# Parskatt/RoMa

Hardware: AMD Instinct MI355X
Metric: image-pairs/sec, roma_outdoor 560->864, batch=8 per GPU (higher is better)
Workload: dtype bf16; 1 GPU; roma_outdoor match() 560->864, symmetric, upsample_preds, 8 pairs/GPU/step, seeded synthetic weights + N(0,1) images; precision policy of the reference's bf16 timing script: bfloat16 DINOv2 + float16 autocast for VGG / decoder / refiners (ROMA_MIXED), f32 accumulate; precision_policy=mixed, global_batch=8, streams_per_gpu=2, parallelism=single GPU, outputs_finite=True

## Files before the change

include/roma_hip.h:

```cpp
#ifndef ROMA_HIP_H
#define ROMA_HIP_H
#include <stdint.h>
#ifdef __cplusplus
extern "C" {
#endif

typedef struct roma_model* roma_handle_t;

enum { ROMA_F32 = 0, ROMA_BF16 = 1, ROMA_F16 = 2,
       ROMA_MIXED = 3 };
int roma_h16_format(void);
enum { ROMA_ERR_ARG = -1, ROMA_ERR_HIP = -2, ROMA_ERR_STATE = -3 };

typedef struct {
  int coarse_h, coarse_w;
  int upsample_h, upsample_w;
  int symmetric;
  int upsample_preds;
  int attenuate_cert;
  int precision;
  int max_batch;
  int device;
} roma_config_t;

const char* roma_last_error(void);
const char* roma_version(void);
#define ROMA_ABI_VERSION 5
int roma_abi_stamp(void);
int roma_self_check(void);

typedef struct {
  const float *ln1_w, *ln1_b, *ln2_w, *ln2_b;
  const float *ls1, *ls2;
  const void *qkv_w, *proj_w, *fc1_w, *fc2_w;
  const float *qkv_b, *proj_b, *fc1_b, *fc2_b;
  int qkv_ldw, proj_ldw, fc1_ldw, fc2_ldw;
} roma_vit_block_t;

typedef struct {
  int B, H, W;
  int act;
  int bf16_residual;
  const float *im_a, *im_b;
  const void* patch_w;
  const float* patch_b;
  int patch_ldw;
  const float *cls_tok, *pos_emb;
  const roma_vit_block_t* blocks;
  int nblocks;
  const float *norm_w, *norm_b;
  void *col, *pt, *x, *xs, *ln, *ao, *hid, *q, *k, *vt;
  void* feat_out;
} roma_vit_args_t;
int roma_vit_forward(const roma_vit_args_t* a, void* stream);
int roma_op_convert_from_bf16(const void* in_bf16, void* out_h16, long n, void* stream);

int roma_create(const roma_config_t* cfg, roma_handle_t* out);
int roma_set_tensor(roma_handle_t h, const char* name, int ndim, const int64_t* shape, const void* data, int is_int64);
int roma_finalize(roma_handle_t h);
int roma_set_option(roma_handle_t h, const char* key, int value);
int roma_set_option_f(roma_handle_t h, const char* key, double value);
int roma_match(roma_handle_t h, int B, const float* im_a, const float* im_b, const float* im_a_hr,
               const float* im_b_hr, float* warp_out, float* cert_out, void* stream);
typedef struct {
  int upsample;
  int symmetric;
  double scale_factor;
  const float* seed_flow;
  const float* seed_cert;
  int seed_h, seed_w;
  float* flow[5];
  float* cert[5];
  void* feat[5];
} roma_forward_args_t;
int roma_forward(roma_handle_t h, int B, const float* im_a, const float* im_b, const roma_forward_args_t* a, void* stream);
long roma_debug_fetch(roma_handle_t h, const char* name, void* dst_host, long nbytes);
int roma_debug_inject(roma_handle_t h, const char* name, const void* src_host, long nbytes);
long roma_debug_trace(roma_handle_t h, int slot, unsigned long long* sums_host, long max_entries, char* names_host,
                      long names_bytes);
int roma_destroy(roma_handle_t h);
int roma_tuning(const char* key, int value);
long roma_tuning_describe(char* buf, long nbytes);
long roma_debug_gemm_trace(unsigned int* dst_host, long nbytes);
int roma_profile_enable(int on);
long roma_profile_report(char* buf, long nbytes);


int roma_op_local_corr(const void* feature0, const void* feature1, const float* warp, void* out, int B, int H, int W,
                       int C, int K, int nearest, int dt_in, int dt_out, void* stream);
int roma_op_local_corr_window(const void* feature0, const void* feature1, const float* warp, void* out, int B, int H,
                              int W, int C, int radius, float scale, long ldo, int dt_in, int dt_out, void* stream);

int roma_op_gemm(const void* A, long lda, const void* W, long ldw, void* C, long ldc, int M, int N, int K, int batch,
                 long sA, long sW, long sC, const float* bias, const float* scale, const float* res, long ldr,
                 int act, float alpha, int dt_in, int dt_out, void* stream);
int roma_op_conv3x3(const void* in, const void* w, const float* bias, void* out, int B, int H, int W, int Cin, int Cout,
                    int relu, int dt, void* stream);
int roma_op_conv3x3_slab(const void* in, const void* w, const float* bias, void* out, int B, int H, int W, int Cin, int Cout,
                         int relu, int dt, void* stream);
int roma_op_attention(const void* q, const void* k, const void* vt, void* out, int B, int heads, int N, int npad, int hd,
                      int dt_in, int dt_out, void* stream);
int roma_op_qkv_scatter_gemm(const void* A, const void* W, const float* bias, void* q, void* k, void* vt, int B, int N,
                             int npad, int heads, int hd, int K, int dt_in, int dt_out, void* stream);
int roma_op_layernorm(const float* x, const float* w, const float* b, void* out, long M, int D, float eps, int dt_out,
                      void* stream);
int roma_op_layernorm_dt(const void* x, int dt_in, const float* w, const float* b, void* out, long M, int D, float eps,
                         int dt_out, void* stream);
int roma_op_gemm_res_bf16(const void* A, long lda, const void* W, long ldw, void* C, long ldc, int M, int N, int K,
                          const float* bias, const float* scale, const void* res, long ldr, void* stream);
int roma_op_cholesky_solve_t(float* A, float* Ft, float* LT, float* Linv, float* LinvT, int n, int d, int batch,
                             void* stream);
int roma_op_gp(const void* x, const void* y, const float* pos_w, const float* pos_b, float* mu, int b, int h, int w, int dt,
               void* stream);
int roma_op_cls_to_flow(const float* logits, long ld, float* flow, float* cert, long M, void* stream);
int roma_op_resize_bilinear(const float* in, float* out, int B, int Hin, int Win, int Hout, int Wout, int nc,
                            void* stream);
int roma_op_refiner_input(const void* feat, long ldf, const float* flow, void* d, long ldd, const float* emb_w,
                          const float* emb_b, int B, int H, int W, int C, int E, int Kcorr, int nimg, int shift,
                          float disp_scale, int dt, void* stream);
int roma_op_dwconv5x5(const void* in, void* out, const float* w, const float* bias, int B, int H, int W, int Cp, int dt,
                      void* stream);
int roma_op_refiner_block(const void* in, void* out, const float* dw_w, const float* dw_b, const void* pw,
                          const float* pw_b, int B, int H, int W, int Cp, int dt, void* stream);
int roma_op_refiner_block_final(const void* in, float* delta, const float* dw_w, const float* dw_b, const void* pw_final,
                                const float* bias_final, int B, int H, int W, int Cp, int dt, void* stream);
int roma_op_refiner_apply_delta(const float* delta, float* flow, float* cert, long M, float sx, float sy, void* stream);
int roma_op_kde(const float* x, long n, int down, float std, int half_inputs, float* density, void* stream);
int roma_op_sample_warp_at(const float* warp, const float* cert, int H, int W, const float* xa, long n, float* xa_to_b,
                           float* cert_a, void* stream);
int roma_op_mutual_nn(const float* a, long na, const float* b, long nb, const float* cert_a, float cert_th, float max_dist,
                      int* match_b, void* ws_a, void* ws_b, void* stream);
int roma_op_mutual_nn_count(const float* a, long na, const float* b, long nb, const float* cert_a, float cert_th, float max_dist,
                            void* ws_a, void* ws_b, long long* offsets, void* stream);
int roma_op_mutual_nn_fill(const float* a, long na, const float* b, long nb, const float* cert_a, float cert_th, float max_dist,
                           const void* ws_a, const void* ws_b, long long* offsets, long long* pairs, void* stream);
long roma_op_multinomial_workspace(long n, long k);
int roma_op_multinomial(const float* weights, long n, long k, unsigned long long seed, long long* out_indices, void* workspace,
                        long workspace_bytes, void* stream);
long roma_op_ransac_workspace(int B, int N);
int roma_op_ransac(int model, const float* kpts_a, const float* kpts_b, const int* counts, const unsigned long long* seeds, int B,
                   int N, float threshold, double confidence, int max_iters, int refine, double* out_model, unsigned char* out_mask,
                   unsigned char* out_ok, int* out_info, void* workspace, long workspace_bytes, void* stream);
long roma_op_magsac_workspace(int B, int N);
int roma_op_magsac(int model, const float* kpts_a, const float* kpts_b, const int* counts, const unsigned long long* seeds, int B,
                   int N, float threshold, double confidence, int max_iters, int lo_iters, double* out_model, unsigned char* out_mask,
                   unsigned char* out_ok, int* out_info, double* out_score, void* workspace, long workspace_bytes, void* stream);
long roma_op_essential_workspace(int B, int N);
int roma_op_essential(const float* kpts_a, const float* kpts_b, const int* counts, const unsigned long long* seeds,
                      const double* camera_matrix, int B, int N, float threshold, double prob, int max_iters, double* out_e,
                      unsigned char* out_mask, unsigned char* out_ok, int* out_info, void* workspace, long workspace_bytes,
                      void* stream);
long roma_op_essential_magsac_workspace(int B, int N);
int roma_op_essential_magsac(const float* kpts_a, const float* kpts_b, const int* counts, const unsigned long long* seeds,
                             const double* camera_matrix, int B, int N, float threshold, double prob, int max_iters, int lo_iters,
                             double* out_e, unsigned char* out_mask, unsigned char* out_ok, int* out_info, double* out_score,
                             void* workspace, long workspace_bytes, void* stream);
int roma_op_essential_minimal(const double* x0, const double* x1, int S, double* out_e, int* out_n, void* stream);
long roma_op_recover_pose_workspace(int B, int N);
int roma_op_recover_pose(const double* E, const float* kpts_a, const float* kpts_b, const unsigned char* mask, const int* counts,
                         const double* camera_matrix, int B, int N, double distance_thresh, int* out_n_good, double* out_r,
                         double* out_t, unsigned char* out_mask, void* workspace, long workspace_bytes, void* stream);
long roma_op_refine_pose_workspace(int B, int N);
int roma_op_refine_pose(const double* R, const double* t, const float* kpts_a, const float* kpts_b, const int* counts,
                        const unsigned char* valid, int B, int N, double thr, int max_steps, double* out_r, double* out_t,
                        unsigned char* out_mask, int* out_info, void* workspace, long workspace_bytes, void* stream);
long roma_op_refine_model_workspace(int B, int N);
int roma_op_refine_model(int model, const double* M, const float* kpts_a, const float* kpts_b, const int* counts,
                         const unsigned char* valid, int B, int N, double thr, int max_steps, double* out_m, unsigned char* out_mask,
                         int* out_info, double* out_cost, void* workspace, long workspace_bytes, void* stream);
int roma_op_nchw_to_nhwc(const float* in, float* out, int B, int C, int H, int W, void* stream);
int roma_op_tiny_pos_embed(const float* corr_volume, float* out, int B, int H1, int W1, int H0, int W0, int exact_softmax,
                           void* stream);
int roma_op_gray_instnorm(const float* in, float* out, int B, int H, int W, int C, float eps, void* stream);
int roma_op_conv2d_nhwc(const float* in, const float* w, const float* bias, const float* res, float* out, int B, int H, int W,
                        int Cin, int Cout, int K, int stride, int pad, int relu, void* stream);
int roma_op_avgpool_nhwc(const float* in, float* out, int B, int H, int W, int C, int k, void* stream);
int roma_op_add3(const float* a, const float* b, const float* c, float* out, long n, void* stream);
int roma_op_tiny_matcher_input(const float* f0, const float* f1, const float* warp, int warp_channels, float* d, int B, int H,
                               int W, int H1, int W1, int C, int Cp, void* stream);
int roma_op_tiny_update(const float* base, int base_channels, const float* delta, long ldd, float sx, float sy, float* out,
                        long npix, void* stream);
int roma_op_tiny_final(const float* matches, float* warp, float* certainty, int B, int H, int W, void* stream);
int roma_op_visualize_warp(const float* warp, const float* certainty, const float* im_a, const float* im_b, int H, int W,
                           int symmetric, int im_h, int im_w, float* out, void* stream);
int roma_op_fb_consistency(const float* flow_fwd, const float* flow_bwd, int B, int H, int W, float th_n, float* out,
                           void* stream);
int roma_op_maxpool2x2(const void* in, void* out, int B, int H, int W, int C, int dt, void* stream);
int roma_op_pool_proj(const void* in, void* pooled, void* pf, const void* pw, long ldw, const float* pb, int N, int ldf, int B, int H,
                      int W, int C, int dt, void* stream);
int roma_op_refiner_out(const void* d, long ldd, int dt, const float* w, const float* b, float* flow, float* cert, long M,
                        int Cp, float sx, float sy, void* stream);
int roma_op_conv3x3_c3(const float* img, const float* w, const float* bias, void* out, int B, int H, int W, int dt_out,
                       void* stream);
int roma_op_conv3x3_c3_bf16(const float* img, const void* w, const float* bias, void* out, int B, int H, int W, void* stream);

#ifdef __cplusplus
}
#endif
#endif
```

roma_amd/_lib.py:

```python
from __future__ import annotations

import ctypes as C
import os

_HERE = os.path.dirname(os.path.abspath(__file__))
_HERE = os.environ.get("ROMA_LIB_DIR", _HERE)
LIB_PATH = os.path.join(_HERE, "libroma_hip.so")
LIB_PATHS = {"bf16": LIB_PATH, "f16": os.path.join(_HERE, "libroma_hip_f16.so")}

ROMA_F32, ROMA_BF16, ROMA_F16, ROMA_MIXED = 0, 1, 2, 3
H16_CODE = {"bf16": ROMA_BF16, "f16": ROMA_F16}


class RomaConfig(C.Structure):
    _fields_ = [("coarse_h", C.c_int), ("coarse_w", C.c_int), ("upsample_h", C.c_int), ("upsample_w", C.c_int),
                ("symmetric", C.c_int), ("upsample_preds", C.c_int), ("attenuate_cert", C.c_int),
                ("precision", C.c_int), ("max_batch", C.c_int), ("device", C.c_int)]


class RomaForwardArgs(C.Structure):
    _fields_ = [("upsample", C.c_int), ("symmetric", C.c_int), ("scale_factor", C.c_double),
                ("seed_flow", C.c_void_p), ("seed_cert", C.c_void_p), ("seed_h", C.c_int), ("seed_w", C.c_int),
                ("flow", C.c_void_p * 5), ("cert", C.c_void_p * 5), ("feat", C.c_void_p * 5)]


_vp, _i, _l, _f = C.c_void_p, C.c_int, C.c_long, C.c_float

SIGNATURES = {
    "roma_last_error": (C.c_char_p, []),
    "roma_version": (C.c_char_p, []),
    "roma_h16_format": (_i, []),
    "roma_abi_stamp": (_i, []),
    "roma_self_check": (_i, []),
    "roma_create": (_i, [C.POINTER(RomaConfig), C.POINTER(_vp)]),
    "roma_set_tensor": (_i, [_vp, C.c_char_p, _i, C.POINTER(C.c_int64), _vp, _i]),
    "roma_finalize": (_i, [_vp]),
    "roma_set_option": (_i, [_vp, C.c_char_p, _i]),
    "roma_set_option_f": (_i, [_vp, C.c_char_p, C.c_double]),
    "roma_match": (_i, [_vp, _i, _vp, _vp, _vp, _vp, _vp, _vp, _vp]),
    "roma_forward": (_i, [_vp, _i, _vp, _vp, C.POINTER(RomaForwardArgs), _vp]),
    "roma_debug_fetch": (_l, [_vp, C.c_char_p, _vp, _l]),
    "roma_debug_trace": (_l, [_vp, _i, _vp, _l, C.c_char_p, _l]),
    "roma_debug_inject": (_i, [_vp, C.c_char_p, _vp, _l]),
    "roma_destroy": (_i, [_vp]),
    "roma_tuning": (_i, [C.c_char_p, _i]),
    "roma_tuning_describe": (_l, [C.c_char_p, _l]),
    "roma_debug_gemm_trace": (_l, [_vp, _l]),
    "roma_vit_forward": (_i, [_vp, _vp]),
    "roma_op_convert_from_bf16": (_i, [_vp, _vp, _l, _vp]),
    "roma_profile_enable": (_i, [_i]),
    "roma_profile_report": (_l, [C.c_char_p, _l]),
    "roma_op_local_corr": (_i, [_vp, _vp, _vp, _vp, _i, _i, _i, _i, _i, _i, _i, _i, _vp]),
    "roma_op_local_corr_window": (_i, [_vp, _vp, _vp, _vp, _i, _i, _i, _i, _i, _f, _l, _i, _i, _vp]),
    "roma_op_gemm": (_i, [_vp, _l, _vp, _l, _vp, _l, _i, _i, _i, _i, _l, _l, _l, _vp, _vp, _vp, _l, _i, _f, _i, _i, _vp]),
    "roma_op_conv3x3": (_i, [_vp, _vp, _vp, _vp, _i, _i, _i, _i, _i, _i, _i, _vp]),
    "roma_op_conv3x3_slab": (_i, [_vp, _vp, _vp, _vp, _i, _i, _i, _i, _i, _i, _i, _vp]),
    "roma_op_attention": (_i, [_vp, _vp, _vp, _vp, _i, _i, _i, _i, _i, _i, _i, _vp]),
    "roma_op_qkv_scatter_gemm": (_i, [_vp, _vp, _vp, _vp, _vp, _vp, _i, _i, _i, _i, _i, _i, _i, _i, _vp]),
    "roma_op_layernorm": (_i, [_vp, _vp, _vp, _vp, _l, _i, _f, _i, _vp]),
    "roma_op_layernorm_dt": (_i, [_vp, _i, _vp, _vp, _vp, _l, _i, _f, _i, _vp]),
    "roma_op_gemm_res_bf16": (_i, [_vp, _l, _vp, _l, _vp, _l, _i, _i, _i, _vp, _vp, _vp, _l, _vp]),
    "roma_op_cholesky_solve_t": (_i, [_vp, _vp, _vp, _vp, _vp, _i, _i, _i, _vp]),
    "roma_op_gp": (_i, [_vp, _vp, _vp, _vp, _vp, _i, _i, _i, _i, _vp]),
    "roma_op_cls_to_flow": (_i, [_vp, _l, _vp, _vp, _l, _vp]),
    "roma_op_resize_bilinear": (_i, [_vp, _vp, _i, _i, _i, _i, _i, _i, _vp]),
    "roma_op_refiner_input": (_i, [_vp, _l, _vp, _vp, _l, _vp, _vp, _i, _i, _i, _i, _i, _i, _i, _i, _f, _i, _vp]),
    "roma_op_dwconv5x5": (_i, [_vp, _vp, _vp, _vp, _i, _i, _i, _i, _i, _vp]),
    "roma_op_refiner_block": (_i, [_vp, _vp, _vp, _vp, _vp, _vp, _i, _i, _i, _i, _i, _vp]),
    "roma_op_refiner_block_final": (_i, [_vp, _vp, _vp, _vp, _vp, _vp, _i, _i, _i, _i, _i, _vp]),
    "roma_op_refiner_apply_delta": (_i, [_vp, _vp, _vp, _l, _f, _f, _vp]),
    "roma_op_kde": (_i, [_vp, _l, _i, _f, _i, _vp, _vp]),
    "roma_op_sample_warp_at": (_i, [_vp, _vp, _i, _i, _vp, _l, _vp, _vp, _vp]),
    "roma_op_mutual_nn": (_i, [_vp, _l, _vp, _l, _vp, _f, _f, _vp, _vp, _vp, _vp]),
    "roma_op_mutual_nn_count": (_i, [_vp, _l, _vp, _l, _vp, _f, _f, _vp, _vp, _vp, _vp]),
    "roma_op_mutual_nn_fill": (_i, [_vp, _l, _vp, _l, _vp, _f, _f, _vp, _vp, _vp, _vp, _vp]),
    "roma_op_fb_consistency": (_i, [_vp, _vp, _i, _i, _i, _f, _vp, _vp]),
    "roma_op_visualize_warp": (_i, [_vp, _vp, _vp, _vp, _i, _i, _i, _i, _i, _vp, _vp]),
    "roma_op_multinomial_workspace": (_l, [_l, _l]),
    "roma_op_multinomial": (_i, [_vp, _l, _l, C.c_ulonglong, _vp, _vp, _l, _vp]),
    "roma_op_ransac_workspace": (_l, [_i, _i]),
    "roma_op_ransac": (_i, [_i, _vp, _vp, _vp, _vp, _i, _i, _f, C.c_double, _i, _i, _vp, _vp, _vp, _vp, _vp, _l, _vp]),
    "roma_op_magsac_workspace": (_l, [_i, _i]),
    "roma_op_magsac": (_i, [_i, _vp, _vp, _vp, _vp, _i, _i, _f, C.c_double, _i, _i, _vp, _vp, _vp, _vp, _vp, _vp, _l, _vp]),
    "roma_op_essential_workspace": (_l, [_i, _i]),
    "roma_op_essential": (_i, [_vp, _vp, _vp, _vp, _vp, _i, _i, _f, C.c_double, _i, _vp, _vp, _vp, _vp, _vp, _l, _vp]),
    "roma_op_essential_magsac_workspace": (_l, [_i, _i]),
    "roma_op_essential_magsac": (_i, [_vp, _vp, _vp, _vp, _vp, _i, _i, _f, C.c_double, _i, _i, _vp, _vp, _vp, _vp, _vp, _vp, _l, _vp]),
    "roma_op_essential_minimal": (_i, [_vp, _vp, _i, _vp, _vp, _vp]),
    "roma_op_recover_pose_workspace": (_l, [_i, _i]),
    "roma_op_recover_pose": (_i, [_vp, _vp, _vp, _vp, _vp, _vp, _i, _i, C.c_double, _vp, _vp, _vp, _vp, _vp, _l, _vp]),
    "roma_op_refine_pose_workspace": (_l, [_i, _i]),
    "roma_op_refine_pose": (_i, [_vp, _vp, _vp, _vp, _vp, _vp, _i, _i, C.c_double, _i, _vp, _vp, _vp, _vp, _vp, _l, _vp]),
    "roma_op_refine_model_workspace": (_l, [_i, _i]),
    "roma_op_refine_model": (_i, [_i, _vp, _vp, _vp, _vp, _vp, _i, _i, C.c_double, _i, _vp, _vp, _vp, _vp, _vp, _l, _vp]),
    "roma_op_nchw_to_nhwc": (_i, [_vp, _vp, _i, _i, _i, _i, _vp]),
    "roma_op_tiny_pos_embed": (_i, [_vp, _vp, _i, _i, _i, _i, _i, _i, _vp]),
    "roma_op_gray_instnorm": (_i, [_vp, _vp, _i, _i, _i, _i, _f, _vp]),
    "roma_op_conv2d_nhwc": (_i, [_vp, _vp, _vp, _vp, _vp, _i, _i, _i, _i, _i, _i, _i, _i, _i, _vp]),
    "roma_op_avgpool_nhwc": (_i, [_vp, _vp, _i, _i, _i, _i, _i, _vp]),
    "roma_op_add3": (_i, [_vp, _vp, _vp, _vp, _l, _vp]),
    "roma_op_tiny_matcher_input": (_i, [_vp, _vp, _vp, _i, _vp, _i, _i, _i, _i, _i, _i, _i, _vp]),
    "roma_op_tiny_update": (_i, [_vp, _i, _vp, _l, _f, _f, _vp, _l, _vp]),
    "roma_op_tiny_final": (_i, [_vp, _vp, _vp, _i, _i, _i, _vp]),
    "roma_op_maxpool2x2": (_i, [_vp, _vp, _i, _i, _i, _i, _i, _vp]),
    "roma_op_pool_proj": (_i, [_vp, _vp, _vp, _vp, _l, _vp, _i, _i, _i, _i, _i, _i, _i, _vp]),
    "roma_op_conv3x3_c3": (_i, [_vp, _vp, _vp, _vp, _i, _i, _i, _i, _vp]),
    "roma_op_conv3x3_c3_bf16": (_i, [_vp, _vp, _vp, _vp, _i, _i, _i, _vp]),
    "roma_op_refiner_out": (_i, [_vp, _l, _i, _vp, _vp, _vp, _vp, _l, _i, _f, _f, _vp]),
}

_libs = {}


class RomaHipError(RuntimeError):
    pass


def load(fmt: str = "bf16"):
    if fmt in _libs:
        return _libs[fmt]
    path = LIB_PATHS[fmt]
    if not os.path.exists(path):
        raise ImportError(f"{path} not found - build it with `python -c 'import __graft_entry__ as g; g.build()'` "
                          "(roma_amd has no CPU fallback)")
    lib = C.CDLL(path)
    for name, (res, args) in SIGNATURES.items():
        fn = getattr(lib, name)
        fn.restype = res
        fn.argtypes = args
    if lib.roma_h16_format() != H16_CODE[fmt]:
        raise ImportError(f"{path} does not store {fmt} (roma_h16_format() = {lib.roma_h16_format()})")
    lib.h16 = fmt
    _libs[fmt] = lib
    return lib


def fmt_of(dtype) -> str:
    return "f16" if str(dtype) == "torch.float16" else "bf16"


def last_error(lib=None) -> str:
    return (lib or load()).roma_last_error().decode("utf-8", "replace")


def check(rc: int, exc=RomaHipError, lib=None):
    if rc != 0:
        raise exc(last_error(lib))
    return rc
```

roma_amd/csrc/api.hip:

```cpp
#include <algorithm>
#include <mutex>
#include <map>
#include <vector>
#include <dlfcn.h>
#include <string.h>

#include "../../include/roma_hip.h"
#include "attention.h"
#include "conv64.h"
#include "conv_patch.h"
#include "elementwise.h"
#include "gemm.h"
#include "local_corr.h"
#include "pool_proj.h"
#include "model.h"
#include "refiner_block.h"
#include "kde.h"
#include "keypoints.h"
#include "tiny.h"
#include "tuning.h"
#include "vit.h"
#include "sampling.h"
#include "essential.h"
#include "model_refine.h"
// ... 262 lines not shown
    first = false;
  }
  if (auto f = peer_sym<long (*)(char*, long)>("roma_profile_report")) {
    const long n = f(nullptr, 0);
    if (n > 3) {
      std::string peer((size_t)n, '\0');
      if (f(&peer[0], n) > 0) {
        peer.resize(strlen(peer.c_str()));
        if (peer.size() > 2) js += (first ? "" : ", ") + peer.substr(1, peer.size() - 2);
      }
    }
  }
  js += "}";
  if (!buf) return (long)js.size() + 1;
  if (nbytes < (long)js.size() + 1) return ROMA_ERR_ARG;
  memcpy(buf, js.c_str(), js.size() + 1);
  return (long)js.size() + 1;
}

int roma_op_local_corr(const void* feature0, const void* feature1, const float* warp, void* out, int B, int H, int W,
                       int C, int K, int nearest, int dt_in, int dt_out, void* stream) {
  LocalCorrArgs a;
  a.nearest = nearest ? 1 : 0;
  a.f0 = feature0; a.f1 = feature1; a.warp = warp; a.out = out; a.B = B; a.H = H; a.W = W; a.C = C; a.K = K;
  a.ld0 = C; a.ld1 = C; a.ldo = K; a.nimg = B; a.f1_shift = 0; a.scale = 1.f; a.in_dt = DT(dt_in); a.out_dt = DT(dt_out);
  return local_corr_general_launch(a, S(stream));
}

int roma_op_local_corr_window(const void* feature0, const void* feature1, const float* warp, void* out, int B, int H,
                              int W, int C, int radius, float scale, long ldo, int dt_in, int dt_out, void* stream) {
  LocalCorrArgs a;
  a.f0 = feature0; a.f1 = feature1; a.warp = warp; a.out = out; a.B = B; a.H = H; a.W = W; a.C = C; a.radius = radius;
  a.ld0 = C; a.ld1 = C; a.ldo = ldo; a.nimg = B; a.f1_shift = 0; a.scale = scale; a.in_dt = DT(dt_in); a.out_dt = DT(dt_out);
  ROMA_REQUIRE(ldo >= (2 * radius + 1) * (2 * radius + 1), "local_corr_window: ldo < K");
  return local_corr_window_launch(a, S(stream));
}

int roma_op_gemm(const void* A, long lda, const void* W, long ldw, void* C, long ldc, int M, int N, int K, int batch,
                 long sA, long sW, long sC, const float* bias, const float* scale, const float* res, long ldr, int act,
                 float alpha, int dt_in, int dt_out, void* stream) {
  GemmArgs g;
  g.A = A; g.lda = lda; g.W = W; g.ldw = ldw; g.C = C; g.ldc = ldc; g.M = M; g.N = N; g.K = K; g.batch = batch;
  g.sA = sA; g.sW = sW; g.sC = sC; g.bias = bias; g.scale = scale; g.res = res; g.ldr = ldr; g.sR = sC; g.act = act;
  g.alpha = alpha; g.in_dt = DT(dt_in); g.out_dt = DT(dt_out);
  return gemm_launch(g, S(stream));
}

int roma_op_conv3x3(const void* in, const void* w, const float* bias, void* out, int B, int H, int W, int Cin, int Cout,
                    int relu, int dt, void* stream) {
  GemmArgs g;
  g.A = in; g.W = w; g.ldw = 9 * Cin; g.C = out; g.ldc = Cout; g.M = B * H * W; g.N = Cout; g.K = 9 * Cin;
  g.in_dt = DT(dt); g.out_dt = DT(dt); g.bias = bias; g.act = relu ? ACT_RELU : ACT_NONE;
  g.conv_h = H; g.conv_w = W; g.conv_c = Cin;
  return gemm_launch(g, S(stream));
}

int roma_op_conv3x3_slab(const void* in, const void* w, const float* bias, void* out, int B, int H, int W, int Cin, int Cout,
                         int relu, int dt, void* stream) {
  GemmArgs g;
  g.A = in; g.W = w; g.ldw = 9 * Cin; g.C = out; g.ldc = Cout; g.M = B * H * W; g.N = Cout; g.K = 9 * Cin;
  g.in_dt = DT(dt); g.out_dt = DT(dt); g.bias = bias; g.act = relu ? ACT_RELU : ACT_NONE;
  g.conv_h = H; g.conv_w = W; g.conv_c = Cin; g.conv_korder = 1;
  return gemm_launch(g, S(stream));
}

int roma_op_attention(const void* q, const void* k, const void* vt, void* out, int B, int heads, int N, int npad, int hd,
                      int dt_in, int dt_out, void* stream) {
  AttnArgs a;
  a.q = q; a.k = k; a.vt = vt; a.out = out; a.B = B; a.heads = heads; a.N = N; a.npad = npad; a.hd = hd;
  a.ldo = (long)heads * hd; a.in_dt = DT(dt_in); a.out_dt = DT(dt_out);
  return attention_launch(a, S(stream));
}

int roma_op_qkv_scatter_gemm(const void* A, const void* W, const float* bias, void* q, void* k, void* vt, int B, int N,
                             int npad, int heads, int hd, int K, int dt_in, int dt_out, void* stream) {
  GemmArgs g;
  g.A = A; g.lda = K; g.W = W; g.ldw = K; g.M = B * N; g.N = 3 * heads * hd; g.K = K; g.in_dt = DT(dt_in);
  g.out_dt = DT(dt_out); g.bias = bias; g.mode = EPI_QKV; g.q = q; g.k = k; g.vt = vt; g.heads = heads; g.hd = hd;
  g.ntok = N; g.npad = npad; g.qscale = 1.0f / sqrtf((float)hd);
  return gemm_launch(g, S(stream));
}

int roma_op_layernorm(const float* x, const float* w, const float* b, void* out, long M, int D, float eps, int dt_out,
                      void* stream) {
  return layernorm_launch(x, w, b, out, M, D, eps, DT(dt_out), S(stream));
}

int roma_op_layernorm_dt(const void* x, int dt_in, const float* w, const float* b, void* out, long M, int D, float eps,
                         int dt_out, void* stream) {
  return layernorm_launch_dt(x, DT(dt_in), w, b, out, M, D, eps, DT(dt_out), S(stream));
}

int roma_op_gemm_res_bf16(const void* A, long lda, const void* W, long ldw, void* C, long ldc, int M, int N, int K,
                          const float* bias, const float* scale, const void* res, long ldr, void* stream) {
  GemmArgs g;
  g.A = A; g.lda = lda; g.W = W; g.ldw = ldw; g.C = C; g.ldc = ldc; g.M = M; g.N = N; g.K = K;
  g.bias = bias; g.scale = scale; g.res_bf16 = res; g.ldr = ldr; g.in_dt = DT_BF16; g.out_dt = DT_BF16;
  return gemm_launch(g, S(stream));
}

int roma_op_cholesky_solve_t(float* A, float* Ft, float* LT, float* Linv, float* LinvT, int n, int d, int batch,
                             void* stream) {
  if (batch > 1 && Ft == A + (long)n * n)
    return cholesky_solve_t(A, Ft, LT, Linv, LinvT, n, d, batch, S(stream), (long)(n + d) * n, (long)(n + d) * n);
  return cholesky_solve_t(A, Ft, LT, Linv, LinvT, n, d, batch, S(stream));
}

int roma_op_gp(const void* x, const void* y, const float* pos_w, const float* pos_b, float* mu, int b, int h, int w, int dt,
               void* stream) {
  ROMA_REQUIRE(x && y && pos_w && pos_b && mu && b > 0 && h > 0 && w > 0, "roma_op_gp: bad arguments");
  hipStream_t st = S(stream);
  const int n = h * w;
  const size_t esz = DT(dt) == DT_F32 ? 4 : 2;
  Arena plan;
  plan.alloc((size_t)2 * b * n * 512 * esz);
  if (int rc = gp_posterior(nullptr, 512, DT(dt), b, false, h, w, pos_w, pos_b, mu, 512, plan, st, true)) return rc;
  Arena ar;
  ar.cap = plan.peak + 4096;
  ar.dry = false;
  ROMA_CHECK_HIP(hipMallocAsync(reinterpret_cast<void**>(&ar.base), ar.cap, st));
  char* pf = static_cast<char*>(ar.alloc((size_t)2 * b * n * 512 * esz));
  int rc = 0;
  if (hipMemcpyAsync(pf, x, (size_t)b * n * 512 * esz, hipMemcpyDeviceToDevice, st) != hipSuccess ||
      hipMemcpyAsync(pf + (size_t)b * n * 512 * esz, y, (size_t)b * n * 512 * esz, hipMemcpyDeviceToDevice, st) != hipSuccess) {
    set_error("roma_op_gp: device copy failed");
    rc = ROMA_ERR_HIP;
  }
  if (!rc) rc = gp_posterior(pf, 512, DT(dt), b, false, h, w, pos_w, pos_b, mu, 512, ar, st, false);
  (void)hipFreeAsync(ar.base, st);
  return rc;
}

int roma_op_cls_to_flow(const float* logits, long ld, float* flow, float* cert, long M, void* stream) {
  return cls_to_flow_launch(logits, ld, flow, cert, M, S(stream));
}

int roma_op_resize_bilinear(const float* in, float* out, int B, int Hin, int Win, int Hout, int Wout, int nc,
                            void* stream) {
  return resize_bilinear_launch(in, out, B, Hin, Win, Hout, Wout, nc, S(stream));
}

int roma_op_refiner_input(const void* feat, long ldf, const float* flow, void* d, long ldd, const float* emb_w,
                          const float* emb_b, int B, int H, int W, int C, int E, int Kcorr, int nimg, int shift,
                          float disp_scale, int dt, void* stream) {
  RefinerInputArgs a;
  a.feat = feat; a.ldf = ldf; a.flow = flow; a.d = d; a.ldd = ldd; a.emb_w = emb_w; a.emb_b = emb_b;
  a.B = B; a.H = H; a.W = W; a.C = C; a.E = E; a.Kcorr = Kcorr; a.nimg = nimg; a.shift = shift;
  a.disp_scale = disp_scale; a.dt = DT(dt);
  ROMA_REQUIRE(feat && flow && d && B > 0 && H > 0 && W > 0 && C > 0 && nimg > 0, "roma_op_refiner_input: bad arguments");
  ROMA_REQUIRE(ldd >= 2 * C + E + Kcorr && ldf >= C, "roma_op_refiner_input: row strides too small");
  return refiner_input_launch(a, S(stream));
}

int roma_op_dwconv5x5(const void* in, void* out, const float* w, const float* bias, int B, int H, int W, int Cp, int dt,
                      void* stream) {
  return dwconv5x5_launch(in, out, w, bias, B, H, W, Cp, DT(dt), S(stream));
}

int roma_op_refiner_block(const void* in, void* out, const float* dw_w, const float* dw_b, const void* pw,
                          const float* pw_b, int B, int H, int W, int Cp, int dt, void* stream) {
  if (refiner_block_wide_supported(Cp, DT(dt))) {
    const int rc = refiner_block_wide_try_launch(in, out, dw_w, dw_b, pw, Cp, pw_b, B, H, W, Cp, DT(dt), S(stream), true);
    if (rc <= 0) return rc;
    set_error("roma_op_refiner_block: the C = 576 kernel declined these tensors (16-byte aligned bf16 in / out / weights are required)");
    return ROMA_ERR_ARG;
  }
  return refiner_block_launch(in, out, dw_w, dw_b, pw, Cp, pw_b, B, H, W, Cp, DT(dt), S(stream));
}

int roma_op_refiner_block_final(const void* in, float* delta, const float* dw_w, const float* dw_b, const void* pw_final,
                                const float* bias_final, int B, int H, int W, int Cp, int dt, void* stream) {
  ROMA_REQUIRE(in && delta && dw_w && dw_b && pw_final && bias_final, "roma_op_refiner_block_final: null pointer");
  return refiner_block_final_launch(in, delta, dw_w, dw_b, pw_final, Cp, bias_final, B, H, W, Cp, DT(dt), S(stream));
}

int roma_op_refiner_apply_delta(const float* delta, float* flow, float* cert, long M, float sx, float sy, void* stream) {
  ROMA_REQUIRE(delta && flow && cert && M >= 0, "roma_op_refiner_apply_delta: null pointer");
  return refiner_apply_delta_launch(delta, flow, cert, M, sx, sy, S(stream));
}

int roma_op_kde(const float* x, long n, int down, float std, int half_inputs, float* density, void* stream) {
  return kde_launch(x, n, down, std, half_inputs, density, S(stream));
}

int roma_op_sample_warp_at(const float* warp, const float* cert, int H, int W, const float* xa, long n, float* xa_to_b,
                           float* cert_a, void* stream) {
  return sample_warp_at_launch(warp, cert, H, W, xa, n, xa_to_b, cert_a, S(stream));
}

int roma_op_mutual_nn(const float* a, long na, const float* b, long nb, const float* cert_a, float cert_th, float max_dist,
                      int* match_b, void* ws_a, void* ws_b, void* stream) {
  return mutual_nn_launch(a, na, b, nb, cert_a, cert_th, max_dist, match_b, static_cast<unsigned long long*>(ws_a),
                          static_cast<unsigned long long*>(ws_b), S(stream));
}

int roma_op_mutual_nn_count(const float* a, long na, const float* b, long nb, const float* cert_a, float cert_th, float max_dist,
                            void* ws_a, void* ws_b, long long* offsets, void* stream) {
  return mutual_nn_count_launch(a, na, b, nb, cert_a, cert_th, max_dist, static_cast<unsigned long long*>(ws_a),
                                static_cast<unsigned long long*>(ws_b), offsets, S(stream));
}
int roma_op_mutual_nn_fill(const float* a, long na, const float* b, long nb, const float* cert_a, float cert_th, float max_dist,
                           const void* ws_a, const void* ws_b, long long* offsets, long long* pairs, void* stream) {
  return mutual_nn_fill_launch(a, na, b, nb, cert_a, cert_th, max_dist, static_cast<const unsigned long long*>(ws_a),
                               static_cast<const unsigned long long*>(ws_b), offsets, pairs, S(stream));
}

long roma_op_multinomial_workspace(long n, long k) { return (long)multinomial_workspace_bytes(n, k); }
int roma_op_multinomial(const float* weights, long n, long k, unsigned long long seed, long long* out_indices, void* workspace,
                        long workspace_bytes, void* stream) {
  return multinomial_launch(weights, n, k, seed, out_indices, workspace, (size_t)workspace_bytes, S(stream));
}
long roma_op_ransac_workspace(int B, int N) { return (long)ransac_workspace_bytes(B, N); }
int roma_op_ransac(int model, const float* kpts_a, const float* kpts_b, const int* counts, const unsigned long long* seeds, int B,
                   int N, float threshold, double confidence, int max_iters, int refine, double* out_model, unsigned char* out_mask,
                   unsigned char* out_ok, int* out_info, void* workspace, long workspace_bytes, void* stream) {
  return ransac_launch(model, kpts_a, kpts_b, counts, seeds, B, N, threshold, confidence, max_iters, refine, out_model, out_mask,
                       out_ok, out_info, workspace, (size_t)(workspace_bytes > 0 ? workspace_bytes : 0), S(stream));
}
long roma_op_magsac_workspace(int B, int N) { return (long)magsac_workspace_bytes(B, N); }
int roma_op_magsac(int model, const float* kpts_a, const float* kpts_b, const int* counts, const unsigned long long* seeds, int B,
                   int N, float threshold, double confidence, int max_iters, int lo_iters, double* out_model, unsigned char* out_mask,
                   unsigned char* out_ok, int* out_info, double* out_score, void* workspace, long workspace_bytes, void* stream) {
  return magsac_launch(model, kpts_a, kpts_b, counts, seeds, B, N, threshold, confidence, max_iters, lo_iters, out_model, out_mask,
                       out_ok, out_info, out_score, workspace, (size_t)(workspace_bytes > 0 ? workspace_bytes : 0), S(stream));
}
long roma_op_essential_workspace(int B, int N) { return (long)essential_workspace_bytes(B, N); }
int roma_op_essential(const float* kpts_a, const float* kpts_b, const int* counts, const unsigned long long* seeds,
                      const double* camera_matrix, int B, int N, float threshold, double prob, int max_iters, double* out_e,
                      unsigned char* out_mask, unsigned char* out_ok, int* out_info, void* workspace, long workspace_bytes,
                      void* stream) {
  return essential_launch(kpts_a, kpts_b, counts, seeds, camera_matrix, B, N, threshold, prob, max_iters, out_e, out_mask, out_ok,
                          out_info, workspace, (size_t)(workspace_bytes > 0 ? workspace_bytes : 0), S(stream));
}
long roma_op_essential_magsac_workspace(int B, int N) { return (long)essential_magsac_workspace_bytes(B, N); }
int roma_op_essential_magsac(const float* kpts_a, const float* kpts_b, const int* counts, const unsigned long long* seeds,
                             const double* camera_matrix, int B, int N, float threshold, double prob, int max_iters, int lo_iters,
                             double* out_e, unsigned char* out_mask, unsigned char* out_ok, int* out_info, double* out_score,
                             void* workspace, long workspace_bytes, void* stream) {
  return essential_magsac_launch(kpts_a, kpts_b, counts, seeds, camera_matrix, B, N, threshold, prob, max_iters, lo_iters, out_e,
                                 out_mask, out_ok, out_info, out_score, workspace,
                                 (size_t)(workspace_bytes > 0 ? workspace_bytes : 0), S(stream));
}
int roma_op_essential_minimal(const double* x0, const double* x1, int S_, double* out_e, int* out_n, void* stream) {
  return essential_minimal_launch(x0, x1, S_, out_e, out_n, S(stream));
}
long roma_op_recover_pose_workspace(int B, int N) { return (long)recover_pose_workspace_bytes(B, N); }
int roma_op_recover_pose(const double* E, const float* kpts_a, const float* kpts_b, const unsigned char* mask, const int* counts,
                         const double* camera_matrix, int B, int N, double distance_thresh, int* out_n_good, double* out_r,
                         double* out_t, unsigned char* out_mask, void* workspace, long workspace_bytes, void* stream) {
  return recover_pose_launch(E, kpts_a, kpts_b, mask, counts, camera_matrix, B, N, distance_thresh, out_n_good, out_r, out_t,
                             out_mask, workspace, (size_t)(workspace_bytes > 0 ? workspace_bytes : 0), S(stream));
}
long roma_op_refine_pose_workspace(int B, int N) { return (long)refine_pose_workspace_bytes(B, N); }
int roma_op_refine_pose(const double* R, const double* t, const float* kpts_a, const float* kpts_b, const int* counts,
                        const unsigned char* valid, int B, int N, double thr, int max_steps, double* out_r, double* out_t,
                        unsigned char* out_mask, int* out_info, void* workspace, long workspace_bytes, void* stream) {
  return refine_pose_launch(R, t, kpts_a, kpts_b, counts, valid, B, N, thr, max_steps, out_r, out_t, out_mask, out_info, workspace,
                            (size_t)(workspace_bytes > 0 ? workspace_bytes : 0), S(stream));
}
long roma_op_refine_model_workspace(int B, int N) { return (long)refine_model_workspace_bytes(B, N); }
int roma_op_refine_model(int model, const double* M, const float* kpts_a, const float* kpts_b, const int* counts,
                         const unsigned char* valid, int B, int N, double thr, int max_steps, double* out_m, unsigned char* out_mask,
                         int* out_info, double* out_cost, void* workspace, long workspace_bytes, void* stream) {
  return refine_model_launch(model, M, kpts_a, kpts_b, counts, valid, B, N, thr, max_steps, out_m, out_mask, out_info, out_cost,
                             workspace, (size_t)(workspace_bytes > 0 ? workspace_bytes : 0), S(stream));
}
int roma_op_nchw_to_nhwc(const float* in, float* out, int B, int C, int H, int W, void* stream) {
  return nchw_to_nhwc_launch(in, out, B, C, H, W, S(stream));
}
int roma_op_tiny_pos_embed(const float* corr_volume, float* out, int B, int H1, int W1, int H0, int W0, int exact_softmax,
                           void* stream) {
  return tiny_pos_embed_launch(corr_volume, out, B, H1, W1, H0, W0, exact_softmax, S(stream));
}
int roma_op_gray_instnorm(const float* in, float* out, int B, int H, int W, int C, float eps, void* stream) {
  return gray_instnorm_launch(in, out, B, H, W, C, eps, S(stream));
}
int roma_op_conv2d_nhwc(const float* in, const float* w, const float* bias, const float* res, float* out, int B, int H, int W,
                        int Cin, int Cout, int K, int stride, int pad, int relu, void* stream) {
  return conv2d_nhwc_launch(in, w, bias, res, out, B, H, W, Cin, Cout, K, stride, pad, relu, S(stream));
}
int roma_op_avgpool_nhwc(const float* in, float* out, int B, int H, int W, int C, int k, void* stream) {
  return avgpool_nhwc_launch(in, out, B, H, W, C, k, S(stream));
}
int roma_op_add3(const float* a, const float* b, const float* c, float* out, long n, void* stream) {
  return add3_launch(a, b, c, out, n, S(stream));
}
int roma_op_tiny_matcher_input(const float* f0, const float* f1, const float* warp, int warp_channels, float* d, int B, int H,
                               int W, int H1, int W1, int C, int Cp, void* stream) {
  return tiny_matcher_input_launch(f0, f1, warp, warp_channels, d, B, H, W, H1, W1, C, Cp, S(stream));
}
int roma_op_tiny_update(const float* base, int base_channels, const float* delta, long ldd, float sx, float sy, float* out,
                        long npix, void* stream) {
  return tiny_update_launch(base, base_channels, delta, ldd, sx, sy, out, npix, S(stream));
}
int roma_op_tiny_final(const float* matches, float* warp, float* certainty, int B, int H, int W, void* stream) {
  return tiny_final_launch(matches, warp, certainty, B, H, W, S(stream));
}
int roma_op_visualize_warp(const float* warp, const float* certainty, const float* im_a, const float* im_b, int H, int W,
                           int symmetric, int im_h, int im_w, float* out, void* stream) {
  return visualize_warp_launch(warp, certainty, im_a, im_b, H, W, symmetric, im_h, im_w, out, S(stream));
}
int roma_op_fb_consistency(const float* flow_fwd, const float* flow_bwd, int B, int H, int W, float th_n, float* out,
                           void* stream) {
  return fb_consistency_launch(flow_fwd, flow_bwd, B, H, W, th_n, out, S(stream));
}

int roma_op_maxpool2x2(const void* in, void* out, int B, int H, int W, int C, int dt, void* stream) {
  return maxpool2x2_launch(in, out, B, H, W, C, DT(dt), S(stream));
}
// ... 23 lines not shown
```

roma_amd/csrc/dwconv_ring.hip:

```cpp
#include <stdlib.h>

#include <algorithm>

#include "elementwise.h"
#include "tuning.h"
#include "gemm.h"

namespace roma {

typedef __attribute__((ext_vector_type(2))) float f32x2;
#define ROMA_LDS __attribute__((address_space(3)))
typedef ROMA_LDS unsigned char lds_u8;

__device__ __attribute__((aligned(256))) unsigned int g_dwr_zero_page[64];

constexpr int DWR_ROWB = 3072;
constexpr int DWR_PXW = 16;
constexpr int DWR_NR = 6;
constexpr int DWR_RING = 4 * DWR_NR * DWR_ROWB;
static_assert(3 * (DWR_NR - 1) + 4 * (DWR_NR - 1) <= 63, "vmcnt is a 6-bit counter");
static_assert(2 * DWR_RING <= 160 * 1024, "two workgroups per CU");

#define ROMA_DWR_WAIT_VM(N) asm volatile("s_waitcnt vmcnt(%0)" ::"n"(N) : "memory")

__device__ __forceinline__ void dwr_glds16(const char* src, lds_u8* lds_wave_base) {
  __builtin_amdgcn_global_load_lds((const __attribute__((address_space(1))) void*)src, (ROMA_LDS void*)lds_wave_base, 16, 0, 0);
}

__device__ __forceinline__ void dwr_read(unsigned long long (&cr)[8], unsigned rd) {
  asm volatile(
      "ds_read_b64 %0, %8\n\tds_read_b64 %1, %8 offset:128\n\tds_read_b64 %2, %8 offset:256\n\t"
      "ds_read_b64 %3, %8 offset:384\n\tds_read_b64 %4, %8 offset:640\n\tds_read_b64 %5, %8 offset:768\n\t"
      "ds_read_b64 %6, %8 offset:896\n\tds_read_b64 %7, %8 offset:1024"
      : "=&v"(cr[0]), "=&v"(cr[1]), "=&v"(cr[2]), "=&v"(cr[3]), "=&v"(cr[4]), "=&v"(cr[5]), "=&v"(cr[6]), "=&v"(cr[7])
      : "v"(rd)
      : "memory");
}
__device__ __forceinline__ void dwr_wait(unsigned long long (&cr)[8]) {
  asm volatile("s_waitcnt lgkmcnt(0)"
               : "+v"(cr[0]), "+v"(cr[1]), "+v"(cr[2]), "+v"(cr[3]), "+v"(cr[4]), "+v"(cr[5]), "+v"(cr[6]), "+v"(cr[7])::"memory");
}

__device__ __forceinline__ void dwr_row(f32x2 (&acc)[5][4][2], const f32x4 (&wreg)[25], f32x2 bias0, f32x2 bias1,
                                        unsigned long long (&cr)[8], unsigned rd_next, bool store, bf16_t* orow, long Cp, int npx) {
  f32x2 v[8][2];
#define ROMA_DWR_CVT(J)                                                  \
  {                                                                      \
    const uint32_t lo_ = (uint32_t)cr[J], hi_ = (uint32_t)(cr[J] >> 32); \
    v[J][0] = f32x2{h16_lo(lo_), h16_hi(lo_)};                           \
    v[J][1] = f32x2{h16_lo(hi_), h16_hi(hi_)};                           \
  }
  ROMA_DWR_CVT(0) ROMA_DWR_CVT(1) ROMA_DWR_CVT(2) ROMA_DWR_CVT(3) ROMA_DWR_CVT(4) ROMA_DWR_CVT(5) ROMA_DWR_CVT(6) ROMA_DWR_CVT(7)
#undef ROMA_DWR_CVT
#pragma unroll
  for (int j = 0; j < 8; ++j) asm volatile("" : "+v"(v[j][0]), "+v"(v[j][1]));
  dwr_read(cr, rd_next);
#pragma unroll
  for (int kx = 0; kx < 5; ++kx) {
    __builtin_amdgcn_sched_barrier(0);
#pragma unroll
    for (int k = 0; k < 5; ++k) {
      const f32x4 wx = wreg[(4 - k) * 5 + kx];
      const f32x2 w0 = f32x2{wx[0], wx[1]}, w1 = f32x2{wx[2], wx[3]};
#pragma unroll
      for (int px = 0; px < 4; ++px) {
        acc[k][px][0] = v[px + kx][0] * w0 + (k == 4 && kx == 0 ? bias0 : acc[k][px][0]);
        acc[k][px][1] = v[px + kx][1] * w1 + (k == 4 && kx == 0 ? bias1 : acc[k][px][1]);
      }
    }
    __builtin_amdgcn_sched_barrier(0);
  }
  if (store) {
#pragma unroll
    for (int px = 0; px < 4; ++px) {
      if (px < npx) {
        uint2 u;
        u.x = pack_relu_h16x2(acc[0][px][0][0], acc[0][px][0][1]);
        u.y = pack_relu_h16x2(acc[0][px][1][0], acc[0][px][1][1]);
        *reinterpret_cast<uint2*>(orow + (long)px * Cp) = u;
      }
    }
  }
#pragma unroll
  for (int k = 0; k < 4; ++k)
#pragma unroll
    for (int px = 0; px < 4; ++px) {
      acc[k][px][0] = acc[k + 1][px][0];
      acc[k][px][1] = acc[k + 1][px][1];
    }
  dwr_wait(cr);
}

__global__ __launch_bounds__(256, 2) void dwconv5x5_ring_kernel(const bf16_t* __restrict__ in, bf16_t* __restrict__ out,
                                                                const float* __restrict__ w, const float* __restrict__ bias,
                                                                int B, int H, int W, int Cp, int SY, int nchunk, int nxg,
                                                                long ntasks) {
  constexpr int NR = DWR_NR;
  __shared__ __attribute__((aligned(1024))) unsigned char ring[DWR_RING];
  const long nwg = (ntasks + 3) / 4, wg_per_xcd = (nwg + 7) / 8;
  const long lw = (long)(blockIdx.x % 8) * wg_per_xcd + blockIdx.x / 8;
  const int lane = threadIdx.x & 63;
  const int wv = __builtin_amdgcn_readfirstlane((int)(threadIdx.x >> 6));
  const long task = lw * 4 + wv;
  if (lw >= nwg || task >= ntasks) return;
  const int xg = (int)(task % nxg);
  long r = task / nxg;
  const int chunk = (int)(r % nchunk);
  r /= nchunk;
  const int yt = (H + SY - 1) / SY;
  const int ys = (int)(r % yt) * SY;
  const int b = (int)(r / yt);
  const int sy = min(SY, H - ys);
  const int T = sy + 4;

  const int cg = lane & 15, xq = lane >> 4;
  const int c = chunk * 64 + cg * 4;

  f32x4 wreg[25];
#pragma unroll
  for (int t = 0; t < 25; ++t) wreg[t] = *reinterpret_cast<const f32x4*>(w + (long)t * Cp + c);
  const f32x4 bx = *reinterpret_cast<const f32x4*>(bias + c);
#pragma unroll
  for (int t = 0; t < 25; ++t) asm volatile("" : "+v"(wreg[t]));
  const f32x2 bias0 = f32x2{bx[0], bx[1]}, bias1 = f32x2{bx[2], bx[3]};
  asm volatile("s_waitcnt vmcnt(0)" ::: "memory");

  const int xb = xg * DWR_PXW + xq * 4;
  const int x0 = xg * DWR_PXW - 2;
  const int npx = min(4, W - xb);

  const char* zsrc = reinterpret_cast<const char*>(g_dwr_zero_page);
  const char* inb = reinterpret_cast<const char*>(in + ((long)b * H * W) * Cp) + (long)chunk * 128;
  const long pitch = (long)W * Cp * 2;
  const __amdgpu_buffer_rsrc_t rs_in = __builtin_amdgcn_make_buffer_rsrc(const_cast<char*>(inb), 0, (int)((long)H * pitch - (long)chunk * 128), 0x00020000);
  unsigned voff[3];
#pragma unroll
  for (int i = 0; i < 3; ++i) {
    const int p = 64 * i + lane, s = p >> 3, part = p & 7;
    const int x = x0 + s - s / 5;
    const bool ok = (s % 5 != 4) && x >= 0 && x < W;
    voff[i] = ok ? (unsigned)(x * Cp * 2 + part * 16) : 0x80000000u;
  }
  unsigned vout = 0x80000000u;
  asm volatile("" : "+v"(vout));
  lds_u8* const myring = (lds_u8*)ring + wv * (NR * DWR_ROWB);
#define ROMA_DWR_BL16(VOFF, SOFF, DST) \
  __builtin_amdgcn_raw_ptr_buffer_load_lds(rs_in, (ROMA_LDS void*)(DST), 16, (int)(VOFF), (int)(SOFF), 0, 0)
#define ROMA_DWR_ISSUE(RROW, SLOT)                                                         \
  {                                                                                        \
    const int yy_ = ys - 2 + (RROW);                                                       \
    if ((RROW) < T && yy_ >= 0 && yy_ < H) {                             \
      const int so_ = yy_ * (int)pitch;                                                    \
      _Pragma("unroll") for (int i = 0; i < 3; ++i) ROMA_DWR_BL16(voff[i], so_, myring + (SLOT) * DWR_ROWB + i * 1024); \
    } else {                                                                               \
      _Pragma("unroll") for (int i = 0; i < 3; ++i) ROMA_DWR_BL16(vout, 0, myring + (SLOT) * DWR_ROWB + i * 1024); \
    }                                                                                      \
  }

  f32x2 acc[5][4][2];
#pragma unroll
  for (int s5 = 0; s5 < 5; ++s5)
#pragma unroll
    for (int px = 0; px < 4; ++px) {
      acc[s5][px][0] = bias0;
      acc[s5][px][1] = bias1;
    }
  const unsigned ring_lds = (unsigned)(size_t)myring;
  const unsigned rd0 = ring_lds + (unsigned)(xq * 5 * 128 + cg * 8);
  bf16_t* const obase = out + ((long)b * H * W) * Cp + c;

#pragma unroll
  for (int rr = 0; rr < NR - 1; ++rr) ROMA_DWR_ISSUE(rr, rr);
  unsigned long long cr[8];
  ROMA_DWR_WAIT_VM(3 * (NR - 2));
  dwr_read(cr, rd0);
  dwr_wait(cr);

  int slot1 = 1;
  int fill = NR - 1;
  bf16_t* orow = obase + ((long)ys * W + xb) * Cp;
  const long orow_step = (long)W * Cp;
#pragma nounroll
  for (int t = 0; t < T; ++t) {
    ROMA_DWR_ISSUE(t + NR - 1, fill);
    ROMA_DWR_WAIT_VM(3 * (NR - 2));
    const bool st = t >= 4;
    dwr_row(acc, wreg, bias0, bias1, cr, rd0 + (unsigned)slot1 * DWR_ROWB, st && npx > 0, orow, (long)Cp, npx);
    if (st) orow += orow_step;
    fill = fill + 1 == NR ? 0 : fill + 1;
    slot1 = slot1 + 1 == NR ? 0 : slot1 + 1;
  }
#undef ROMA_DWR_ISSUE
  ROMA_DWR_WAIT_VM(0);
}

int dwconv5x5_ring_try_launch(const void* in, void* out, const float* w, const float* bias, int B, int H, int W, int Cp, int dt,
                              hipStream_t s) {
  const int dw_ring = tuning(SW_DW_RING);
  if (!dw_ring) return 1;
  if (dt != DT_BF16 || Cp % 64 != 0 || Cp < 256 || H < 1 || W < 1) return 1;
  if ((long)H * W * Cp * 2 >= (1l << 31)) return 1;
  if ((reinterpret_cast<uintptr_t>(in) & 15) != 0 || (reinterpret_cast<uintptr_t>(out) & 7) != 0) return 1;
  if ((reinterpret_cast<uintptr_t>(w) & 15) != 0 || (reinterpret_cast<uintptr_t>(bias) & 15) != 0) return 1;
  const int nchunk = Cp / 64;
  const int nxg = (W + DWR_PXW - 1) / DWR_PXW;
  int SY = H;
  {
    long best = -1;
    const long per_strip = (long)B * nxg * nchunk;
    const int max_sy = std::max(6, (int)tuning(SW_DWR_MAXSY));
    for (int ns = (H + max_sy - 1) / max_sy; ns <= std::max(1, H / 6); ++ns) {
      const int sy = (H + ns - 1) / ns;
      const long nt = per_strip * ((H + sy - 1) / sy);
      const long cost = ((nt + 2047) / 2048) * (sy + 7);
      if (best < 0 || cost < best) {
        best = cost;
        SY = sy;
      }
    }
  }
  const long ntasks = (long)B * ((H + SY - 1) / SY) * nxg * nchunk;
  ROMA_REQUIRE(ntasks < (1l << 31), "dwconv5x5: grid too large");
  const long min_elems = tuning(SW_DW_RING_MINELEMS);
  if (dw_ring != 2 && (long)B * H * W * Cp < min_elems) return 1;
  ProfScope ps("dwconv5x5_kernel<" ROMA_H16_NAME ">", 2.0 * (double)B * H * W * Cp * 2.0, "byte", s);
  const long nwg = (ntasks + 3) / 4;
  hipLaunchKernelGGL(dwconv5x5_ring_kernel, dim3((unsigned)(((nwg + 7) / 8) * 8)), dim3(256), 0, s, (const bf16_t*)in,
                     (bf16_t*)out, w, bias, B, H, W, Cp, SY, nchunk, nxg, ntasks);
  ROMA_LAUNCH_CHECK();
  return 0;
}

}
```

roma_amd/csrc/elementwise.h:

```cpp
#pragma once
#include "common.h"

namespace roma {

int layernorm_launch(const float* x, const float* w, const float* b, void* out, long M, int D, float eps,
                     int dt_out, hipStream_t s);
int layernorm_launch_dt(const void* x, int dt_in, const float* w, const float* b, void* out, long M, int D, float eps,
                        int dt_out, hipStream_t s);

int conv3x3_c3_launch(const float* img, const float* w, const float* bias, void* out, int B, int H, int W,
                      int dt_out, hipStream_t s);

int im2col3x3_c3_launch(const float* img, void* out, int B, int H, int W, int dt_out, hipStream_t s);

int maxpool2x2_launch(const void* in, void* out, int B, int H, int W, int C, int dt, hipStream_t s);

int im2col_patch14_launch(const float* img, void* out, int B, int H, int W, int Kpad, int dt_out, hipStream_t s);

int assemble_tokens_launch(const float* patch, const float* cls, const float* pos, float* tokens, int B, int T,
                           int D, hipStream_t s);

int copy2d_launch(const void* in, long ldi, int dt_in, void* out, long ldo, int dt_out, long rows, int cols,
                  hipStream_t s);

int convert_from_bf16_launch(const void* in, void* out, long n, hipStream_t s);

int rownorm_launch(const void* in, long ld, int dt, float* norms, long M, int C, hipStream_t s);

int gp_basis_launch(const float* w, const float* b, float* Ft, int Dg, int h, int wdt, int npad, hipStream_t s, int copies = 1,
                    long stride = 0);

int transpose_launch(const float* in, float* out, int n, long ld, int batch, hipStream_t s, long stride_in = 0, long stride_out = 0);

int chol_diag_launch(float* A, long ld, long strideA, float* Linv, float* LinvT, int k, int nblk, int batch,
                     hipStream_t s);

int chol_col_launch(float* A, long ld, long strideA, float* LT, long strideLT, int n, int d, float* Linv, float* LinvT, int k,
                    int nblk, int batch, unsigned epoch, hipStream_t s);
int chol_col_restore_launch(float* A, long ld, long strideA, const float* LT, long strideLT, int n, int batch, hipStream_t s);

int pad_identity_launch(float* A, long ld, long strideA, int n, int npad, int batch, hipStream_t s);

int cls_to_flow_launch(const float* logits, long ld, float* flow, float* cert, long M, hipStream_t s);

struct RefinerInputArgs {
  const void* feat = nullptr;
  long ldf = 0;
  const float* flow = nullptr;
  void* d = nullptr;
  long ldd = 0;
  const float* emb_w = nullptr;
  const float* emb_b = nullptr;
  int B = 0, H = 0, W = 0, C = 0, E = 0, Kcorr = 0, nimg = 0, shift = 0;
  float disp_scale = 1.f;
  int dt = 0;
};
int refiner_input_launch(const RefinerInputArgs& a, hipStream_t s);

int dwconv5x5_launch(const void* in, void* out, const float* w, const float* bias, int B, int H, int W, int Cp,
                     int dt, hipStream_t s);
int dwconv5x5_ring_try_launch(const void* in, void* out, const float* w, const float* bias, int B, int H, int W, int Cp, int dt,
                              hipStream_t s);

int refiner_out_launch(const void* d, long ldd, int dt, const float* w , const float* b ,
                       float* flow, float* cert, long M, int Cp, float sx, float sy, hipStream_t s);
int refiner_apply_delta_launch(const float* delta, float* flow, float* cert, long M, float sx, float sy, hipStream_t s);

int resize_bilinear_launch(const float* in, float* out, int B, int Hin, int Win, int Hout, int Wout, int nc,
                           hipStream_t s);

struct FinalArgs {
  const float* flow = nullptr;
  const float* cert = nullptr;
  const float* cert16 = nullptr;
  float* warp = nullptr;
  float* certainty = nullptr;
  int B = 0, H = 0, W = 0, h16 = 0, w16 = 0, symmetric = 1;
};
int final_epilogue_launch(const FinalArgs& a, hipStream_t s);

int checksum_cols_launch(const void* p, long rows, int ld, int c0, int c1, unsigned long long* out, hipStream_t s);
int checksum_launch(const void* p, size_t bytes, unsigned long long* out, hipStream_t s);

}
```

roma_amd/csrc/elementwise.hip:

```cpp
#include <algorithm>
#include "elementwise.h"
#include "tuning.h"
#include "chol_diag.h"
#include <stdio.h>

#include <stdlib.h>
#include "gemm.h"

namespace roma {

#define ROMA_DT_SWITCH(dt, T, ...)            \
  if ((dt) == DT_F32) { using T = float; __VA_ARGS__; } else { using T = bf16_t; __VA_ARGS__; }

__device__ inline float wave_sum(float v) {
#pragma unroll
  for (int off = 32; off >= 1; off >>= 1) v += __shfl_xor(v, off);
  return v;
}

__device__ inline float pix_coord(int i, int n) {
  const float start = (float)(-1.0 + 1.0 / n), end = (float)(1.0 - 1.0 / n);
  if (n == 1) return start;
  const float step = (end - start) / (float)(n - 1);
  return (i < n / 2) ? start + step * (float)i : end - step * (float)(n - 1 - i);
// ... 357 lines not shown
  for (int j = ty; j < 32; j += 8)
    if (y0 + j < n && x0 + tx < n) tile[j][tx] = ib[(long)(y0 + j) * ld + x0 + tx];
  __syncthreads();
  for (int j = ty; j < 32; j += 8)
    if (x0 + j < n && y0 + tx < n) ob[(long)(x0 + j) * ld + y0 + tx] = tile[tx][j];
}

int transpose_launch(const float* in, float* out, int n, long ld, int batch, hipStream_t s, long stride_in, long stride_out) {
  dim3 grid((unsigned)((n + 31) / 32), (unsigned)((n + 31) / 32), (unsigned)batch);
  hipLaunchKernelGGL(transpose_kernel, grid, dim3(256), 0, s, in, out, n, ld, stride_in > 0 ? stride_in : (long)n * ld,
                     stride_out > 0 ? stride_out : (long)n * ld);
  ROMA_LAUNCH_CHECK();
  return 0;
}

__global__ __launch_bounds__(256) void chol_diag_kernel(float* A, long ld, long strideA, float* Linv, float* LinvT,
                                                        int k, int nblk) {
  constexpr int S = CHOL_S;
  __shared__ __attribute__((aligned(16))) float L[64 * S];
  __shared__ __attribute__((aligned(16))) float LT[64 * S];
  __shared__ __attribute__((aligned(16))) float XT[64 * S];
  __shared__ int progress;
  float* Ab = A + (long)blockIdx.x * strideA + ((long)k * 64) * ld + (long)k * 64;
  const int tid = threadIdx.x;
  const int wave = __builtin_amdgcn_readfirstlane(tid >> 6);
  const int i = tid & 63;
  for (int idx = tid; idx < 64 * 16; idx += 256) {
    const int row = idx >> 4, c4 = idx & 15;
    *reinterpret_cast<f32x4*>(&L[row * S + c4 * 4]) = *reinterpret_cast<const f32x4*>(Ab + (long)row * ld + c4 * 4);
  }
  if (tid == 0) progress = -1;
  __syncthreads();
  if (wave == 0) chol_diag_factor_wave(L, LT, &progress, i);
  else if (wave == 1) chol_diag_inverse_wave(L, XT, &progress, i);
  __syncthreads();
  chol_diag_writeback(L, XT, Ab, ld, Linv + ((long)blockIdx.x * nblk + k) * 4096, LinvT + ((long)blockIdx.x * nblk + k) * 4096,
                      tid, 256);
}

int chol_diag_launch(float* A, long ld, long strideA, float* Linv, float* LinvT, int k, int nblk, int batch,
                     hipStream_t s) {
  hipLaunchKernelGGL(chol_diag_kernel, dim3((unsigned)batch), dim3(256), 0, s, A, ld, strideA, Linv, LinvT, k, nblk);
  ROMA_LAUNCH_CHECK();
  return 0;
}

__global__ __launch_bounds__(256) void pad_identity_kernel(float* A, long ld, long strideA, int n, int npad) {
  float* Ab = A + (long)blockIdx.y * strideA;
  const long total = (long)npad * npad;
  for (long idx = (long)blockIdx.x * 256 + threadIdx.x; idx < total; idx += (long)gridDim.x * 256) {
    const int i = (int)(idx / npad), j = (int)(idx % npad);
    if (i >= n || j >= n) Ab[(long)i * ld + j] = (i == j) ? 1.f : 0.f;
  }
}

int pad_identity_launch(float* A, long ld, long strideA, int n, int npad, int batch, hipStream_t s) {
  if (npad == n) return 0;
  const long total = (long)npad * npad;
  dim3 grid((unsigned)std::min<long>((total + 255) / 256, 4096), (unsigned)batch);
  hipLaunchKernelGGL(pad_identity_kernel, grid, dim3(256), 0, s, A, ld, strideA, n, npad);
  ROMA_LAUNCH_CHECK();
  return 0;
}

__global__ __launch_bounds__(256) void cls_to_flow_kernel(const float* logits, long ld, float* flow, float* cert, long M) {
  const int lane = threadIdx.x & 63;
  const long row = (long)blockIdx.x * 4 + (threadIdx.x >> 6);
  if (row >= M) return;
  const float* lr = logits + row * ld;
  float mx = -INFINITY;
  int arg = 0;
  f32x4 v[16];
#pragma unroll
  for (int i = 0; i < 16; ++i) {
    v[i] = *reinterpret_cast<const f32x4*>(lr + (i * 64 + lane) * 4);
#pragma unroll
    for (int j = 0; j < 4; ++j)
      if (v[i][j] > mx) {
        mx = v[i][j];
        arg = (i * 64 + lane) * 4 + j;
      }
  }
#pragma unroll
  for (int off = 32; off >= 1; off >>= 1) {
    const float om = __shfl_xor(mx, off);
    const int oa = __shfl_xor(arg, off);
    if (om > mx || (om == mx && oa < arg)) {
      mx = om;
      arg = oa;
    }
  }
  float se = 0.f;
#pragma unroll
  for (int i = 0; i < 16; ++i)
#pragma unroll
    for (int j = 0; j < 4; ++j) se += expf(v[i][j] - mx);
  se = wave_sum(se);
  if (lane == 0) {
    const int idx5[5] = {arg - 1, arg, arg + 1, arg - 64, arg + 64};
    float fx = 0.f, fy = 0.f, tot = 0.f;
#pragma unroll
    for (int t = 0; t < 5; ++t) {
      const int c = min(max(idx5[t], 0), 4095);
      const float p = expf(lr[c] - mx) / se;
      fx += p * pix_coord(c & 63, 64);
      fy += p * pix_coord(c >> 6, 64);
      tot += p;
    }
    flow[row * 2 + 0] = fx / tot;
    flow[row * 2 + 1] = fy / tot;
    cert[row] = lr[4096];
  }
}

int cls_to_flow_launch(const float* logits, long ld, float* flow, float* cert, long M, hipStream_t s) {
  ROMA_REQUIRE(ld % 4 == 0 && ld >= 4097, "cls_to_flow: bad leading dimension");
  dim3 grid((unsigned)((M + 3) / 4));
  hipLaunchKernelGGL(cls_to_flow_kernel, grid, dim3(256), 0, s, logits, ld, flow, cert, M);
  ROMA_LAUNCH_CHECK();
  return 0;
}

template <typename T>
__global__ __launch_bounds__(256) void refiner_input_kernel(const RefinerInputArgs a) {
  const int lane = threadIdx.x & 63;
  const long HW = (long)a.H * a.W;
  const long pix = (long)blockIdx.x * 4 + (threadIdx.x >> 6);
  if (pix >= (long)a.B * HW) return;
  const int b = (int)(pix / HW);
  const long p = pix - (long)b * HW;
  const int y = (int)(p / a.W), x = (int)(p - (long)y * a.W);
  const T* feat = reinterpret_cast<const T*>(a.feat);
  const T* fq = feat + ((long)b * HW + p) * a.ldf;
  const int simg = (b + a.shift) % a.nimg;
  const T* fs = feat + (long)simg * HW * a.ldf;
  T* d = reinterpret_cast<T*>(a.d) + pix * a.ldd;
  const float wx = a.flow[pix * 2 + 0], wy = a.flow[pix * 2 + 1];
  float ix = ((wx + 1.f) * a.W - 1.f) * 0.5f, iy = ((wy + 1.f) * a.H - 1.f) * 0.5f;
  ix = fminf(fmaxf(ix, -1.0e6f), 1.0e6f);
  iy = fminf(fmaxf(iy, -1.0e6f), 1.0e6f);
  const float fx0 = floorf(ix), fy0 = floorf(iy);
  const int x0 = (int)fx0, y0 = (int)fy0;
  const float tx = ix - fx0, ty = iy - fy0;
  const float wgt[4] = {(1.f - tx) * (1.f - ty), tx * (1.f - ty), (1.f - tx) * ty, tx * ty};
  bool ok[4];
  long off[4];
#pragma unroll
  for (int t = 0; t < 4; ++t) {
    const int yy = y0 + (t >> 1), xx = x0 + (t & 1);
    ok[t] = yy >= 0 && yy < a.H && xx >= 0 && xx < a.W;
    off[t] = ((long)yy * a.W + xx) * a.ldf;
  }
  for (int c = lane * 4; c < a.C; c += 256) {
    ElemIO<T>::st4(d + c, ElemIO<T>::ld4(fq + c));
    f32x4 acc = {0.f, 0.f, 0.f, 0.f};
#pragma unroll
    for (int t = 0; t < 4; ++t)
      if (ok[t]) {
        const f32x4 v = ElemIO<T>::ld4(fs + off[t] + c);
        acc += wgt[t] * v;
      }
    ElemIO<T>::st4(d + a.C + c, acc);
  }
  const float dx = a.disp_scale * (wx - pix_coord(x, a.W)), dy = a.disp_scale * (wy - pix_coord(y, a.H));
  for (int e = lane; e < a.E; e += 64) {
    const float v = a.emb_w[e * 2 + 0] * dx + a.emb_w[e * 2 + 1] * dy + a.emb_b[e];
    ElemIO<T>::st(d + 2 * a.C + e, v);
  }
  for (long c = 2 * a.C + a.E + a.Kcorr + lane; c < a.ldd; c += 64) ElemIO<T>::st(d + c, 0.f);
}

template <typename T>
__global__ __launch_bounds__(256) void refiner_input_small_kernel(const RefinerInputArgs a) {
  const long HW = (long)a.H * a.W;
  const int slots = (int)a.ldd;
  const long total = (long)a.B * HW * slots;
  const T* feat = reinterpret_cast<const T*>(a.feat);
  for (long idx = (long)blockIdx.x * 256 + threadIdx.x; idx < total; idx += (long)gridDim.x * 256) {
    const int c = (int)(idx % slots);
    const long pix = idx / slots;
    const int b = (int)(pix / HW);
    const long p = pix - (long)b * HW;
    T* d = reinterpret_cast<T*>(a.d) + pix * a.ldd;
    if (c < a.C) {
      ElemIO<T>::st(d + c, ElemIO<T>::ld(feat + ((long)b * HW + p) * a.ldf + c));
    } else if (c < 2 * a.C) {
      const int cc = c - a.C;
      const int simg = (b + a.shift) % a.nimg;
      const T* fs = feat + (long)simg * HW * a.ldf;
      const float wx = a.flow[pix * 2 + 0], wy = a.flow[pix * 2 + 1];
      float ix = ((wx + 1.f) * a.W - 1.f) * 0.5f, iy = ((wy + 1.f) * a.H - 1.f) * 0.5f;
      ix = fminf(fmaxf(ix, -1.0e6f), 1.0e6f);
      iy = fminf(fmaxf(iy, -1.0e6f), 1.0e6f);
      const float fx0 = floorf(ix), fy0 = floorf(iy);
      const int x0 = (int)fx0, y0 = (int)fy0;
      const float tx = ix - fx0, ty = iy - fy0;
      const float wgt[4] = {(1.f - tx) * (1.f - ty), tx * (1.f - ty), (1.f - tx) * ty, tx * ty};
      float acc = 0.f;
#pragma unroll
      for (int t = 0; t < 4; ++t) {
        const int yy = y0 + (t >> 1), xx = x0 + (t & 1);
        if (yy >= 0 && yy < a.H && xx >= 0 && xx < a.W)
          acc += wgt[t] * ElemIO<T>::ld(fs + ((long)yy * a.W + xx) * a.ldf + cc);
      }
      ElemIO<T>::st(d + c, acc);
    } else if (c < 2 * a.C + a.E) {
      const int e = c - 2 * a.C;
      const int y = (int)(p / a.W), x = (int)(p - (long)y * a.W);
      const float dx = a.disp_scale * (a.flow[pix * 2 + 0] - pix_coord(x, a.W));
      const float dy = a.disp_scale * (a.flow[pix * 2 + 1] - pix_coord(y, a.H));
      ElemIO<T>::st(d + c, a.emb_w[e * 2 + 0] * dx + a.emb_w[e * 2 + 1] * dy + a.emb_b[e]);
    } else if (c >= 2 * a.C + a.E + a.Kcorr) {
      ElemIO<T>::st(d + c, 0.f);
    }
  }
}

template <typename T> struct VecIO;
template <> struct VecIO<float> {
  static constexpr int CV = 4;
  typedef f32x4 Raw;
  __device__ static inline Raw ldraw(const float* p) { return *reinterpret_cast<const f32x4*>(p); }
  __device__ static inline void cvt(const Raw& x, float* v) { v[0] = x[0]; v[1] = x[1]; v[2] = x[2]; v[3] = x[3]; }
  __device__ static inline void ld(const float* p, float* v) {
    const f32x4 x = *reinterpret_cast<const f32x4*>(p);
    v[0] = x[0]; v[1] = x[1]; v[2] = x[2]; v[3] = x[3];
  }
  __device__ static inline void st(float* p, const float* v) { *reinterpret_cast<f32x4*>(p) = f32x4{v[0], v[1], v[2], v[3]}; }
};
template <> struct VecIO<bf16_t> {
  static constexpr int CV = 8;
  typedef uint4 Raw;
  __device__ static inline Raw ldraw(const bf16_t* p) { return *reinterpret_cast<const uint4*>(p); }
  __device__ static inline void cvt(const Raw& u, float* v) {
    v[0] = h16_lo(u.x); v[1] = h16_hi(u.x);
    v[2] = h16_lo(u.y); v[3] = h16_hi(u.y);
    v[4] = h16_lo(u.z); v[5] = h16_hi(u.z);
    v[6] = h16_lo(u.w); v[7] = h16_hi(u.w);
  }
  __device__ static inline void ld(const bf16_t* p, float* v) {
    const uint4 u = *reinterpret_cast<const uint4*>(p);
    v[0] = h16_lo(u.x); v[1] = h16_hi(u.x);
    v[2] = h16_lo(u.y); v[3] = h16_hi(u.y);
    v[4] = h16_lo(u.z); v[5] = h16_hi(u.z);
    v[6] = h16_lo(u.w); v[7] = h16_hi(u.w);
  }
  __device__ static inline void st(bf16_t* p, const float* v) {
    uint4 u;
    u.x = pack_bf16x2(v[0], v[1]);
    u.y = pack_bf16x2(v[2], v[3]);
    u.z = pack_bf16x2(v[4], v[5]);
    u.w = pack_bf16x2(v[6], v[7]);
    *reinterpret_cast<uint4*>(p) = u;
  }
};

template <typename T, int C, int E>
__global__ __launch_bounds__(256) void refiner_input_pix_kernel(const RefinerInputArgs a) {
  constexpr int LDF = 16, LDD = 24;
  const long HW = (long)a.H * a.W;
  const long pix = (long)blockIdx.x * 256 + threadIdx.x;
  if (pix >= (long)a.B * HW) return;
  const int b = (int)(pix / HW);
  const long p = pix - (long)b * HW;
  const int y = (int)(p / a.W), x = (int)(p - (long)y * a.W);
  const T* feat = reinterpret_cast<const T*>(a.feat);
  const T* fq = feat + ((long)b * HW + p) * LDF;
  const int simg = (b + a.shift) % a.nimg;
  const T* fs = feat + (long)simg * HW * LDF;
  if constexpr (sizeof(T) == 2) {
    static_assert(C <= 16 && 2 * C + E <= LDD && LDD == 24 && LDF == 16, "layout");
    float q[16], xh[16];
    VecIO<T>::ld(fq, q);
    VecIO<T>::ld(fq + 8, q + 8);
#pragma unroll
    for (int j = 0; j < 16; ++j) xh[j] = 0.f;
    const float wx = a.flow[pix * 2 + 0], wy = a.flow[pix * 2 + 1];
    float ix = ((wx + 1.f) * a.W - 1.f) * 0.5f, iy = ((wy + 1.f) * a.H - 1.f) * 0.5f;
    ix = fminf(fmaxf(ix, -1.0e6f), 1.0e6f);
    iy = fminf(fmaxf(iy, -1.0e6f), 1.0e6f);
    const float fx0 = floorf(ix), fy0 = floorf(iy);
    const int x0 = (int)fx0, y0 = (int)fy0;
    const float tx = ix - fx0, ty = iy - fy0;
    const float wgt[4] = {(1.f - tx) * (1.f - ty), tx * (1.f - ty), (1.f - tx) * ty, tx * ty};
#pragma unroll
    for (int t = 0; t < 4; ++t) {
      const int yy = y0 + (t >> 1), xx = x0 + (t & 1);
      if (yy >= 0 && yy < a.H && xx >= 0 && xx < a.W) {
        const T* r = fs + ((long)yy * a.W + xx) * LDF;
        float v[16];
        VecIO<T>::ld(r, v);
        VecIO<T>::ld(r + 8, v + 8);
#pragma unroll
        for (int j = 0; j < C; ++j) xh[j] += wgt[t] * v[j];
      }
    }
    const float dx = a.disp_scale * (wx - pix_coord(x, a.W)), dy = a.disp_scale * (wy - pix_coord(y, a.H));
    float o[LDD];
#pragma unroll
    for (int c = 0; c < C; ++c) {
      o[c] = q[c];
      o[C + c] = xh[c];
    }
#pragma unroll
    for (int e = 0; e < E; ++e) o[2 * C + e] = a.emb_w[e * 2 + 0] * dx + a.emb_w[e * 2 + 1] * dy + a.emb_b[e];
#pragma unroll
    for (int c = 2 * C + E; c < LDD; ++c) o[c] = 0.f;
    T* d = reinterpret_cast<T*>(a.d) + pix * LDD;
#pragma unroll
    for (int c8 = 0; c8 < LDD / 8; ++c8) VecIO<T>::st(d + c8 * 8, o + c8 * 8);
    return;
  }
  float q[12], xh[12];
#pragma unroll
  for (int c4 = 0; c4 < 3; ++c4) {
    const f32x4 v = ElemIO<T>::ld4(fq + c4 * 4);
#pragma unroll
    for (int j = 0; j < 4; ++j) {
      q[c4 * 4 + j] = v[j];
      xh[c4 * 4 + j] = 0.f;
    }
  }
  const float wx = a.flow[pix * 2 + 0], wy = a.flow[pix * 2 + 1];
  float ix = ((wx + 1.f) * a.W - 1.f) * 0.5f, iy = ((wy + 1.f) * a.H - 1.f) * 0.5f;
  ix = fminf(fmaxf(ix, -1.0e6f), 1.0e6f);
  iy = fminf(fmaxf(iy, -1.0e6f), 1.0e6f);
  const float fx0 = floorf(ix), fy0 = floorf(iy);
  const int x0 = (int)fx0, y0 = (int)fy0;
  const float tx = ix - fx0, ty = iy - fy0;
  const float wgt[4] = {(1.f - tx) * (1.f - ty), tx * (1.f - ty), (1.f - tx) * ty, tx * ty};
#pragma unroll
  for (int t = 0; t < 4; ++t) {
    const int yy = y0 + (t >> 1), xx = x0 + (t & 1);
    if (yy >= 0 && yy < a.H && xx >= 0 && xx < a.W) {
      const T* r = fs + ((long)yy * a.W + xx) * LDF;
#pragma unroll
      for (int c4 = 0; c4 < 3; ++c4) {
        const f32x4 v = ElemIO<T>::ld4(r + c4 * 4);
#pragma unroll
        for (int j = 0; j < 4; ++j) xh[c4 * 4 + j] += wgt[t] * v[j];
      }
    }
  }
  const float dx = a.disp_scale * (wx - pix_coord(x, a.W)), dy = a.disp_scale * (wy - pix_coord(y, a.H));
  float o[LDD];
#pragma unroll
  for (int c = 0; c < C; ++c) {
    o[c] = q[c];
    o[C + c] = xh[c];
  }
#pragma unroll
  for (int e = 0; e < E; ++e) o[2 * C + e] = a.emb_w[e * 2 + 0] * dx + a.emb_w[e * 2 + 1] * dy + a.emb_b[e];
#pragma unroll
  for (int c = 2 * C + E; c < LDD; ++c) o[c] = 0.f;
  T* d = reinterpret_cast<T*>(a.d) + pix * LDD;
#pragma unroll
  for (int c4 = 0; c4 < LDD / 4; ++c4) ElemIO<T>::st4(d + c4 * 4, f32x4{o[c4 * 4], o[c4 * 4 + 1], o[c4 * 4 + 2], o[c4 * 4 + 3]});
}

template <typename T>
__global__ __launch_bounds__(256) void refiner_input_vec_kernel(const RefinerInputArgs a, int lpp) {
  constexpr int CV = VecIO<T>::CV;
  const int lane = threadIdx.x & 63;
  const int sub = lane & (lpp - 1), pw = lane / lpp, ppw = 64 / lpp;
  const long HW = (long)a.H * a.W;
  const long pix = ((long)blockIdx.x * 4 + (threadIdx.x >> 6)) * ppw + pw;
  if (pix >= (long)a.B * HW) return;
  const int b = (int)(pix / HW);
  const long p = pix - (long)b * HW;
  const int y = (int)(p / a.W), x = (int)(p - (long)y * a.W);
  const T* feat = reinterpret_cast<const T*>(a.feat);
  const T* fq = feat + ((long)b * HW + p) * a.ldf;
  const int simg = (b + a.shift) % a.nimg;
  const T* fs = feat + (long)simg * HW * a.ldf;
  T* d = reinterpret_cast<T*>(a.d) + pix * a.ldd;
  const float wx = a.flow[pix * 2 + 0], wy = a.flow[pix * 2 + 1];
  float ix = ((wx + 1.f) * a.W - 1.f) * 0.5f, iy = ((wy + 1.f) * a.H - 1.f) * 0.5f;
  ix = fminf(fmaxf(ix, -1.0e6f), 1.0e6f);
  iy = fminf(fmaxf(iy, -1.0e6f), 1.0e6f);
  const float fx0 = floorf(ix), fy0 = floorf(iy);
  const int x0 = (int)fx0, y0 = (int)fy0;
  const float tx = ix - fx0, ty = iy - fy0;
  const float wgt[4] = {(1.f - tx) * (1.f - ty), tx * (1.f - ty), (1.f - tx) * ty, tx * ty};
  bool ok[4];
  long off[4];
#pragma unroll
  for (int t = 0; t < 4; ++t) {
    const int yy = y0 + (t >> 1), xx = x0 + (t & 1);
    ok[t] = yy >= 0 && yy < a.H && xx >= 0 && xx < a.W;
    off[t] = ((long)min(max(yy, 0), a.H - 1) * a.W + min(max(xx, 0), a.W - 1)) * a.ldf;
  }
  for (int c = sub * CV; c < a.C; c += lpp * CV) {
    *reinterpret_cast<uint4*>(d + c) = *reinterpret_cast<const uint4*>(fq + c);
    float r[CV];
#pragma unroll
    for (int j = 0; j < CV; ++j) r[j] = 0.f;
#pragma unroll
    for (int t = 0; t < 4; ++t) {
      float tv[CV];
      VecIO<T>::ld(fs + off[t] + c, tv);
#pragma unroll
      for (int j = 0; j < CV; ++j) r[j] = ok[t] ? r[j] + wgt[t] * tv[j] : r[j];
    }
    VecIO<T>::st(d + a.C + c, r);
  }
  const float dx = a.disp_scale * (wx - pix_coord(x, a.W)), dy = a.disp_scale * (wy - pix_coord(y, a.H));
  for (int e = sub; e < a.E; e += lpp) {
    const float v = a.emb_w[e * 2 + 0] * dx + a.emb_w[e * 2 + 1] * dy + a.emb_b[e];
    ElemIO<T>::st(d + 2 * a.C + e, v);
  }
  for (long c = 2 * a.C + a.E + a.Kcorr + sub; c < a.ldd; c += lpp) ElemIO<T>::st(d + c, 0.f);
}

int refiner_input_launch(const RefinerInputArgs& a, hipStream_t s) {
  const long npix = (long)a.B * a.H * a.W;
  const double es = a.dt == DT_F32 ? 4.0 : 2.0;
  char pname[64];
  snprintf(pname, sizeof pname, "refiner_input_warp<C=%d,%s>", a.C, a.dt == DT_F32 ? "f32" : ROMA_H16_NAME);
  ProfScope ps(pname, (double)npix * (2.0 * a.C * es + 8.0 + (double)(a.ldd - a.Kcorr) * es), "byte", s);
  if (a.C == 9 && a.E == 6 && a.Kcorr == 0 && a.ldf == 16 && a.ldd == 24) {
    dim3 grid((unsigned)((npix + 255) / 256));
    ROMA_DT_SWITCH(a.dt, T, hipLaunchKernelGGL((refiner_input_pix_kernel<T, 9, 6>), grid, dim3(256), 0, s, a));
    ROMA_LAUNCH_CHECK();
    return 0;
  }
  if (a.C % 4 != 0 || a.C < 32) {
    const long total = npix * a.ldd;
    dim3 grid((unsigned)std::min<long>((total + 255) / 256, 1 << 20));
    ROMA_DT_SWITCH(a.dt, T, hipLaunchKernelGGL(refiner_input_small_kernel<T>, grid, dim3(256), 0, s, a));
    ROMA_LAUNCH_CHECK();
    return 0;
  }
  ROMA_REQUIRE(a.ldf % 4 == 0 && a.ldd % 4 == 0, "refiner_input: strides must be multiples of 4");
  {
    const int cv = a.dt == DT_F32 ? 4 : 8;
    const bool aligned = ((reinterpret_cast<uintptr_t>(a.feat) | reinterpret_cast<uintptr_t>(a.d)) & 15) == 0;
    const bool vec_off = tuning(SW_RI_VEC) == 0;
    if (!vec_off && aligned && a.C % cv == 0 && a.ldf % cv == 0 && a.ldd % cv == 0) {
      int lpp = 1;
      while (lpp < 64 && lpp * cv < a.C) lpp *= 2;
      const long per_wg = 4 * (64 / lpp);
      dim3 vgrid((unsigned)((npix + per_wg - 1) / per_wg));
      ROMA_DT_SWITCH(a.dt, T, hipLaunchKernelGGL(refiner_input_vec_kernel<T>, vgrid, dim3(256), 0, s, a, lpp));
      ROMA_LAUNCH_CHECK();
      return 0;
    }
  }
  dim3 grid((unsigned)((npix + 3) / 4));
  ROMA_DT_SWITCH(a.dt, T, hipLaunchKernelGGL(refiner_input_kernel<T>, grid, dim3(256), 0, s, a));
  ROMA_LAUNCH_CHECK();
  return 0;
}

typedef __attribute__((ext_vector_type(2))) float f32x2;

template <typename T> struct RawVec;
template <> struct RawVec<float> {
  typedef f32x4 raw;
  __device__ static inline raw ld(const float* p) { return *reinterpret_cast<const f32x4*>(p); }
  __device__ static inline raw zero() { return f32x4{0.f, 0.f, 0.f, 0.f}; }
  __device__ static inline raw mask(raw r, uint32_t m) {
    return f32x4{__uint_as_float(__float_as_uint(r[0]) & m), __uint_as_float(__float_as_uint(r[1]) & m),
                 __uint_as_float(__float_as_uint(r[2]) & m), __uint_as_float(__float_as_uint(r[3]) & m)};
  }
  __device__ static inline void cvt(raw r, f32x2& a, f32x2& b) { a = f32x2{r[0], r[1]}; b = f32x2{r[2], r[3]}; }
  __device__ static inline void st(float* p, f32x2 a, f32x2 b) { *reinterpret_cast<f32x4*>(p) = f32x4{a[0], a[1], b[0], b[1]}; }
};
template <> struct RawVec<bf16_t> {
  typedef uint2 raw;
  __device__ static inline raw ld(const bf16_t* p) { return *reinterpret_cast<const uint2*>(p); }
  __device__ static inline raw zero() { return make_uint2(0, 0); }
  __device__ static inline raw mask(raw r, uint32_t m) { return make_uint2(r.x & m, r.y & m); }
  __device__ static inline void cvt(raw r, f32x2& a, f32x2& b) {
    a = f32x2{h16_lo(r.x), h16_hi(r.x)};
    b = f32x2{h16_lo(r.y), h16_hi(r.y)};
  }
  __device__ static inline void st(bf16_t* p, f32x2 a, f32x2 b) {
    uint2 u;
    u.x = pack_bf16x2(a[0], a[1]);
    u.y = pack_bf16x2(b[0], b[1]);
    *reinterpret_cast<uint2*>(p) = u;
  }
};

template <typename T>
__global__ __launch_bounds__(256, 2) void dwconv5x5_kernel(const T* in, T* out, const float* w, const float* bias, int B,
                                                           int H, int W, int Cp, int SY, int GC, int nchunk, int nxg,
                                                           int nblocks) {
  typedef typename RawVec<T>::raw raw_t;
  extern __shared__ __attribute__((aligned(16))) float wsm[];
  const int per_xcd = (nblocks + 7) / 8;
  const long lb = (long)(blockIdx.x % 8) * per_xcd + blockIdx.x / 8;
  if (lb >= nblocks) return;
  const int chunk = (int)(lb % nchunk);
  long r = lb / nchunk;
  const int xg = (int)(r % nxg);
  r /= nxg;
  const int yt = (H + SY - 1) / SY;
  const int ys = (int)(r % yt) * SY;
  const int b = (int)(r / yt);
  const int XQ = 256 / GC;
  const int cg = threadIdx.x % GC, xq = threadIdx.x / GC;
  const int c0 = chunk * GC * 4;
  constexpr int cw = 256;
  {
    const int q4 = GC;
    const int nvec = 26 * q4;
    f32x4 tmp[7];
#pragma unroll
    for (int it = 0; it < 7; ++it) {
      const int i = threadIdx.x + 256 * it;
      f32x4 v = {0.f, 0.f, 0.f, 0.f};
      if (i < nvec) {
        const int t = i / q4, cq = i - t * q4;
        const int ch = c0 + cq * 4;
        if (ch < Cp) v = *reinterpret_cast<const f32x4*>(t < 25 ? w + (long)t * Cp + ch : bias + ch);
      }
      tmp[it] = v;
    }
#pragma unroll
    for (int it = 0; it < 7; ++it) {
      const int i = threadIdx.x + 256 * it;
      if (i < nvec) {
        const int t = i / q4, cq = i - t * q4;
        *reinterpret_cast<f32x4*>(&wsm[t * cw + cq * 4]) = tmp[it];
      }
    }
  }
  __syncthreads();
  const int c = c0 + cg * 4;
  const int xb = (xg * XQ + xq) * 4;
  if (xq >= XQ || c >= Cp || xb >= W) return;
  const int sy = min(SY, H - ys);

  const f32x4 bx = *reinterpret_cast<const f32x4*>(&wsm[25 * cw + cg * 4]);
  const f32x2 bias0 = f32x2{bx[0], bx[1]}, bias1 = f32x2{bx[2], bx[3]};
  f32x2 acc[5][4][2];
#pragma unroll
  for (int s5 = 0; s5 < 5; ++s5)
#pragma unroll
    for (int px = 0; px < 4; ++px) {
      acc[s5][px][0] = bias0;
      acc[s5][px][1] = bias1;
    }
  bool colok[8];
#pragma unroll
  for (int j = 0; j < 8; ++j) colok[j] = (xb - 2 + j >= 0) && (xb - 2 + j < W);
  long colofs[8];
#pragma unroll
  for (int j = 0; j < 8; ++j) colofs[j] = (long)min(max(xb - 2 + j, 0), W - 1) * Cp;
  const T* base = in + ((long)b * H * W) * Cp + c;
  T* obase = out + ((long)b * H * W) * Cp + c;

#define ROMA_DW_LOAD_ROW(TT, DST)                                                                         \
  {                                                                                                       \
    const int yy_ = ys - 2 + (TT);                                                                        \
    const bool rok_ = yy_ >= 0 && yy_ < H;                                                                \
    const T* rowp_ = base + (long)min(max(yy_, 0), H - 1) * W * Cp;                                       \
    _Pragma("unroll") for (int j = 0; j < 8; ++j) {                                                       \
      DST[j] = RawVec<T>::mask(RawVec<T>::ld(rowp_ + colofs[j]), (rok_ && colok[j]) ? 0xffffffffu : 0u);  \
    }                                                                                                     \
  }

  raw_t cur[8], nxt[8];
  ROMA_DW_LOAD_ROW(0, cur);
#pragma nounroll
  for (int t = 0; t < sy + 4; ++t) {
    ROMA_DW_LOAD_ROW(t + 1, nxt);
    f32x2 v[8][2];
#pragma unroll
    for (int j = 0; j < 8; ++j) RawVec<T>::cvt(cur[j], v[j][0], v[j][1]);
#pragma unroll
// ... 74 lines not shown
  const int lane = threadIdx.x & 63;
  const int sub = lane % G, rw = lane / G;
  constexpr int RPW = 64 / G;
  const long row = ((long)blockIdx.x * 4 + (threadIdx.x >> 6)) * RPW + rw;
  float a0 = 0.f, a1 = 0.f, a2 = 0.f;
  if (row < M) {
    for (int c = sub * 4; c < Cp; c += G * 4) {
      const f32x4 v = ElemIO<T>::ld4(d + row * ldd + c);
      const f32x4 w0 = *reinterpret_cast<const f32x4*>(w + c);
      const f32x4 w1 = *reinterpret_cast<const f32x4*>(w + Cp + c);
      const f32x4 w2 = *reinterpret_cast<const f32x4*>(w + 2 * Cp + c);
#pragma unroll
      for (int j = 0; j < 4; ++j) {
        a0 = fmaf(v[j], w0[j], a0);
        a1 = fmaf(v[j], w1[j], a1);
        a2 = fmaf(v[j], w2[j], a2);
      }
    }
  }
#pragma unroll
  for (int off = G / 2; off >= 1; off >>= 1) {
    a0 += __shfl_xor(a0, off);
    a1 += __shfl_xor(a1, off);
    a2 += __shfl_xor(a2, off);
  }
  if (row < M && sub == 0) {
    flow[row * 2 + 0] += sx * (a0 + bb[0]);
    flow[row * 2 + 1] += sy * (a1 + bb[1]);
    cert[row] += a2 + bb[2];
  }
}

template <typename T, int NK>
__global__ __launch_bounds__(256) void refiner_out_vec_kernel(const T* d, long ldd, const float* w, const float* bb,
                                                              float* flow, float* cert, long M, int Cp, float sx, float sy,
                                                              int lpr, int rows_it) {
  constexpr int CV = VecIO<T>::CV;
  const int lane = threadIdx.x & 63;
  const int sub = lane & (lpr - 1), rw = lane / lpr, rpw = 64 / lpr;
  float wr[NK][3][CV];
#pragma unroll
  for (int k = 0; k < NK; ++k) {
    const int c = (sub + k * lpr) * CV;
    const bool okc = c < Cp;
#pragma unroll
    for (int o = 0; o < 3; ++o)
#pragma unroll
      for (int j4 = 0; j4 < CV; j4 += 4) {
        const f32x4 t = *reinterpret_cast<const f32x4*>(w + (long)o * Cp + (okc ? c : 0) + j4);
#pragma unroll
        for (int u = 0; u < 4; ++u) wr[k][o][j4 + u] = okc ? t[u] : 0.f;
      }
  }
  const float b0 = bb[0], b1 = bb[1], b2 = bb[2];
  const long row0 = ((long)blockIdx.x * 4 + (threadIdx.x >> 6)) * rpw * rows_it + rw;
  typedef typename VecIO<T>::Raw Raw;
  struct Group {
    Raw v[NK];
    float f0, f1, c0;
  };
  auto fetch = [&](Group& g, long row) __attribute__((always_inline)) {
    const long rowc = row < M ? row : M - 1;
    g.f0 = flow[rowc * 2 + 0];
    g.f1 = flow[rowc * 2 + 1];
    g.c0 = cert[rowc];
#pragma unroll
    for (int k = 0; k < NK; ++k) {
      const int c = (sub + k * lpr) * CV;
      g.v[k] = VecIO<T>::ldraw(d + rowc * ldd + (c < Cp ? c : 0));
    }
  };
  auto finish = [&](const Group& g, long row) __attribute__((always_inline)) {
    float a0 = 0.f, a1 = 0.f, a2 = 0.f;
#pragma unroll
    for (int k = 0; k < NK; ++k) {
      float v[CV];
      VecIO<T>::cvt(g.v[k], v);
      const bool ok = (sub + k * lpr) * CV < Cp;
#pragma unroll
      for (int j = 0; j < CV; ++j) {
        const float x = ok ? v[j] : 0.f;
        a0 = fmaf(x, wr[k][0][j], a0);
        a1 = fmaf(x, wr[k][1][j], a1);
        a2 = fmaf(x, wr[k][2][j], a2);
      }
    }
    for (int off = lpr >> 1; off >= 1; off >>= 1) {
      a0 += __shfl_xor(a0, off);
      a1 += __shfl_xor(a1, off);
      a2 += __shfl_xor(a2, off);
    }
    if (row < M && sub == 0) {
      flow[row * 2 + 0] = g.f0 + sx * (a0 + b0);
      flow[row * 2 + 1] = g.f1 + sy * (a1 + b1);
      cert[row] = g.c0 + (a2 + b2);
    }
  };
  Group ga, gb;
  fetch(ga, row0);
  for (int it = 0; it < rows_it; it += 2) {
    const long row = row0 + (long)it * rpw;
    fetch(gb, row + rpw);
    finish(ga, row);
    if (it + 2 < rows_it) fetch(ga, row + 2 * rpw);
    finish(gb, row + rpw);
  }
}

template <int NCH, int ROWS>
__global__ __launch_bounds__(256) void refiner_out_row_kernel(const bf16_t* d, long ldd, const float* w, const float* bb,
                                                              float* flow, float* cert, long M, int Cp, float sx, float sy) {
  float wr[3][NCH * 8];
#pragma unroll
  for (int o = 0; o < 3; ++o)
#pragma unroll
    for (int j = 0; j < NCH * 8; ++j) wr[o][j] = j < Cp ? w[(long)o * Cp + j] : 0.f;
  const float b0 = bb[0], b1 = bb[1], b2 = bb[2];
  const long row0 = (long)blockIdx.x * 256 * ROWS + threadIdx.x;
#pragma unroll 2
  for (int it = 0; it < ROWS; ++it) {
    const long row = row0 + (long)it * 256;
    if (row >= M) break;
    const f32x2 f = *reinterpret_cast<const f32x2*>(flow + row * 2);
    const float c0 = cert[row];
    float v[NCH][8];
#pragma unroll
    for (int k = 0; k < NCH; ++k) VecIO<bf16_t>::ld(d + row * ldd + k * 8, v[k]);
    float a0 = 0.f, a1 = 0.f, a2 = 0.f;
#pragma unroll
    for (int k = 0; k < NCH; ++k)
#pragma unroll
      for (int j = 0; j < 8; ++j) {
        a0 = fmaf(v[k][j], wr[0][k * 8 + j], a0);
        a1 = fmaf(v[k][j], wr[1][k * 8 + j], a1);
        a2 = fmaf(v[k][j], wr[2][k * 8 + j], a2);
      }
    *reinterpret_cast<f32x2*>(flow + row * 2) = f32x2{f[0] + sx * (a0 + b0), f[1] + sy * (a1 + b1)};
    cert[row] = c0 + (a2 + b2);
  }
}

__global__ __launch_bounds__(256) void refiner_apply_delta_kernel(const f32x4* __restrict__ delta, float* __restrict__ flow,
                                                                  float* __restrict__ cert, long M, float sx, float sy) {
  for (long i = (long)blockIdx.x * 256 + threadIdx.x; i < M; i += (long)gridDim.x * 256) {
    const f32x4 d = delta[i];
    f32x2 f = *reinterpret_cast<const f32x2*>(flow + 2 * i);
    f[0] += sx * d[0];
    f[1] += sy * d[1];
    *reinterpret_cast<f32x2*>(flow + 2 * i) = f;
    cert[i] += d[2];
  }
}

int refiner_apply_delta_launch(const float* delta, float* flow, float* cert, long M, float sx, float sy, hipStream_t s) {
  ROMA_REQUIRE((reinterpret_cast<uintptr_t>(delta) & 15) == 0 && (reinterpret_cast<uintptr_t>(flow) & 7) == 0, "refiner_apply_delta: alignment");
  const long nb = std::min<long>((M + 255) / 256, 256 * 32);
  hipLaunchKernelGGL(refiner_apply_delta_kernel, dim3((unsigned)nb), dim3(256), 0, s, (const f32x4*)delta, flow, cert, M, sx, sy);
  ROMA_LAUNCH_CHECK();
  return 0;
}

int refiner_out_launch(const void* d, long ldd, int dt, const float* w, const float* b, float* flow, float* cert,
                       long M, int Cp, float sx, float sy, hipStream_t s) {
  ROMA_REQUIRE(Cp % 4 == 0 && ldd % 4 == 0, "refiner_out: channel padding must be a multiple of 4");
  const int row_env = tuning(SW_OUT_ROW);
  if (row_env && dt == DT_BF16 && Cp == 24 && ldd % 8 == 0 && (reinterpret_cast<uintptr_t>(d) & 15) == 0 &&
      (reinterpret_cast<uintptr_t>(flow) & 7) == 0) {
    constexpr int ROWS = 8;
    dim3 grid((unsigned)((M + 256l * ROWS - 1) / (256l * ROWS)));
    hipLaunchKernelGGL((refiner_out_row_kernel<3, ROWS>), grid, dim3(256), 0, s, (const bf16_t*)d, ldd, w, b, flow, cert, M, Cp, sx, sy);
    ROMA_LAUNCH_CHECK();
    return 0;
  }
  {
    const int cv = dt == DT_F32 ? 4 : 8;
    const int chunks = Cp / cv;
    if (Cp % cv == 0 && ldd % cv == 0 && (reinterpret_cast<uintptr_t>(d) & 15) == 0 && (reinterpret_cast<uintptr_t>(w) & 15) == 0 && chunks >= 1) {
      int lpr = 1;
      while (lpr < 64 && lpr * 2 <= chunks) lpr *= 2;
      const int lpr_env = tuning(SW_OUT_LPR);
      if (dt == DT_BF16 && lpr_env) {
        int best_l = lpr;
        double best_e = (double)chunks / ((double)lpr * ((chunks + lpr - 1) / lpr));
        for (int l = lpr / 2; l >= 2; l /= 2) {
          const int n = (chunks + l - 1) / l;
          if (n > 5) break;
          const double e = (double)chunks / ((double)l * n);
          if (e > best_e + 1e-9) {
            best_e = e;
            best_l = l;
          }
        }
        lpr = best_l;
      }
      const int nk = (chunks + lpr - 1) / lpr;
      if (nk <= 6) {
        const int rows_it_env = tuning(SW_OUT_ROWS_IT);
        const int rows_it = rows_it_env >= 2 ? rows_it_env & ~1 : 8;
        const long rows_per_block = 4l * (64 / lpr) * rows_it;
        dim3 grid((unsigned)((M + rows_per_block - 1) / rows_per_block));
#define ROMA_ROV(NKV)                                                                                          \
  ROMA_DT_SWITCH(dt, T, hipLaunchKernelGGL((refiner_out_vec_kernel<T, NKV>), grid, dim3(256), 0, s, (const T*)d, ldd, w, b, \
                                           flow, cert, M, Cp, sx, sy, lpr, rows_it))
        if (nk <= 1) { ROMA_ROV(1); }
        else if (nk == 2) { ROMA_ROV(2); }
        else if (nk == 3) { ROMA_ROV(3); }
        else if (nk == 5) { ROMA_ROV(5); }
        else { ROMA_ROV(6); }
#undef ROMA_ROV
        ROMA_LAUNCH_CHECK();
        return 0;
      }
    }
  }
  const int chunks = Cp / 4;
#define ROMA_RO(G)                                                                                          \
  {                                                                                                         \
    const long rows_per_block = 4 * (64 / G);                                                               \
    dim3 grid((unsigned)((M + rows_per_block - 1) / rows_per_block));                                       \
    ROMA_DT_SWITCH(dt, T, hipLaunchKernelGGL((refiner_out_kernel<T, G>), grid, dim3(256), 0, s, (const T*)d, ldd, w, b, \
                                             flow, cert, M, Cp, sx, sy));                                   \
  }
  if (chunks <= 8) ROMA_RO(8)
  else if (chunks <= 16) ROMA_RO(16)
  else if (chunks <= 32) ROMA_RO(32)
  else ROMA_RO(64)
#undef ROMA_RO
  ROMA_LAUNCH_CHECK();
  return 0;
}

__device__ inline void bilinear_src(int dst, float scale, int in_size, int& i0, int& i1, float& l1) {
  float src = scale * ((float)dst + 0.5f) - 0.5f;
  if (src < 0.f) src = 0.f;
  i0 = (int)src;
  if (i0 > in_size - 1) i0 = in_size - 1;
  i1 = i0 + ((i0 < in_size - 1) ? 1 : 0);
  l1 = src - (float)i0;
}

__global__ __launch_bounds__(256) void resize_bilinear_kernel(const float* in, float* out, int B, int Hin, int Win, int Hout,
                                                              int Wout, int nc) {
  const float sh = (float)Hin / (float)Hout, sw = (float)Win / (float)Wout;
  const long total = (long)B * Hout * Wout;
  for (long idx = (long)blockIdx.x * 256 + threadIdx.x; idx < total; idx += (long)gridDim.x * 256) {
    const int x = (int)(idx % Wout);
    long r = idx / Wout;
    const int y = (int)(r % Hout);
    const int b = (int)(r / Hout);
    int y0, y1, x0, x1;
    float ly, lx;
    bilinear_src(y, sh, Hin, y0, y1, ly);
    bilinear_src(x, sw, Win, x0, x1, lx);
    const float* ib = in + (long)b * Hin * Win * nc;
    for (int c = 0; c < nc; ++c) {
      const float v00 = ib[((long)y0 * Win + x0) * nc + c], v01 = ib[((long)y0 * Win + x1) * nc + c];
      const float v10 = ib[((long)y1 * Win + x0) * nc + c], v11 = ib[((long)y1 * Win + x1) * nc + c];
      out[idx * nc + c] = (1.f - ly) * ((1.f - lx) * v00 + lx * v01) + ly * ((1.f - lx) * v10 + lx * v11);
    }
  }
}

int resize_bilinear_launch(const float* in, float* out, int B, int Hin, int Win, int Hout, int Wout, int nc,
                           hipStream_t s) {
  const long total = (long)B * Hout * Wout;
  dim3 grid((unsigned)std::min<long>((total + 255) / 256, 65536));
  hipLaunchKernelGGL(resize_bilinear_kernel, grid, dim3(256), 0, s, in, out, B, Hin, Win, Hout, Wout, nc);
  ROMA_LAUNCH_CHECK();
  return 0;
}

__global__ __launch_bounds__(256) void final_epilogue_kernel(const FinalArgs a) {
  const int Wout = a.symmetric ? 2 * a.W : a.W;
  const long total = (long)a.B * a.H * Wout;
  const float sh = a.cert16 ? (float)a.h16 / (float)a.H : 0.f, sw = a.cert16 ? (float)a.w16 / (float)a.W : 0.f;
  for (long idx = (long)blockIdx.x * 256 + threadIdx.x; idx < total; idx += (long)gridDim.x * 256) {
    const int xo = (int)(idx % Wout);
    long r = idx / Wout;
    const int y = (int)(r % a.H);
    const int bo = (int)(r / a.H);
    const int half = xo / a.W, x = xo - half * a.W;
    const int dp = bo + half * a.B;
    const long src = ((long)dp * a.H + y) * a.W + x;
    float fx = a.flow[src * 2 + 0], fy = a.flow[src * 2 + 1];
    float c = a.cert[src];
    if (a.cert16) {
      int y0, y1, x0, x1;
      float ly, lx;
      bilinear_src(y, sh, a.h16, y0, y1, ly);
      bilinear_src(x, sw, a.w16, x0, x1, lx);
      const float* cb = a.cert16 + (long)dp * a.h16 * a.w16;
      const float low = (1.f - ly) * ((1.f - lx) * cb[y0 * a.w16 + x0] + lx * cb[y0 * a.w16 + x1]) +
                        ly * ((1.f - lx) * cb[y1 * a.w16 + x0] + lx * cb[y1 * a.w16 + x1]);
      c -= (low < 0.f) ? 0.5f * low : 0.f;
    }
    c = 1.f / (1.f + expf(-c));
    if (fabsf(fx) > 1.f || fabsf(fy) > 1.f) c = 0.f;
    fx = fminf(fmaxf(fx, -1.f), 1.f);
    fy = fminf(fmaxf(fy, -1.f), 1.f);
    const float gx = pix_coord(x, a.W), gy = pix_coord(y, a.H);
    f32x4 o;
    if (half == 0) o = f32x4{gx, gy, fx, fy};
    else o = f32x4{fx, fy, gx, gy};
    *reinterpret_cast<f32x4*>(a.warp + idx * 4) = o;
    a.certainty[idx] = c;
  }
// ... 68 lines not shown
```

roma_amd/csrc/model.hip:

```cpp
#include "model.h"

#include <dlfcn.h>
#include <math.h>
#include <stdlib.h>
#include <string.h>

#include <algorithm>
#include <atomic>
#include <set>

#include "attention.h"
#include "conv64.h"
#include "pool_proj.h"
#include "elementwise.h"
#include "gemm.h"
#include "local_corr.h"
#include "refiner_block.h"
#include "vit.h"

namespace roma {

std::mutex g_peer_mutex;
extern void* g_peer_lib;
extern int g_mixed_handles;
// ... 929 lines not shown
      if (int rc = CK((up ? "p2_feat" : "p1_feat") + std::to_string(1 << l), feat[l], (size_t)nimg * fh[l] * fw_[l] * fc[l] * esz)) return rc;
    if (fw && !dry)
      for (int l = 0; l < 4; ++l)
        if (fw->feat[4 - l])
          ROMA_CHECK_HIP(hipMemcpyAsync(fw->feat[4 - l], feat[l], (size_t)nimg * fh[l] * fw_[l] * fc[l] * esz, hipMemcpyDeviceToDevice, st));
    if (debug && !dry && !up) {
      for (int l = 0; l < 4; ++l) {
        const std::string nm = "feat" + std::to_string(1 << l);
        if (int rc = dbg_save(nm.c_str(), feat[l], (size_t)nimg * fh[l] * fw_[l] * fc[l] * esz, st)) return rc;
      }
    }
    const long rows_d = (long)nimg * Nd, rows_t = (long)ndp * T;
    void *ln = nullptr, *ao = nullptr, *hid = nullptr;
    if (!up) {
      feat[4] = AL((size_t)nimg * T * 1024, esz);
      const long rmax = std::max(rows_d, rows_t);
      ln = AL((size_t)rmax * 1024, esz);
      ao = AL((size_t)rmax * 1024, esz);
      hid = AL((size_t)rmax * 4096, esz);
      const size_t dmark = arena.mark();
      void* col = AL((size_t)nimg * T * patch.ldw, esz);
      float* pt = (float*)AL((size_t)nimg * T * 1024, 4);
      float* x = (float*)AL((size_t)rows_d * 1024, 4);
      const bool res_f32_env = tuning(SW_VIT_RES_F32) != 0;
      void* xs = nullptr;
      if (act_dt == DT_BF16) xs = AL((size_t)rows_d * 1024, 2);
      void* feat_vit = feat[4];
      if (mixed) feat_vit = AL((size_t)nimg * T * 1024, 2);
      if (!dry) {
        roma_vit_block_t blk[24];
        for (int i = 0; i < 24; ++i) blk[i] = dino[i].pub();
        roma_vit_args_t va{};
        va.B = B; va.H = H; va.W = W;
        va.act = act_dt == DT_F32 ? ROMA_F32 : (mixed ? ROMA_BF16 : roma_h16_format());
        va.bf16_residual = act_dt == DT_BF16 && vit_bf16_residual && !res_f32_env;
        va.im_a = imA; va.im_b = imB;
        va.patch_w = patch.w; va.patch_b = patch.b; va.patch_ldw = patch.ldw;
        va.cls_tok = cls_tok; va.pos_emb = pos_emb;
        va.blocks = blk; va.nblocks = 24;
        va.norm_w = dino_nw; va.norm_b = dino_nb;
        va.col = col; va.pt = pt; va.x = x; va.xs = xs; va.ln = ln; va.ao = ao; va.hid = hid;
        va.q = qbuf; va.k = kbuf; va.vt = vtbuf;
        va.feat_out = feat_vit;
        if (mixed) {
          if (int rc = peer_vit_forward(&va, st)) {
            set_error("ROMA_MIXED: roma_vit_forward of the bfloat16 library failed");
            return rc;
          }
          RUN(convert_from_bf16_launch(feat_vit, feat[4], (long)nimg * T * 1024, st));
        } else {
          RUN(vit_forward(va, st));
        }
      }
      arena.release(dmark);
      if (int rc = CK("feat16", feat[4], (size_t)nimg * T * 1024 * esz)) return rc;
      if (debug && !dry)
        if (int rc = dbg_save("feat16", feat[4], (size_t)nimg * T * 1024 * esz, st)) return rc;
      if (fw && !dry && fw->feat[0])
        ROMA_CHECK_HIP(hipMemcpyAsync(fw->feat[0], feat[4], (size_t)nimg * T * 1024 * esz, hipMemcpyDeviceToDevice, st));
    }

    float *flow = pp_flow[pass][0], *cert = pp_cert[pass][0], *flow_alt = pp_flow[pass][1], *cert_alt = pp_cert[pass][1];
    int ch = 0, cw = 0;
    if (up) {
      ch = H / 8; cw = W / 8;
      if (fw) {
        RUN(resize_bilinear_launch(fw->seed_flow, flow, ndp, fw->seed_h, fw->seed_w, ch, cw, 2, st));
        RUN(resize_bilinear_launch(fw->seed_cert, cert, ndp, fw->seed_h, fw->seed_w, ch, cw, 1, st));
      } else {
        RUN(resize_bilinear_launch(flow_p1, flow, ndp, cfg.coarse_h, cfg.coarse_w, ch, cw, 2, st));
        RUN(resize_bilinear_launch(cert_p1, cert, ndp, cfg.coarse_h, cfg.coarse_w, ch, cw, 1, st));
      }
    }
    double scale_factor = sqrt((double)H * (double)W / (560.0 * 560.0));
    if (!up && coarse_scale_factor > 0.0) scale_factor = coarse_scale_factor;
    if (fw && fw->scale_factor > 0.0) scale_factor = fw->scale_factor;
    for (int si = up ? 1 : 0; si < 5; ++si) {
      const int ins = SCALE_INT[si];
      const int hs = ins == 16 ? th : H / ins, ws = ins == 16 ? tw : W / ins;
      const long hw = (long)hs * ws;
      const RefinerW& r = ref[si];
      const size_t smark = arena.mark();
      const int ldf = (int)round_up(r.Cf, 8);
      const int lvl = ins == 16 ? 4 : (ins == 8 ? 3 : (ins == 4 ? 2 : (ins == 2 ? 1 : 0)));
      const bool pf_ready = lvl < 2 && pp_on[lvl];
      void* pf = pf_ready ? pf_pre[lvl] : AL((size_t)nimg * hw * ldf, esz);
      if (!pf_ready) {
        GemmArgs g;
        g.A = feat[lvl]; g.lda = PROJ_CIN[si]; g.W = proj[si].w; g.ldw = proj[si].ldw; g.C = pf; g.ldc = ldf;
        g.M = (int)(nimg * hw); g.N = r.Cf; g.K = PROJ_CIN[si]; g.in_dt = act_dt; g.out_dt = act_dt; g.bias = proj[si].b;
        RUN(gemm_launch(g, st));
      }
      const std::string tp = std::string(up ? "p2_s" : "p1_s") + SCALES[si];
      if (int rc = CK(tp + "_proj", pf, (size_t)nimg * hw * ldf * esz)) return rc;
      if (ins == 16) {
        if (debug && !dry)
          if (int rc = dbg_save("proj16", pf, (size_t)nimg * hw * ldf * esz, st)) return rc;
        const size_t gmark = arena.mark();
        float* tokens = (float*)AL((size_t)rows_t * 1024, 4);
        const size_t gmark2 = arena.mark();
        if (int rc = gp_posterior(pf, ldf, act_dt, B, sym, th, tw, gp_w, gp_b, tokens, 1024, arena, st, dry)) return rc;
        arena.release(gmark2);
        RUN(copy2d_launch(pf, ldf, act_dt, tokens + 512, 1024, DT_F32, rows_t, 512, st));
        if (debug && !dry)
          if (int rc = dbg_save("tokens16", tokens, (size_t)rows_t * 1024 * 4, st)) return rc;
        for (int i = 0; i < 5; ++i)
          if (int rc = vit_block(tdec[i], tokens, DT_F32, rows_t, ndp, T, Npt, 8, 128, 1e-5f, ln, ao, hid)) return rc;
        const int ldl = 4104;
        float* logits = (float*)AL((size_t)rows_t * ldl, 4);
        const void* zin = tokens;
        if (act_dt != DT_F32) {
          RUN(copy2d_launch(tokens, 1024, DT_F32, ln, 1024, act_dt, rows_t, 1024, st));
          zin = ln;
        }
        {
          GemmArgs g;
          g.A = zin; g.lda = 1024; g.W = to_out.w; g.ldw = to_out.ldw; g.C = logits; g.ldc = ldl;
          g.M = (int)rows_t; g.N = to_out.N; g.K = 1024; g.in_dt = act_dt; g.out_dt = DT_F32; g.bias = to_out.b;
          RUN(gemm_launch(g, st));
        }
        if (debug && !dry)
          if (int rc = dbg_save("logits16", logits, (size_t)rows_t * ldl * 4, st)) return rc;
        if (int rc = CK(tp + "_tokens_gp", tokens, (size_t)rows_t * 1024 * 4)) return rc;
        if (int rc = CK(tp + "_logits", logits, (size_t)rows_t * ldl * 4)) return rc;
        RUN(cls_to_flow_launch(logits, ldl, flow, cert, rows_t, st));
        if (int rc = CK(tp + "_gm_flow", flow, (size_t)rows_t * 2 * 4)) return rc;
        ch = th; cw = tw;
        if (debug && !dry) {
          if (int rc = dbg_save("gm_flow16_own", flow, (size_t)rows_t * 2 * 4, st)) return rc;
          auto inj = [&](const char* nm, float* dst, size_t bytes) -> int {
            auto it = inject.find(nm);
            if (it == inject.end()) return 0;
            ROMA_REQUIRE(it->second.second == bytes, "roma_debug_inject: injected stage has the wrong size for this batch");
            ROMA_CHECK_HIP(hipMemcpyAsync(dst, it->second.first, bytes, hipMemcpyDeviceToDevice, st));
            return 0;
          };
          if (int rc = inj("gm_flow16", flow, (size_t)rows_t * 2 * 4)) return rc;
          if (int rc = inj("gm_cert16", cert, (size_t)rows_t * 4)) return rc;
        }
        if (debug && !dry) {
          if (int rc = dbg_save("gm_flow16", flow, (size_t)rows_t * 2 * 4, st)) return rc;
          if (int rc = dbg_save("gm_cert16", cert, (size_t)rows_t * 4, st)) return rc;
        }
        arena.release(gmark);
      }
      {
        const long M = (long)ndp * hw;
        void* d0 = AL((size_t)M * r.Cp, esz);
        void* d1 = AL((size_t)M * r.Cp, esz);
        RefinerInputArgs ia;
        ia.feat = pf; ia.ldf = ldf; ia.flow = flow; ia.d = d0; ia.ldd = r.Cp; ia.emb_w = r.emb_w; ia.emb_b = r.emb_b;
        ia.B = ndp; ia.H = hs; ia.W = ws; ia.C = r.Cf; ia.E = r.E; ia.Kcorr = r.K; ia.nimg = nimg; ia.shift = shift;
        ia.disp_scale = (float)(40.0 / 32.0 * scale_factor); ia.dt = act_dt;
        if (tracing)
          if (int rc = CK(tp + "_flow_before", flow, (size_t)M * 2 * 4)) return rc;
        RUN(refiner_input_launch(ia, st));
        if (r.radius) {
          LocalCorrArgs lc;
          lc.f0 = pf; lc.f1 = pf; lc.warp = flow; lc.out = off(d0, 2 * r.Cf + r.E);
          lc.B = ndp; lc.H = hs; lc.W = ws; lc.C = r.Cf; lc.radius = r.radius; lc.ld0 = ldf; lc.ld1 = ldf; lc.ldo = r.Cp;
          lc.nimg = nimg; lc.f1_shift = shift; lc.scale = 1.0f / sqrtf((float)r.Cf); lc.in_dt = act_dt; lc.out_dt = act_dt;
          const long lc_ints = local_corr_ws_ints(ndp, hs, ws, r.radius);
          lc.ws = (int*)AL((size_t)lc_ints, 4); lc.ws_bytes = lc_ints * 4;
          RUN(local_corr_window_launch(lc, st));
        }
        if (debug && !dry) {
          const std::string nm = std::string("p") + (up ? "2" : "1") + "_din" + SCALES[si];
          if ((size_t)M * r.Cp * esz <= ((size_t)(dbg_dual_slot() >= 0 ? 512 : 64) << 20))
            if (int rc = dbg_save(nm.c_str(), d0, (size_t)M * r.Cp * esz, st)) return rc;
          if (dbg_dual_slot() >= 0 && ins == 1)
            if (int rc = dbg_save((std::string("p") + (up ? "2" : "1") + "_flowin1").c_str(), flow, (size_t)M * 2 * 4, st)) return rc;
        }
        void *dcur = d0, *dalt = d1;
        if (int rc = CK(tp + "_din", d0, (size_t)M * r.Cp * esz)) return rc;
        if (tracing) {
          if (int rc = CK(tp + "_proj_again", pf, (size_t)nimg * hw * ldf * esz)) return rc;
          if (int rc = CK(tp + "_flow_again", flow, (size_t)M * 2 * 4)) return rc;
          if (int rc = CK(tp + "_din_again", d0, (size_t)M * r.Cp * esz)) return rc;
          if (esz == 2 && r.E > 0) {
            auto CKC = [&](const std::string& name, const void* p, long rows, int c0, int c1) -> int {
              if (trace_n[tslot] >= TRACE_MAX) return 0;
              const int k = trace_n[tslot]++;
              if ((int)trace_names[tslot].size() <= k) trace_names[tslot].push_back(name);
              else trace_names[tslot][k] = name;
              return checksum_cols_launch(p, rows, r.Cp, c0, c1, trace_dev[tslot] + k, st);
            };
            if (int rc = CKC(tp + "_din_x", d0, M, 0, r.Cf)) return rc;
            if (int rc = CKC(tp + "_din_xhat", d0, M, r.Cf, 2 * r.Cf)) return rc;
            if (int rc = CKC(tp + "_din_emb", d0, M, 2 * r.Cf, 2 * r.Cf + r.E)) return rc;
            if (int rc = CKC(tp + "_din_rest", d0, M, 2 * r.Cf + r.E, r.Cp)) return rc;
            for (int b = 0; b < ndp; ++b)
              if (int rc = CKC(tp + "_din_pair" + std::to_string(b), off(d0, (long)b * hw * r.Cp), hw, 0, r.Cp)) return rc;
          }
        }
        const bool fused = fuse_refiner_blocks && refiner_block_supported(r.Cp, act_dt);
        bool composed = false, final_done = false;
        if (dry && fused) {
          const size_t mk = arena.mark();
          (void)AL((size_t)M * 4, 4);
          arena.release(mk);
        }
        for (int b = 0; b < 9; ++b) {
          if (b == 8 && compose_out_conv && fused) {
            float* delta = (float*)AL((size_t)M * 4, 4);
            RUN(refiner_block_final_launch(dcur, delta, r.dw_w[b], r.dw_b[b], r.ocf_w, r.Cp, r.ocf_b, ndp, hs, ws, r.Cp, act_dt, st));
            const float sxf = (float)ins / (4.0f * (float)W), syf = (float)ins / (4.0f * (float)H);
            RUN(refiner_apply_delta_launch(delta, flow, cert, M, sxf, syf, st));
            composed = true;
            final_done = true;
            break;
          }
          if (b == 8 && compose_out_conv && !fused) {
            RUN(dwconv5x5_launch(dcur, dalt, r.dw_w[b], r.dw_b[b], ndp, hs, ws, r.Cp, act_dt, st));
            std::swap(dcur, dalt);
            if (int rc = CK(tp + "_dw" + std::to_string(b), dcur, (size_t)M * r.Cp * esz)) return rc;
            composed = true;
            break;
          }
          if (fused) {
            RUN(refiner_block_launch(dcur, dalt, r.dw_w[b], r.dw_b[b], r.pw[b].w, r.pw[b].ldw, r.pw[b].b, ndp, hs, ws,
                                     r.Cp, act_dt, st));
            std::swap(dcur, dalt);
            if (int rc = CK(tp + "_blk" + std::to_string(b), dcur, (size_t)M * r.Cp * esz)) return rc;
            continue;
          }
          if (fuse_refiner_blocks && !dry && refiner_block_wide_supported(r.Cp, act_dt)) {
            const int rcw = refiner_block_wide_try_launch(dcur, dalt, r.dw_w[b], r.dw_b[b], r.pw[b].w, r.pw[b].ldw, r.pw[b].b, ndp,
                                                          hs, ws, r.Cp, act_dt, st);
            if (rcw < 0) return rcw;
            if (rcw == 0) {
              std::swap(dcur, dalt);
              if (int rc = CK(tp + "_blk" + std::to_string(b), dcur, (size_t)M * r.Cp * esz)) return rc;
              continue;
            }
          }
          RUN(dwconv5x5_launch(dcur, dalt, r.dw_w[b], r.dw_b[b], ndp, hs, ws, r.Cp, act_dt, st));
          if (int rc = CK(tp + "_dw" + std::to_string(b), dalt, (size_t)M * r.Cp * esz)) return rc;
          GemmArgs g;
          g.A = dalt; g.lda = r.Cp; g.W = r.pw[b].w; g.ldw = r.pw[b].ldw; g.C = dcur; g.ldc = r.Cp;
          g.M = (int)M; g.N = r.Cp; g.K = r.Cp; g.in_dt = act_dt; g.out_dt = act_dt; g.bias = r.pw[b].b;
          g.n_alg = g.k_alg = r.C;
          RUN(gemm_launch(g, st));
          if (int rc = CK(tp + "_blk" + std::to_string(b), dcur, (size_t)M * r.Cp * esz)) return rc;
        }
        const float sx = (float)ins / (4.0f * (float)W), sy = (float)ins / (4.0f * (float)H);
        if (!final_done)
          RUN(refiner_out_launch(dcur, r.Cp, act_dt, composed ? r.oc_w : r.out_w, composed ? r.oc_b : r.out_b, flow, cert, M, r.Cp,
                                 sx, sy, st));
        if (int rc = CK(tp + "_flow", flow, (size_t)M * 2 * 4)) return rc;
        if (int rc = CK(tp + "_cert", cert, (size_t)M * 4)) return rc;
      }
      if (debug && !dry) {
        const std::string pfx = std::string("p") + (up ? "2" : "1");
        if (int rc = dbg_save((pfx + "_flow" + SCALES[si]).c_str(), flow, (size_t)ndp * hw * 2 * 4, st)) return rc;
        if (int rc = dbg_save((pfx + "_cert" + SCALES[si]).c_str(), cert, (size_t)ndp * hw * 4, st)) return rc;
      }
      if (fw && !dry) {
        if (fw->flow[si]) ROMA_CHECK_HIP(hipMemcpyAsync(fw->flow[si], flow, (size_t)ndp * hw * 2 * 4, hipMemcpyDeviceToDevice, st));
        if (fw->cert[si]) ROMA_CHECK_HIP(hipMemcpyAsync(fw->cert[si], cert, (size_t)ndp * hw * 4, hipMemcpyDeviceToDevice, st));
      }
      if (ins == 16) {
        const long nkeep = (long)ndp * hw;
        if (nkeep % 4 == 0) {
          RUN(copy2d_launch(cert, nkeep, DT_F32, cert16_keep, nkeep, DT_F32, 1, (int)nkeep, st));
        } else if (!dry) {
          ROMA_CHECK_HIP(hipMemcpyAsync(cert16_keep, cert, (size_t)nkeep * 4, hipMemcpyDeviceToDevice, st));
        }
      }
      arena.release(smark);
      if (ins != 1) {
        const int nh = H / (ins / 2), nw = W / (ins / 2);
        RUN(resize_bilinear_launch(flow, flow_alt, ndp, hs, ws, nh, nw, 2, st));
        RUN(resize_bilinear_launch(cert, cert_alt, ndp, hs, ws, nh, nw, 1, st));
        std::swap(flow, flow_alt);
        std::swap(cert, cert_alt);
        if (int rc = CK(tp + "_flow_up", flow, (size_t)ndp * nh * nw * 2 * 4)) return rc;
        ch = nh; cw = nw;
      }
    }
    (void)ch; (void)cw;
    flow_fin = flow; cert_fin = cert;
    if (!up) { flow_p1 = flow; cert_p1 = cert; }
    arena.release(pass_mark);
  }
  if (!dry && (arena.overflow || persist.overflow)) {
    arena.overflow = persist.overflow = false;
    set_error("roma_match / roma_forward: the workspace planned by roma_finalize is too small for this call (an option that "
              "changes the buffer plan was switched after roma_finalize); the results of this call are invalid");
    return -5;
  }
  if (fw) return 0;
  FinalArgs fa;
  fa.flow = flow_fin;
  fa.cert = cert_fin;
  fa.cert16 = cfg.attenuate_cert ? cert16_keep : nullptr;
  fa.warp = warp_out; fa.certainty = cert_out;
  fa.B = B; fa.H = Hfin; fa.W = Wfin; fa.h16 = th; fa.w16 = tw; fa.symmetric = cfg.symmetric;
  RUN(final_epilogue_launch(fa, st));
  if (int rc = CK("final_warp", warp_out, (size_t)B * Hfin * Wfin * (cfg.symmetric ? 2 : 1) * 4 * 4)) return rc;
  if (int rc = CK("final_cert", cert_out, (size_t)B * Hfin * Wfin * (cfg.symmetric ? 2 : 1) * 4)) return rc;
  return 0;
}

}
```

roma_amd/csrc/tuning.hip:

```cpp
#include "tuning.h"

#include <stdlib.h>
#include <string.h>

#include "../../include/roma_hip.h"

namespace roma {
void set_error(const std::string& msg);
namespace {

struct Row {
  Switch id;
  const char* key;
  const char* env;
  long def;
  int floor;
  bool tools_env;
  const char* doc;
};

constexpr Row ROWS[] = {
    {SW_GEMM8P, "gemm8p", "ROMA_GEMM8P", 1, 0, false, "large bf16 GEMMs on the 8-phase 256 x 256 kernel (1) or on the one-barrier-per-slab kernel (0)"},
    {SW_GEMM_DBG, "gemm_dbg", "ROMA_GEMM_DBG", 0, 0, false, "experiment bits of the GEMM kernels (1 skip output stores, 2 skip the K loop, 2048 no streaming stores, ...)"},
    {SW_GEMM8P_WALK, "gemm8p_walk", nullptr, -1, 1, false, "gemm8p: tile rows per group of the persistent walk (1 = row major); unset = 8 from 24 tile columns on, else 1"},
    {SW_GEMM8P_SCHED, "gemm8p_sched", "ROMA_GEMM8P_SCHED", 1, 0, false, "gemm8p K-loop schedule: 1 k-half phases, 0 quadrant phases (tools builds only)"},
    {SW_GEMM8P_MAXWG, "gemm8p_maxwg", nullptr, -1, 8, false, "gemm8p, measurement only: cap the persistent grid at n workgroups (a multiple of 8); unset = one per CU"},
    {SW_WS1X1, "ws1x1", "ROMA_WS1X1", 1, 0, false, "N = K = 576 refiner 1x1 on the weight-stationary kernel (1) or on the 256 x 192 tile kernel (0)"},
    {SW_LC_MODE, "lc_mode", "ROMA_LC_MODE", 0, 0, false, "local correlation: 0 tiled form + gather work list, 1 every tile on the gather list (key only), 2 per-pixel kernel"},
    {SW_LC_BIN, "lc_bin", "ROMA_LC_BIN", 1, 0, false, "local correlation: queries of incoherent tiles sorted by target bin (1) or gathered per query (0)"},
    {SW_CONV64, "conv64", "ROMA_CONV64", 7, 0, false, "weight-stationary VGG front end, bit mask: 1 the Cin = 64 kernels, 2 the Cin = 128 kernel, 4 the fused first layer"},
    {SW_CONV_PATCH, "conv_patch", "ROMA_CONV_PATCH", 1, 0, false, "patch-resident 3x3 kernel for slab-major VGG layers (1) or gemm8p (0); environment 0 also packs tap-major weights"},
    {SW_ATTN_XCD, "attn_xcd", "ROMA_ATTN_XCD", 1, 0, false, "attention work items in per-XCD bands of (batch, head) (1) or in plain order (0)"},
    {SW_ATTN_EXP2, "attn_exp2", nullptr, -1, 0, false, "tools only: force the 2^x softmax of the 16-bit attention kernel on / off; unset = as the caller says"},
    {SW_RB24W, "rb24w", "ROMA_RB24W", 1, 0, false, "C = 24 fused refiner block: wave-private kernel (1) or two-barrier workgroup kernel (0); consulted in tools builds only"},
    {SW_RB144_1B, "rb144_1b", "ROMA_RB144_1B", 1, 0, true, "C = 144 fused refiner block: one barrier per row (1) or two (0, tools builds only)"},
    {SW_RB_WIDE, "rb_wide", "ROMA_RB_WIDE", 0, 0, false, "C = 576 refiner block as one fused kernel (1; key 2 / 3 = with the scalar / packed stencil) or dwconv5x5 + 1x1 GEMM (0)"},
    {SW_DW_RING, "dw_ring", "ROMA_DW_RING", 1, 0, false, "depthwise 5x5: 0 register-prefetch kernel, 1 ring kernel for the large launches, 2 ring kernel for every shape it takes"},
    {SW_GP_COL, "gp_col", "ROMA_GP_COL", 1, 0, false, "GP Cholesky left-looking, one launch per block column (1) or the right-looking launch chain (0)"},
    {SW_POOL_PROJ, "pool_proj", "ROMA_POOL_PROJ", 1, 0, false, "max-pool + proj head of strides 1 / 2 in one pass (1) or as separate kernels (0)"},
    {SW_GP_COL_LEADER, "gp_col_leader", "ROMA_GP_COL_LEADER", 1, 0, false, "block-column Cholesky: one leader workgroup factorises the diagonal block (1) or every workgroup its own copy (0)"},
    {SW_GEMM8P_MINM, nullptr, "ROMA_GEMM8P_MINM", 2048, 0, false, "gemm8p: smallest M it takes for the wide (N >= 2048) dense launches"},
    {SW_GEMM_NT, nullptr, "ROMA_GEMM_NT", 1, 0, false, "non-temporal output stores in the 16-bit GEMM row writer"},
    {SW_GEMM_F32_FILL, nullptr, "ROMA_GEMM_F32_FILL", 1, 0, false, "exact-f32 GEMMs below 192 tiles of 256 x 256 run on 128 x 128 tiles"},
    {SW_GEMM_SMALLM, nullptr, "ROMA_GEMM_SMALLM", 1, 0, false, "GEMMs below 320 tiles of 128 x 128 run on 128 x 64 tiles"},
    {SW_CONV64_SY, nullptr, "ROMA_CONV64_SY", 0, 0, false, "conv64 strip height in rows; 0 = the split of H with the fewest rounds"},
    {SW_CONV_KORDER, nullptr, "ROMA_CONV_KORDER", 1, 0, false, "VGG layers with Cout >= 256 pack slab-major weight rows (read when a handle is created)"},
    {SW_RB_SY, nullptr, "ROMA_RB_SY", 0, 0, false, "fused refiner block strip height in rows; 0 = the split of H with the fewest rounds"},
    {SW_RB_DBG, nullptr, "ROMA_RB_DBG", 0, 0, true, "ablation bits of the two-barrier refiner block kernel"},
    {SW_RB_WIDE_PK, nullptr, "ROMA_RB_WIDE_PK", 1, 0, false, "rb_wide: packed (1) or scalar (0) stencil"},
    {SW_RBW_DBG, nullptr, "ROMA_RBW_DBG", 0, 0, true, "ablation bits of the rb_wide kernel (they produce wrong outputs by design)"},
    {SW_DWR_MAXSY, nullptr, "ROMA_DWR_MAXSY", 1 << 20, 0, false, "depthwise ring kernel: cap of the strip height in rows (at least 6)"},
    {SW_DW_RING_MINELEMS, nullptr, "ROMA_DW_RING_MINELEMS", 64l << 20, 0, false, "dw_ring = 1: smallest launch, in elements, that goes to the ring kernel"},
    {SW_RI_VEC, nullptr, "ROMA_RI_VEC", 1, 0, false, "refiner_input on the 16-byte vector kernel where alignment allows"},
    {SW_OUT_ROW, nullptr, "ROMA_OUT_ROW", 1, 0, false, "refiner_out: row kernel for C = 24 in 16-bit storage"},
    {SW_OUT_LPR, nullptr, "ROMA_OUT_LPR", 1, 0, false, "refiner_out, 16-bit: lanes per row chosen to fill the 16-byte pieces best"},
    {SW_OUT_ROWS_IT, nullptr, "ROMA_OUT_ROWS_IT", 0, 0, false, "refiner_out: row groups per wave (even, >= 2); otherwise 8"},
    {SW_GP_AUG, nullptr, "ROMA_GP_AUG", 1, 0, false, "GP Cholesky: right-hand sides stored behind A ride along the factorisation (0 = separate forward loop)"},
    {SW_GP_BWD2, nullptr, "ROMA_GP_BWD2", 1, 0, false, "GP Cholesky: backward substitution with one launch per step (0 = two)"},
    {SW_COMPOSE_OUT, nullptr, "ROMA_COMPOSE_OUT", 1, 0, false, "initial value of the handle option compose_out_conv (read when a handle is created)"},
    {SW_VIT_RES_F32, nullptr, "ROMA_VIT_RES_F32", 0, 0, false, "force DINOv2's f32 residual stream in the 16-bit modes"},
    {SW_STREAMS, nullptr, "ROMA_STREAMS", 0, 0, false, "number of sub-batch streams of match(); 0 = the handle's option"},
    {SW_STREAMS_SERIAL, nullptr, "ROMA_STREAMS_SERIAL", 0, 0, false, "diagnostic: sub-batch streams run one after the other"},
    {SW_DEBUG_DUAL_SLOT, nullptr, "ROMA_DEBUG_DUAL_SLOT", -1, 0, false, "diagnostic: keep the stream split in debug mode, sub-batch k captures the stages of ROMA_DEBUG_ONLY"},
};
constexpr int NROWS = sizeof(ROWS) / sizeof(ROWS[0]);
constexpr bool rows_in_enum_order() {
  for (int i = 0; i < NROWS; ++i)
    if (ROWS[i].id != i) return false;
  return true;
}
static_assert(NROWS == SW_COUNT && rows_in_enum_order(), "one row per Switch, in enum order");
constexpr bool json_plain(const char* s) {
  for (; s && *s; ++s)
    if (*s == '"' || *s == '\\' || *s < ' ') return false;
  return true;
}
constexpr bool rows_json_plain() {
  for (const Row& r : ROWS)
    if (!json_plain(r.key) || !json_plain(r.env) || !json_plain(r.doc)) return false;
  return true;
}
static_assert(rows_json_plain(), "keys, environment names and docs: plain ASCII without quote, backslash or control character");

#ifdef ROMA_TOOLS_BUILD
constexpr bool TOOLS_BUILD = true;
#else
constexpr bool TOOLS_BUILD = false;
#endif

struct Overrides {
  long v[SW_COUNT];
  constexpr Overrides() : v{} {
    for (long& x : v) x = -1;
  }
};
[[clang::require_constant_initialization]] Overrides g_override;

struct Env {
  long v[SW_COUNT];
  Env() {
    for (int i = 0; i < NROWS; ++i) {
      const char* s = ROWS[i].env && (TOOLS_BUILD || !ROWS[i].tools_env) ? getenv(ROWS[i].env) : nullptr;
      v[i] = s ? atol(s) : ROWS[i].def;
    }
  }
};
const Env& env() {
  static const Env e;
  return e;
}

}

long tuning_env(Switch id) { return env().v[id]; }
long tuning_override(Switch id) { return g_override.v[id] >= ROWS[id].floor ? g_override.v[id] : -1; }
long tuning(Switch id) { return g_override.v[id] >= ROWS[id].floor ? g_override.v[id] : tuning_env(id); }

int tuning_set(const char* key, long value) {
  for (const Row& r : ROWS)
    if (r.key && !strcmp(r.key, key)) {
      g_override.v[r.id] = value >= r.floor ? value : -1;
      return 0;
    }
  set_error(std::string("roma_tuning: unknown key ") + key);
  return ROMA_ERR_ARG;
}

std::string tuning_describe() {
  std::string js = "[";
  for (const Row& r : ROWS) {
    const auto quoted = [](const char* s) { return s ? "\"" + std::string(s) + "\"" : std::string("null"); };
    const long ov = tuning_override(r.id);
    js += std::string(r.id ? ", " : "") + "{\"key\": " + quoted(r.key) + ", \"env\": " + quoted(r.env) +
          ", \"default\": " + std::to_string(r.def) + ", \"override\": " + (ov >= 0 ? std::to_string(ov) : "null") +
          ", \"value\": " + std::to_string(tuning(r.id)) + ", \"tools_only_env\": " + (r.tools_env ? "true" : "false") + ", \"doc\": " + quoted(r.doc) + "}";
  }
  return js + "]";
}

}
```

Measured before the change: 106.5 image-pairs/s.

## Fuse refiner x-copy into block-0 depthwise conv and out-conv into last depthwise

For the wide ConvRefiner path on the ring depthwise kernel, refiner_input no longer copies the feature columns of x into the block input. The block-0 depthwise conv reads them straight from the feature map as a second source. The last block's depthwise conv also applies the 1x1 output conv in-kernel and writes per-channel-chunk partial sums. A small kernel then reduces those partials into flow and certainty. This removes one large activation copy and the full-size store and reload of the last depthwise output, at the cost of a more complex kernel template and an extra partials buffer.

```diff
diff --git a/include/roma_hip.h b/include/roma_hip.h
--- a/include/roma_hip.h
+++ b/include/roma_hip.h
@@ -118,8 +118,17 @@
 int roma_op_refiner_input(const void* feat, long ldf, const float* flow, void* d, long ldd, const float* emb_w,
                           const float* emb_b, int B, int H, int W, int C, int E, int Kcorr, int nimg, int shift,
                           float disp_scale, int dt, void* stream);
+int roma_op_refiner_input_skip(const void* feat, long ldf, const float* flow, void* d, long ldd, const float* emb_w,
+                               const float* emb_b, int B, int H, int W, int C, int E, int Kcorr, int nimg, int shift,
+                               float disp_scale, int dt, int skip_x, void* stream);
 int roma_op_dwconv5x5(const void* in, void* out, const float* w, const float* bias, int B, int H, int W, int Cp, int dt,
                       void* stream);
+int roma_op_dwconv5x5_two_source(const void* in, const void* x2, long ldx, int Cx, void* out, const float* w, const float* bias,
+                                 int B, int H, int W, int Cp, int dt, void* stream);
+int roma_op_dwconv5x5_final(const void* in, float* part, const float* w, const float* bias, const float* oc_w, int B, int H, int W,
+                            int Cp, int dt, void* stream);
+int roma_op_refiner_out_partials(const float* part, int nblk, const float* b, float* flow, float* cert, long M, float sx, float sy,
+                                 void* stream);
 int roma_op_refiner_block(const void* in, void* out, const float* dw_w, const float* dw_b, const void* pw,
                           const float* pw_b, int B, int H, int W, int Cp, int dt, void* stream);
 int roma_op_refiner_block_final(const void* in, float* delta, const float* dw_w, const float* dw_b, const void* pw_final,
diff --git a/roma_amd/_lib.py b/roma_amd/_lib.py
--- a/roma_amd/_lib.py
+++ b/roma_amd/_lib.py
@@ -65,7 +65,11 @@
     "roma_op_cls_to_flow": (_i, [_vp, _l, _vp, _vp, _l, _vp]),
     "roma_op_resize_bilinear": (_i, [_vp, _vp, _i, _i, _i, _i, _i, _i, _vp]),
     "roma_op_refiner_input": (_i, [_vp, _l, _vp, _vp, _l, _vp, _vp, _i, _i, _i, _i, _i, _i, _i, _i, _f, _i, _vp]),
+    "roma_op_refiner_input_skip": (_i, [_vp, _l, _vp, _vp, _l, _vp, _vp, _i, _i, _i, _i, _i, _i, _i, _i, _f, _i, _i, _vp]),
     "roma_op_dwconv5x5": (_i, [_vp, _vp, _vp, _vp, _i, _i, _i, _i, _i, _vp]),
+    "roma_op_dwconv5x5_two_source": (_i, [_vp, _vp, _l, _i, _vp, _vp, _vp, _i, _i, _i, _i, _i, _vp]),
+    "roma_op_dwconv5x5_final": (_i, [_vp, _vp, _vp, _vp, _vp, _i, _i, _i, _i, _i, _vp]),
+    "roma_op_refiner_out_partials": (_i, [_vp, _i, _vp, _vp, _vp, _l, _f, _f, _vp]),
     "roma_op_refiner_block": (_i, [_vp, _vp, _vp, _vp, _vp, _vp, _i, _i, _i, _i, _i, _vp]),
     "roma_op_refiner_block_final": (_i, [_vp, _vp, _vp, _vp, _vp, _vp, _i, _i, _i, _i, _i, _vp]),
     "roma_op_refiner_apply_delta": (_i, [_vp, _vp, _vp, _l, _f, _f, _vp]),
diff --git a/roma_amd/csrc/api.hip b/roma_amd/csrc/api.hip
--- a/roma_amd/csrc/api.hip
+++ b/roma_amd/csrc/api.hip
@@ -438,9 +438,45 @@
   return refiner_input_launch(a, S(stream));
 }
 
+int roma_op_refiner_input_skip(const void* feat, long ldf, const float* flow, void* d, long ldd, const float* emb_w,
+                               const float* emb_b, int B, int H, int W, int C, int E, int Kcorr, int nimg, int shift,
+                               float disp_scale, int dt, int skip_x, void* stream) {
+  RefinerInputArgs a;
+  a.feat = feat; a.ldf = ldf; a.flow = flow; a.d = d; a.ldd = ldd; a.emb_w = emb_w; a.emb_b = emb_b;
+  a.B = B; a.H = H; a.W = W; a.C = C; a.E = E; a.Kcorr = Kcorr; a.nimg = nimg; a.shift = shift;
+  a.disp_scale = disp_scale; a.dt = DT(dt); a.skip_x = skip_x != 0;
+  ROMA_REQUIRE(feat && flow && d && B > 0 && H > 0 && W > 0 && C > 0 && nimg > 0, "roma_op_refiner_input_skip: bad arguments");
+  ROMA_REQUIRE(ldd >= 2 * C + E + Kcorr && ldf >= C, "roma_op_refiner_input_skip: row strides too small");
+  return refiner_input_launch(a, S(stream));
+}
+
 int roma_op_dwconv5x5(const void* in, void* out, const float* w, const float* bias, int B, int H, int W, int Cp, int dt,
                       void* stream) {
   return dwconv5x5_launch(in, out, w, bias, B, H, W, Cp, DT(dt), S(stream));
+}
+
+int roma_op_dwconv5x5_two_source(const void* in, const void* x2, long ldx, int Cx, void* out, const float* w, const float* bias,
+                                 int B, int H, int W, int Cp, int dt, void* stream) {
+  ROMA_REQUIRE(in && x2 && out && w && bias && in != out && x2 != out, "roma_op_dwconv5x5_two_source: bad pointers");
+  const int rc = dwconv5x5_two_source_try_launch(in, x2, ldx, Cx, out, w, bias, B, H, W, Cp, DT(dt), S(stream));
+  if (rc <= 0) return rc;
+  set_error("roma_op_dwconv5x5_two_source: the ring kernel declined this problem (shape, alignment or the dw_ring switch)");
+  return ROMA_ERR_ARG;
+}
+
+int roma_op_dwconv5x5_final(const void* in, float* part, const float* w, const float* bias, const float* oc_w, int B, int H, int W,
+                            int Cp, int dt, void* stream) {
+  ROMA_REQUIRE(in && part && w && bias && oc_w, "roma_op_dwconv5x5_final: null pointer");
+  const int rc = dwconv5x5_final_try_launch(in, part, w, bias, oc_w, B, H, W, Cp, DT(dt), S(stream));
+  if (rc <= 0) return rc;
+  set_error("roma_op_dwconv5x5_final: the ring kernel declined this problem (shape, alignment or the dw_ring switch)");
+  return ROMA_ERR_ARG;
+}
+
+int roma_op_refiner_out_partials(const float* part, int nblk, const float* b, float* flow, float* cert, long M, float sx, float sy,
+                                 void* stream) {
+  ROMA_REQUIRE(part && b && flow && cert && M > 0 && nblk >= 1, "roma_op_refiner_out_partials: bad arguments");
+  return refiner_out_partials_launch(part, nblk, b, flow, cert, M, sx, sy, S(stream));
 }
 
 int roma_op_refiner_block(const void* in, void* out, const float* dw_w, const float* dw_b, const void* pw,
diff --git a/roma_amd/csrc/dwconv_ring.hip b/roma_amd/csrc/dwconv_ring.hip
--- a/roma_amd/csrc/dwconv_ring.hip
+++ b/roma_amd/csrc/dwconv_ring.hip
@@ -1,234 +1,28 @@
-#include <stdlib.h>
-
-#include <algorithm>
-
-#include "elementwise.h"
-#include "tuning.h"
-#include "gemm.h"
+#include "dwconv_ring.inc"
 
 namespace roma {
 
-typedef __attribute__((ext_vector_type(2))) float f32x2;
-#define ROMA_LDS __attribute__((address_space(3)))
-typedef ROMA_LDS unsigned char lds_u8;
+static int dwr_mode() { return (int)(tuning(SW_DW_RING) & 3); }
+bool dwconv5x5_two_source_enabled() { return (tuning(SW_DW_RING) & 4) == 0; }
+bool dwconv5x5_final_enabled() { return (tuning(SW_DW_RING) & 8) == 0; }
 
-__device__ __attribute__((aligned(256))) unsigned int g_dwr_zero_page[64];
-
-constexpr int DWR_ROWB = 3072;
-constexpr int DWR_PXW = 16;
-constexpr int DWR_NR = 6;
-constexpr int DWR_RING = 4 * DWR_NR * DWR_ROWB;
-static_assert(3 * (DWR_NR - 1) + 4 * (DWR_NR - 1) <= 63, "vmcnt is a 6-bit counter");
-static_assert(2 * DWR_RING <= 160 * 1024, "two workgroups per CU");
-
-#define ROMA_DWR_WAIT_VM(N) asm volatile("s_waitcnt vmcnt(%0)" ::"n"(N) : "memory")
-
-__device__ __forceinline__ void dwr_glds16(const char* src, lds_u8* lds_wave_base) {
-  __builtin_amdgcn_global_load_lds((const __attribute__((address_space(1))) void*)src, (ROMA_LDS void*)lds_wave_base, 16, 0, 0);
-}
-
-__device__ __forceinline__ void dwr_read(unsigned long long (&cr)[8], unsigned rd) {
-  asm volatile(
-      "ds_read_b64 %0, %8\n\tds_read_b64 %1, %8 offset:128\n\tds_read_b64 %2, %8 offset:256\n\t"
-      "ds_read_b64 %3, %8 offset:384\n\tds_read_b64 %4, %8 offset:640\n\tds_read_b64 %5, %8 offset:768\n\t"
-      "ds_read_b64 %6, %8 offset:896\n\tds_read_b64 %7, %8 offset:1024"
-      : "=&v"(cr[0]), "=&v"(cr[1]), "=&v"(cr[2]), "=&v"(cr[3]), "=&v"(cr[4]), "=&v"(cr[5]), "=&v"(cr[6]), "=&v"(cr[7])
-      : "v"(rd)
-      : "memory");
-}
-__device__ __forceinline__ void dwr_wait(unsigned long long (&cr)[8]) {
-  asm volatile("s_waitcnt lgkmcnt(0)"
-               : "+v"(cr[0]), "+v"(cr[1]), "+v"(cr[2]), "+v"(cr[3]), "+v"(cr[4]), "+v"(cr[5]), "+v"(cr[6]), "+v"(cr[7])::"memory");
-}
-
-__device__ __forceinline__ void dwr_row(f32x2 (&acc)[5][4][2], const f32x4 (&wreg)[25], f32x2 bias0, f32x2 bias1,
-                                        unsigned long long (&cr)[8], unsigned rd_next, bool store, bf16_t* orow, long Cp, int npx) {
-  f32x2 v[8][2];
-#define ROMA_DWR_CVT(J)                                                  \
-  {                                                                      \
-    const uint32_t lo_ = (uint32_t)cr[J], hi_ = (uint32_t)(cr[J] >> 32); \
-    v[J][0] = f32x2{h16_lo(lo_), h16_hi(lo_)};                           \
-    v[J][1] = f32x2{h16_lo(hi_), h16_hi(hi_)};                           \
-  }
-  ROMA_DWR_CVT(0) ROMA_DWR_CVT(1) ROMA_DWR_CVT(2) ROMA_DWR_CVT(3) ROMA_DWR_CVT(4) ROMA_DWR_CVT(5) ROMA_DWR_CVT(6) ROMA_DWR_CVT(7)
-#undef ROMA_DWR_CVT
-#pragma unroll
-  for (int j = 0; j < 8; ++j) asm volatile("" : "+v"(v[j][0]), "+v"(v[j][1]));
-  dwr_read(cr, rd_next);
-#pragma unroll
-  for (int kx = 0; kx < 5; ++kx) {
-    __builtin_amdgcn_sched_barrier(0);
-#pragma unroll
-    for (int k = 0; k < 5; ++k) {
-      const f32x4 wx = wreg[(4 - k) * 5 + kx];
-      const f32x2 w0 = f32x2{wx[0], wx[1]}, w1 = f32x2{wx[2], wx[3]};
-#pragma unroll
-      for (int px = 0; px < 4; ++px) {
-        acc[k][px][0] = v[px + kx][0] * w0 + (k == 4 && kx == 0 ? bias0 : acc[k][px][0]);
-        acc[k][px][1] = v[px + kx][1] * w1 + (k == 4 && kx == 0 ? bias1 : acc[k][px][1]);
-      }
-    }
-    __builtin_amdgcn_sched_barrier(0);
-  }
-  if (store) {
-#pragma unroll
-    for (int px = 0; px < 4; ++px) {
-      if (px < npx) {
-        uint2 u;
-        u.x = pack_relu_h16x2(acc[0][px][0][0], acc[0][px][0][1]);
-        u.y = pack_relu_h16x2(acc[0][px][1][0], acc[0][px][1][1]);
-        *reinterpret_cast<uint2*>(orow + (long)px * Cp) = u;
-      }
-    }
-  }
-#pragma unroll
-  for (int k = 0; k < 4; ++k)
-#pragma unroll
-    for (int px = 0; px < 4; ++px) {
-      acc[k][px][0] = acc[k + 1][px][0];
-      acc[k][px][1] = acc[k + 1][px][1];
-    }
-  dwr_wait(cr);
-}
-
-__global__ __launch_bounds__(256, 2) void dwconv5x5_ring_kernel(const bf16_t* __restrict__ in, bf16_t* __restrict__ out,
-                                                                const float* __restrict__ w, const float* __restrict__ bias,
-                                                                int B, int H, int W, int Cp, int SY, int nchunk, int nxg,
-                                                                long ntasks) {
-  constexpr int NR = DWR_NR;
-  __shared__ __attribute__((aligned(1024))) unsigned char ring[DWR_RING];
-  const long nwg = (ntasks + 3) / 4, wg_per_xcd = (nwg + 7) / 8;
-  const long lw = (long)(blockIdx.x % 8) * wg_per_xcd + blockIdx.x / 8;
-  const int lane = threadIdx.x & 63;
-  const int wv = __builtin_amdgcn_readfirstlane((int)(threadIdx.x >> 6));
-  const long task = lw * 4 + wv;
-  if (lw >= nwg || task >= ntasks) return;
-  const int xg = (int)(task % nxg);
-  long r = task / nxg;
-  const int chunk = (int)(r % nchunk);
-  r /= nchunk;
-  const int yt = (H + SY - 1) / SY;
-  const int ys = (int)(r % yt) * SY;
-  const int b = (int)(r / yt);
-  const int sy = min(SY, H - ys);
-  const int T = sy + 4;
-
-  const int cg = lane & 15, xq = lane >> 4;
-  const int c = chunk * 64 + cg * 4;
-
-  f32x4 wreg[25];
-#pragma unroll
-  for (int t = 0; t < 25; ++t) wreg[t] = *reinterpret_cast<const f32x4*>(w + (long)t * Cp + c);
-  const f32x4 bx = *reinterpret_cast<const f32x4*>(bias + c);
-#pragma unroll
-  for (int t = 0; t < 25; ++t) asm volatile("" : "+v"(wreg[t]));
-  const f32x2 bias0 = f32x2{bx[0], bx[1]}, bias1 = f32x2{bx[2], bx[3]};
-  asm volatile("s_waitcnt vmcnt(0)" ::: "memory");
-
-  const int xb = xg * DWR_PXW + xq * 4;
-  const int x0 = xg * DWR_PXW - 2;
-  const int npx = min(4, W - xb);
-
-  const char* zsrc = reinterpret_cast<const char*>(g_dwr_zero_page);
-  const char* inb = reinterpret_cast<const char*>(in + ((long)b * H * W) * Cp) + (long)chunk * 128;
-  const long pitch = (long)W * Cp * 2;
-  const __amdgpu_buffer_rsrc_t rs_in = __builtin_amdgcn_make_buffer_rsrc(const_cast<char*>(inb), 0, (int)((long)H * pitch - (long)chunk * 128), 0x00020000);
-  unsigned voff[3];
-#pragma unroll
-  for (int i = 0; i < 3; ++i) {
-    const int p = 64 * i + lane, s = p >> 3, part = p & 7;
-    const int x = x0 + s - s / 5;
-    const bool ok = (s % 5 != 4) && x >= 0 && x < W;
-    voff[i] = ok ? (unsigned)(x * Cp * 2 + part * 16) : 0x80000000u;
-  }
-  unsigned vout = 0x80000000u;
-  asm volatile("" : "+v"(vout));
-  lds_u8* const myring = (lds_u8*)ring + wv * (NR * DWR_ROWB);
-#define ROMA_DWR_BL16(VOFF, SOFF, DST) \
-  __builtin_amdgcn_raw_ptr_buffer_load_lds(rs_in, (ROMA_LDS void*)(DST), 16, (int)(VOFF), (int)(SOFF), 0, 0)
-#define ROMA_DWR_ISSUE(RROW, SLOT)                                                         \
-  {                                                                                        \
-    const int yy_ = ys - 2 + (RROW);                                                       \
-    if ((RROW) < T && yy_ >= 0 && yy_ < H) {                             \
-      const int so_ = yy_ * (int)pitch;                                                    \
-      _Pragma("unroll") for (int i = 0; i < 3; ++i) ROMA_DWR_BL16(voff[i], so_, myring + (SLOT) * DWR_ROWB + i * 1024); \
-    } else {                                                                               \
-      _Pragma("unroll") for (int i = 0; i < 3; ++i) ROMA_DWR_BL16(vout, 0, myring + (SLOT) * DWR_ROWB + i * 1024); \
-    }                                                                                      \
-  }
-
-  f32x2 acc[5][4][2];
-#pragma unroll
-  for (int s5 = 0; s5 < 5; ++s5)
-#pragma unroll
-    for (int px = 0; px < 4; ++px) {
-      acc[s5][px][0] = bias0;
-      acc[s5][px][1] = bias1;
-    }
-  const unsigned ring_lds = (unsigned)(size_t)myring;
-  const unsigned rd0 = ring_lds + (unsigned)(xq * 5 * 128 + cg * 8);
-  bf16_t* const obase = out + ((long)b * H * W) * Cp + c;
-
-#pragma unroll
-  for (int rr = 0; rr < NR - 1; ++rr) ROMA_DWR_ISSUE(rr, rr);
-  unsigned long long cr[8];
-  ROMA_DWR_WAIT_VM(3 * (NR - 2));
-  dwr_read(cr, rd0);
-  dwr_wait(cr);
-
-  int slot1 = 1;
-  int fill = NR - 1;
-  bf16_t* orow = obase + ((long)ys * W + xb) * Cp;
-  const long orow_step = (long)W * Cp;
-#pragma nounroll
-  for (int t = 0; t < T; ++t) {
-    ROMA_DWR_ISSUE(t + NR - 1, fill);
-    ROMA_DWR_WAIT_VM(3 * (NR - 2));
-    const bool st = t >= 4;
-    dwr_row(acc, wreg, bias0, bias1, cr, rd0 + (unsigned)slot1 * DWR_ROWB, st && npx > 0, orow, (long)Cp, npx);
-    if (st) orow += orow_step;
-    fill = fill + 1 == NR ? 0 : fill + 1;
-    slot1 = slot1 + 1 == NR ? 0 : slot1 + 1;
-  }
-#undef ROMA_DWR_ISSUE
-  ROMA_DWR_WAIT_VM(0);
+bool dwconv5x5_ring_takes(int B, int H, int W, int Cp, int dt) {
+  const int dw_ring = dwr_mode();
+  if (!dw_ring) return false;
+  if (dt != DT_BF16 || Cp % 64 != 0 || Cp < (dw_ring == 2 ? 64 : 256) || B < 1 || H < 1 || W < 1) return false;
+  if ((long)H * W * Cp * 2 >= (1l << 31)) return false;
+  return dw_ring == 2 || (long)B * H * W * Cp >= tuning(SW_DW_RING_MINELEMS);
 }
 
 int dwconv5x5_ring_try_launch(const void* in, void* out, const float* w, const float* bias, int B, int H, int W, int Cp, int dt,
                               hipStream_t s) {
-  const int dw_ring = tuning(SW_DW_RING);
-  if (!dw_ring) return 1;
-  if (dt != DT_BF16 || Cp % 64 != 0 || Cp < 256 || H < 1 || W < 1) return 1;
-  if ((long)H * W * Cp * 2 >= (1l << 31)) return 1;
-  if ((reinterpret_cast<uintptr_t>(in) & 15) != 0 || (reinterpret_cast<uintptr_t>(out) & 7) != 0) return 1;
-  if ((reinterpret_cast<uintptr_t>(w) & 15) != 0 || (reinterpret_cast<uintptr_t>(bias) & 15) != 0) return 1;
-  const int nchunk = Cp / 64;
-  const int nxg = (W + DWR_PXW - 1) / DWR_PXW;
-  int SY = H;
-  {
-    long best = -1;
-    const long per_strip = (long)B * nxg * nchunk;
-    const int max_sy = std::max(6, (int)tuning(SW_DWR_MAXSY));
-    for (int ns = (H + max_sy - 1) / max_sy; ns <= std::max(1, H / 6); ++ns) {
-      const int sy = (H + ns - 1) / ns;
-      const long nt = per_strip * ((H + sy - 1) / sy);
-      const long cost = ((nt + 2047) / 2048) * (sy + 7);
-      if (best < 0 || cost < best) {
-        best = cost;
-        SY = sy;
-      }
-    }
-  }
-  const long ntasks = (long)B * ((H + SY - 1) / SY) * nxg * nchunk;
-  ROMA_REQUIRE(ntasks < (1l << 31), "dwconv5x5: grid too large");
-  const long min_elems = tuning(SW_DW_RING_MINELEMS);
-  if (dw_ring != 2 && (long)B * H * W * Cp < min_elems) return 1;
-  ProfScope ps("dwconv5x5_kernel<" ROMA_H16_NAME ">", 2.0 * (double)B * H * W * Cp * 2.0, "byte", s);
-  const long nwg = (ntasks + 3) / 4;
-  hipLaunchKernelGGL(dwconv5x5_ring_kernel, dim3((unsigned)(((nwg + 7) / 8) * 8)), dim3(256), 0, s, (const bf16_t*)in,
-                     (bf16_t*)out, w, bias, B, H, W, Cp, SY, nchunk, nxg, ntasks);
-  ROMA_LAUNCH_CHECK();
-  return 0;
+  return dwr_launch<false>(in, out, w, bias, B, H, W, Cp, dt, nullptr, 0, 0, nullptr, nullptr, s);
+}
+
+int dwconv5x5_two_source_try_launch(const void* in, const void* x2, long ldx, int Cx, void* out, const float* w, const float* bias,
+                                    int B, int H, int W, int Cp, int dt, hipStream_t s) {
+  if (!x2) return 1;
+  return dwr_launch<false>(in, out, w, bias, B, H, W, Cp, dt, x2, ldx, Cx, nullptr, nullptr, s);
 }
 
 }
diff --git a/roma_amd/csrc/dwconv_ring.inc b/roma_amd/csrc/dwconv_ring.inc
--- /dev/null
+++ b/roma_amd/csrc/dwconv_ring.inc
@@ -0,0 +1,289 @@
+#pragma once
+#include <stdlib.h>
+
+#include <algorithm>
+
+#include "elementwise.h"
+#include "tuning.h"
+#include "gemm.h"
+
+namespace roma {
+
+typedef __attribute__((ext_vector_type(2))) float f32x2;
+#define ROMA_LDS __attribute__((address_space(3)))
+typedef ROMA_LDS unsigned char lds_u8;
+
+static __device__ __attribute__((aligned(256))) unsigned int g_dwr_zero_page[64];
+
+constexpr int DWR_ROWB = 3072;
+constexpr int DWR_PXW = 16;
+constexpr int DWR_NR = 6;
+constexpr int DWR_RING = 4 * DWR_NR * DWR_ROWB;
+static_assert(3 * (DWR_NR - 1) + 4 * (DWR_NR - 1) <= 63, "vmcnt is a 6-bit counter");
+static_assert(2 * DWR_RING <= 160 * 1024, "two workgroups per CU");
+
+#define ROMA_DWR_WAIT_VM(N) asm volatile("s_waitcnt vmcnt(%0)" ::"n"(N) : "memory")
+
+__device__ __forceinline__ void dwr_glds16(const char* src, lds_u8* lds_wave_base) {
+  __builtin_amdgcn_global_load_lds((const __attribute__((address_space(1))) void*)src, (ROMA_LDS void*)lds_wave_base, 16, 0, 0);
+}
+
+__device__ __forceinline__ void dwr_read(unsigned long long (&cr)[8], unsigned rd) {
+  asm volatile(
+      "ds_read_b64 %0, %8\n\tds_read_b64 %1, %8 offset:128\n\tds_read_b64 %2, %8 offset:256\n\t"
+      "ds_read_b64 %3, %8 offset:384\n\tds_read_b64 %4, %8 offset:640\n\tds_read_b64 %5, %8 offset:768\n\t"
+      "ds_read_b64 %6, %8 offset:896\n\tds_read_b64 %7, %8 offset:1024"
+      : "=&v"(cr[0]), "=&v"(cr[1]), "=&v"(cr[2]), "=&v"(cr[3]), "=&v"(cr[4]), "=&v"(cr[5]), "=&v"(cr[6]), "=&v"(cr[7])
+      : "v"(rd)
+      : "memory");
+}
+__device__ __forceinline__ void dwr_wait(unsigned long long (&cr)[8]) {
+  asm volatile("s_waitcnt lgkmcnt(0)"
+               : "+v"(cr[0]), "+v"(cr[1]), "+v"(cr[2]), "+v"(cr[3]), "+v"(cr[4]), "+v"(cr[5]), "+v"(cr[6]), "+v"(cr[7])::"memory");
+}
+
+template <int CTRL>
+__device__ __forceinline__ float dwr_dpp_add(float v) {
+  return v + __builtin_bit_cast(float, __builtin_amdgcn_update_dpp(0, __builtin_bit_cast(int, v), CTRL, 0xf, 0xf, false));
+}
+template <bool FINAL>
+__device__ __forceinline__ void dwr_row(f32x2 (&acc)[5][4][2], const f32x4 (&wreg)[25], f32x2 bias0, f32x2 bias1,
+                                        unsigned long long (&cr)[8], unsigned rd_next, bool store, bf16_t* orow, long Cp, int npx,
+                                        const f32x4 (&ow)[3], f32x4* prow, int cg) {
+  f32x2 v[8][2];
+#define ROMA_DWR_CVT(J)                                                  \
+  {                                                                      \
+    const uint32_t lo_ = (uint32_t)cr[J], hi_ = (uint32_t)(cr[J] >> 32); \
+    v[J][0] = f32x2{h16_lo(lo_), h16_hi(lo_)};                           \
+    v[J][1] = f32x2{h16_lo(hi_), h16_hi(hi_)};                           \
+  }
+  ROMA_DWR_CVT(0) ROMA_DWR_CVT(1) ROMA_DWR_CVT(2) ROMA_DWR_CVT(3) ROMA_DWR_CVT(4) ROMA_DWR_CVT(5) ROMA_DWR_CVT(6) ROMA_DWR_CVT(7)
+#undef ROMA_DWR_CVT
+#pragma unroll
+  for (int j = 0; j < 8; ++j) asm volatile("" : "+v"(v[j][0]), "+v"(v[j][1]));
+  dwr_read(cr, rd_next);
+#pragma unroll
+  for (int kx = 0; kx < 5; ++kx) {
+    __builtin_amdgcn_sched_barrier(0);
+#pragma unroll
+    for (int k = 0; k < 5; ++k) {
+      const f32x4 wx = wreg[(4 - k) * 5 + kx];
+      const f32x2 w0 = f32x2{wx[0], wx[1]}, w1 = f32x2{wx[2], wx[3]};
+#pragma unroll
+      for (int px = 0; px < 4; ++px) {
+        acc[k][px][0] = v[px + kx][0] * w0 + (k == 4 && kx == 0 ? bias0 : acc[k][px][0]);
+        acc[k][px][1] = v[px + kx][1] * w1 + (k == 4 && kx == 0 ? bias1 : acc[k][px][1]);
+      }
+    }
+    __builtin_amdgcn_sched_barrier(0);
+  }
+  if constexpr (FINAL) {
+    if (store) {
+      f32x4 mine = {0.f, 0.f, 0.f, 0.f};
+#pragma unroll
+      for (int px = 0; px < 4; ++px) {
+        const uint32_t lo = pack_relu_h16x2(acc[0][px][0][0], acc[0][px][0][1]), hi = pack_relu_h16x2(acc[0][px][1][0], acc[0][px][1][1]);
+        const float y0 = h16_lo(lo), y1 = h16_hi(lo), y2 = h16_lo(hi), y3 = h16_hi(hi);
+        float p[3];
+#pragma unroll
+        for (int o = 0; o < 3; ++o) {
+          p[o] = fmaf(y3, ow[o][3], fmaf(y2, ow[o][2], fmaf(y1, ow[o][1], y0 * ow[o][0])));
+          p[o] = dwr_dpp_add<0xB1>(p[o]);
+          p[o] = dwr_dpp_add<0x4E>(p[o]);
+          p[o] = dwr_dpp_add<0x141>(p[o]);
+          p[o] = dwr_dpp_add<0x140>(p[o]);
+        }
+        if (cg == px) mine = f32x4{p[0], p[1], p[2], 0.f};
+      }
+      if (cg < npx) *prow = mine;
+    }
+  } else if (store) {
+#pragma unroll
+    for (int px = 0; px < 4; ++px) {
+      if (px < npx) {
+        uint2 u;
+        u.x = pack_relu_h16x2(acc[0][px][0][0], acc[0][px][0][1]);
+        u.y = pack_relu_h16x2(acc[0][px][1][0], acc[0][px][1][1]);
+        *reinterpret_cast<uint2*>(orow + (long)px * Cp) = u;
+      }
+    }
+  }
+#pragma unroll
+  for (int k = 0; k < 4; ++k)
+#pragma unroll
+    for (int px = 0; px < 4; ++px) {
+      acc[k][px][0] = acc[k + 1][px][0];
+      acc[k][px][1] = acc[k + 1][px][1];
+    }
+  dwr_wait(cr);
+}
+
+template <bool FINAL>
+__global__ __launch_bounds__(256, 2) void dwconv5x5_ring_kernel(const bf16_t* __restrict__ in, bf16_t* __restrict__ out,
+                                                                const float* __restrict__ w, const float* __restrict__ bias,
+                                                                int B, int H, int W, int Cp, int SY, int nchunk, int nxg,
+                                                                long ntasks, const bf16_t* __restrict__ x2, int ldx, int Cx,
+                                                                const float* __restrict__ ocw, f32x4* __restrict__ part) {
+  constexpr int NR = DWR_NR;
+  __shared__ __attribute__((aligned(1024))) unsigned char ring[DWR_RING];
+  const long nwg = (ntasks + 3) / 4, wg_per_xcd = (nwg + 7) / 8;
+  const long lw = (long)(blockIdx.x % 8) * wg_per_xcd + blockIdx.x / 8;
+  const int lane = threadIdx.x & 63;
+  const int wv = __builtin_amdgcn_readfirstlane((int)(threadIdx.x >> 6));
+  const long task = lw * 4 + wv;
+  if (lw >= nwg || task >= ntasks) return;
+  const int xg = (int)(task % nxg);
+  long r = task / nxg;
+  const int chunk = (int)(r % nchunk);
+  r /= nchunk;
+  const int yt = (H + SY - 1) / SY;
+  const int ys = (int)(r % yt) * SY;
+  const int b = (int)(r / yt);
+  const int sy = min(SY, H - ys);
+  const int T = sy + 4;
+
+  const int cg = lane & 15, xq = lane >> 4;
+  const int c = chunk * 64 + cg * 4;
+
+  f32x4 wreg[25];
+#pragma unroll
+  for (int t = 0; t < 25; ++t) wreg[t] = *reinterpret_cast<const f32x4*>(w + (long)t * Cp + c);
+  const f32x4 bx = *reinterpret_cast<const f32x4*>(bias + c);
+#pragma unroll
+  for (int t = 0; t < 25; ++t) asm volatile("" : "+v"(wreg[t]));
+  const f32x2 bias0 = f32x2{bx[0], bx[1]}, bias1 = f32x2{bx[2], bx[3]};
+  f32x4 ow[3] = {};
+  if constexpr (FINAL) {
+#pragma unroll
+    for (int o = 0; o < 3; ++o) {
+      ow[o] = *reinterpret_cast<const f32x4*>(ocw + (long)o * Cp + c);
+      asm volatile("" : "+v"(ow[o]));
+    }
+  }
+  asm volatile("s_waitcnt vmcnt(0)" ::: "memory");
+
+  const int xb = xg * DWR_PXW + xq * 4;
+  const int x0 = xg * DWR_PXW - 2;
+  const int npx = min(4, W - xb);
+
+  const char* zsrc = reinterpret_cast<const char*>(g_dwr_zero_page);
+  const bool from_x2 = chunk * 64 < Cx;
+  const int ld = from_x2 ? ldx : Cp;
+  const char* inb = reinterpret_cast<const char*>((from_x2 ? x2 : in) + ((long)b * H * W) * ld) + (long)chunk * 128;
+  const long pitch = (long)W * ld * 2;
+  const __amdgpu_buffer_rsrc_t rs_in = __builtin_amdgcn_make_buffer_rsrc(const_cast<char*>(inb), 0, (int)((long)H * pitch - (long)chunk * 128), 0x00020000);
+  unsigned voff[3];
+#pragma unroll
+  for (int i = 0; i < 3; ++i) {
+    const int p = 64 * i + lane, s = p >> 3, part = p & 7;
+    const int x = x0 + s - s / 5;
+    const bool ok = (s % 5 != 4) && x >= 0 && x < W;
+    voff[i] = ok ? (unsigned)(x * ld * 2 + part * 16) : 0x80000000u;
+  }
+  unsigned vout = 0x80000000u;
+  asm volatile("" : "+v"(vout));
+  lds_u8* const myring = (lds_u8*)ring + wv * (NR * DWR_ROWB);
+#define ROMA_DWR_BL16(VOFF, SOFF, DST) \
+  __builtin_amdgcn_raw_ptr_buffer_load_lds(rs_in, (ROMA_LDS void*)(DST), 16, (int)(VOFF), (int)(SOFF), 0, 0)
+#define ROMA_DWR_ISSUE(RROW, SLOT)                                                         \
+  {                                                                                        \
+    const int yy_ = ys - 2 + (RROW);                                                       \
+    if ((RROW) < T && yy_ >= 0 && yy_ < H) {                             \
+      const int so_ = yy_ * (int)pitch;                                                    \
+      _Pragma("unroll") for (int i = 0; i < 3; ++i) ROMA_DWR_BL16(voff[i], so_, myring + (SLOT) * DWR_ROWB + i * 1024); \
+    } else {                                                                               \
+      _Pragma("unroll") for (int i = 0; i < 3; ++i) ROMA_DWR_BL16(vout, 0, myring + (SLOT) * DWR_ROWB + i * 1024); \
+    }                                                                                      \
+  }
+
+  f32x2 acc[5][4][2];
+#pragma unroll
+  for (int s5 = 0; s5 < 5; ++s5)
+#pragma unroll
+    for (int px = 0; px < 4; ++px) {
+      acc[s5][px][0] = bias0;
+      acc[s5][px][1] = bias1;
+    }
+  const unsigned ring_lds = (unsigned)(size_t)myring;
+  const unsigned rd0 = ring_lds + (unsigned)(xq * 5 * 128 + cg * 8);
+  bf16_t* const obase = out + ((long)b * H * W) * Cp + c;
+
+#pragma unroll
+  for (int rr = 0; rr < NR - 1; ++rr) ROMA_DWR_ISSUE(rr, rr);
+  unsigned long long cr[8];
+  ROMA_DWR_WAIT_VM(3 * (NR - 2));
+  dwr_read(cr, rd0);
+  dwr_wait(cr);
+
+  int slot1 = 1;
+  int fill = NR - 1;
+  bf16_t* orow = obase + ((long)ys * W + xb) * Cp;
+  const long orow_step = (long)W * Cp;
+  f32x4* prow = FINAL ? part + (((long)b * H + ys) * W + xb + cg) * nchunk + chunk : nullptr;
+  const long prow_step = (long)W * nchunk;
+#pragma nounroll
+  for (int t = 0; t < T; ++t) {
+    ROMA_DWR_ISSUE(t + NR - 1, fill);
+    ROMA_DWR_WAIT_VM(3 * (NR - 2));
+    const bool st = t >= 4;
+    dwr_row<FINAL>(acc, wreg, bias0, bias1, cr, rd0 + (unsigned)slot1 * DWR_ROWB, FINAL ? st : st && npx > 0, orow, (long)Cp, npx, ow,
+                   prow, cg);
+    if (st) {
+      if constexpr (FINAL) prow += prow_step; else orow += orow_step;
+    }
+    fill = fill + 1 == NR ? 0 : fill + 1;
+    slot1 = slot1 + 1 == NR ? 0 : slot1 + 1;
+  }
+#undef ROMA_DWR_ISSUE
+  ROMA_DWR_WAIT_VM(0);
+}
+
+template <bool FINAL>
+static int dwr_launch(const void* in, void* out, const float* w, const float* bias, int B, int H, int W, int Cp, int dt,
+                      const void* x2, long ldx, int Cx, const float* ocw, float* part, hipStream_t s) {
+  if (!dwconv5x5_ring_takes(B, H, W, Cp, dt)) return 1;
+  if ((reinterpret_cast<uintptr_t>(in) & 15) != 0 || (reinterpret_cast<uintptr_t>(out) & 7) != 0) return 1;
+  if ((reinterpret_cast<uintptr_t>(w) & 15) != 0 || (reinterpret_cast<uintptr_t>(bias) & 15) != 0) return 1;
+  if (x2) {
+    if (Cx < 64 || Cx % 64 != 0 || Cx > Cp || ldx < Cx || ldx % 8 != 0 || (reinterpret_cast<uintptr_t>(x2) & 15) != 0) return 1;
+    if ((long)H * W * ldx * 2 >= (1l << 31)) return 1;
+  } else {
+    Cx = 0;
+  }
+  if (FINAL && ((reinterpret_cast<uintptr_t>(ocw) & 15) != 0 || (reinterpret_cast<uintptr_t>(part) & 15) != 0 || !part)) return 1;
+  const int nchunk = Cp / 64;
+  const int nxg = (W + DWR_PXW - 1) / DWR_PXW;
+  int SY = H;
+  {
+    long best = -1;
+    const long per_strip = (long)B * nxg * nchunk;
+    const int max_sy = std::max(6, (int)tuning(SW_DWR_MAXSY));
+    for (int ns = (H + max_sy - 1) / max_sy; ns <= std::max(1, H / 6); ++ns) {
+      const int sy = (H + ns - 1) / ns;
+      const long nt = per_strip * ((H + sy - 1) / sy);
+      const long cost = ((nt + 2047) / 2048) * (sy + 7);
+      if (best < 0 || cost < best) {
+        best = cost;
+        SY = sy;
+      }
+    }
+  }
+  const long ntasks = (long)B * ((H + SY - 1) / SY) * nxg * nchunk;
+  ROMA_REQUIRE(ntasks < (1l << 31), "dwconv5x5: grid too large");
+  const long nwg = (ntasks + 3) / 4;
+  const dim3 grid((unsigned)(((nwg + 7) / 8) * 8));
+  if constexpr (FINAL) {
+    ProfScope ps("dwconv5x5_final_kernel<" ROMA_H16_NAME ">", (double)B * H * W * (Cp * 2.0 + nchunk * 16.0), "byte", s);
+    hipLaunchKernelGGL(dwconv5x5_ring_kernel<true>, grid, dim3(256), 0, s, (const bf16_t*)in, (bf16_t*)nullptr, w, bias, B, H, W, Cp,
+                       SY, nchunk, nxg, ntasks, (const bf16_t*)x2, (int)ldx, Cx, ocw, (f32x4*)part);
+    ROMA_LAUNCH_CHECK();
+  } else {
+    ProfScope ps("dwconv5x5_kernel<" ROMA_H16_NAME ">", 2.0 * (double)B * H * W * Cp * 2.0, "byte", s);
+    hipLaunchKernelGGL(dwconv5x5_ring_kernel<false>, grid, dim3(256), 0, s, (const bf16_t*)in, (bf16_t*)out, w, bias, B, H, W, Cp, SY,
+                       nchunk, nxg, ntasks, (const bf16_t*)x2, (int)ldx, Cx, (const float*)nullptr, (f32x4*)nullptr);
+    ROMA_LAUNCH_CHECK();
+  }
+  return 0;
+}
+
+}
diff --git a/roma_amd/csrc/dwconv_ring_final.hip b/roma_amd/csrc/dwconv_ring_final.hip
--- /dev/null
+++ b/roma_amd/csrc/dwconv_ring_final.hip
@@ -0,0 +1,11 @@
+#include "dwconv_ring.inc"
+
+namespace roma {
+
+int dwconv5x5_final_try_launch(const void* in, float* part, const float* w, const float* bias, const float* oc_w, int B, int H,
+                               int W, int Cp, int dt, hipStream_t s) {
+  if (!oc_w || !part) return 1;
+  return dwr_launch<true>(in, nullptr, w, bias, B, H, W, Cp, dt, nullptr, 0, 0, oc_w, part, s);
+}
+
+}
diff --git a/roma_amd/csrc/elementwise.h b/roma_amd/csrc/elementwise.h
--- a/roma_amd/csrc/elementwise.h
+++ b/roma_amd/csrc/elementwise.h
@@ -54,6 +54,7 @@
   int B = 0, H = 0, W = 0, C = 0, E = 0, Kcorr = 0, nimg = 0, shift = 0;
   float disp_scale = 1.f;
   int dt = 0;
+  int skip_x = 0;
 };
 int refiner_input_launch(const RefinerInputArgs& a, hipStream_t s);
 
@@ -61,9 +62,18 @@
                      int dt, hipStream_t s);
 int dwconv5x5_ring_try_launch(const void* in, void* out, const float* w, const float* bias, int B, int H, int W, int Cp, int dt,
                               hipStream_t s);
+bool dwconv5x5_ring_takes(int B, int H, int W, int Cp, int dt);
+bool dwconv5x5_two_source_enabled();
+bool dwconv5x5_final_enabled();
+int dwconv5x5_two_source_try_launch(const void* in, const void* x2, long ldx, int Cx, void* out, const float* w, const float* bias,
+                                    int B, int H, int W, int Cp, int dt, hipStream_t s);
+int dwconv5x5_final_try_launch(const void* in, float* part, const float* w, const float* bias, const float* oc_w , int B,
+                               int H, int W, int Cp, int dt, hipStream_t s);
 
 int refiner_out_launch(const void* d, long ldd, int dt, const float* w , const float* b ,
                        float* flow, float* cert, long M, int Cp, float sx, float sy, hipStream_t s);
+int refiner_out_partials_launch(const float* part, int nblk, const float* b , float* flow, float* cert, long M, float sx,
+                                float sy, hipStream_t s);
 int refiner_apply_delta_launch(const float* delta, float* flow, float* cert, long M, float sx, float sy, hipStream_t s);
 
 int resize_bilinear_launch(const float* in, float* out, int B, int Hin, int Win, int Hout, int Wout, int nc,
diff --git a/roma_amd/csrc/elementwise.hip b/roma_amd/csrc/elementwise.hip
--- a/roma_amd/csrc/elementwise.hip
+++ b/roma_amd/csrc/elementwise.hip
@@ -533,7 +533,7 @@
     off[t] = ((long)yy * a.W + xx) * a.ldf;
   }
   for (int c = lane * 4; c < a.C; c += 256) {
-    ElemIO<T>::st4(d + c, ElemIO<T>::ld4(fq + c));
+    if (!a.skip_x) ElemIO<T>::st4(d + c, ElemIO<T>::ld4(fq + c));
     f32x4 acc = {0.f, 0.f, 0.f, 0.f};
 #pragma unroll
     for (int t = 0; t < 4; ++t)
@@ -564,7 +564,7 @@
     const long p = pix - (long)b * HW;
     T* d = reinterpret_cast<T*>(a.d) + pix * a.ldd;
     if (c < a.C) {
-      ElemIO<T>::st(d + c, ElemIO<T>::ld(feat + ((long)b * HW + p) * a.ldf + c));
+      if (!a.skip_x) ElemIO<T>::st(d + c, ElemIO<T>::ld(feat + ((long)b * HW + p) * a.ldf + c));
     } else if (c < 2 * a.C) {
       const int cc = c - a.C;
       const int simg = (b + a.shift) % a.nimg;
@@ -688,6 +688,12 @@
 #pragma unroll
     for (int c = 2 * C + E; c < LDD; ++c) o[c] = 0.f;
     T* d = reinterpret_cast<T*>(a.d) + pix * LDD;
+    if (a.skip_x) {
+#pragma unroll
+      for (int c = C; c < 16; ++c) ElemIO<T>::st(d + c, o[c]);
+      VecIO<T>::st(d + 16, o + 16);
+      return;
+    }
 #pragma unroll
     for (int c8 = 0; c8 < LDD / 8; ++c8) VecIO<T>::st(d + c8 * 8, o + c8 * 8);
     return;
@@ -735,6 +741,11 @@
 #pragma unroll
   for (int c = 2 * C + E; c < LDD; ++c) o[c] = 0.f;
   T* d = reinterpret_cast<T*>(a.d) + pix * LDD;
+  if (a.skip_x) {
+#pragma unroll
+    for (int c = C; c < LDD; ++c) ElemIO<T>::st(d + c, o[c]);
+    return;
+  }
 #pragma unroll
   for (int c4 = 0; c4 < LDD / 4; ++c4) ElemIO<T>::st4(d + c4 * 4, f32x4{o[c4 * 4], o[c4 * 4 + 1], o[c4 * 4 + 2], o[c4 * 4 + 3]});
 }
@@ -772,7 +783,7 @@
     off[t] = ((long)min(max(yy, 0), a.H - 1) * a.W + min(max(xx, 0), a.W - 1)) * a.ldf;
   }
   for (int c = sub * CV; c < a.C; c += lpp * CV) {
-    *reinterpret_cast<uint4*>(d + c) = *reinterpret_cast<const uint4*>(fq + c);
+    if (!a.skip_x) *reinterpret_cast<uint4*>(d + c) = *reinterpret_cast<const uint4*>(fq + c);
     float r[CV];
 #pragma unroll
     for (int j = 0; j < CV; ++j) r[j] = 0.f;
@@ -798,7 +809,8 @@
   const double es = a.dt == DT_F32 ? 4.0 : 2.0;
   char pname[64];
   snprintf(pname, sizeof pname, "refiner_input_warp<C=%d,%s>", a.C, a.dt == DT_F32 ? "f32" : ROMA_H16_NAME);
-  ProfScope ps(pname, (double)npix * (2.0 * a.C * es + 8.0 + (double)(a.ldd - a.Kcorr) * es), "byte", s);
+  const double xb = a.skip_x ? 2.0 * a.C * es : 0.0;
+  ProfScope ps(pname, (double)npix * (2.0 * a.C * es + 8.0 + (double)(a.ldd - a.Kcorr) * es - xb), "byte", s);
   if (a.C == 9 && a.E == 6 && a.Kcorr == 0 && a.ldf == 16 && a.ldd == 24) {
     dim3 grid((unsigned)((npix + 255) / 256));
     ROMA_DT_SWITCH(a.dt, T, hipLaunchKernelGGL((refiner_input_pix_kernel<T, 9, 6>), grid, dim3(256), 0, s, a));
@@ -1179,6 +1191,39 @@
   }
 }
 
+__global__ __launch_bounds__(256) void refiner_out_partials_kernel(const f32x4* __restrict__ part, int nblk, const float* __restrict__ bb,
+                                                                   float* __restrict__ flow, float* __restrict__ cert, long M,
+                                                                   float sx, float sy) {
+  const float b0 = bb[0], b1 = bb[1], b2 = bb[2];
+  for (long i = (long)blockIdx.x * 256 + threadIdx.x; i < M; i += (long)gridDim.x * 256) {
+    const f32x4* p = part + i * nblk;
+    const f32x2 f = *reinterpret_cast<const f32x2*>(flow + 2 * i);
+    const float c0 = cert[i];
+    f32x4 v = p[0];
+    float a0 = v[0], a1 = v[1], a2 = v[2];
+#pragma unroll 4
+    for (int k = 1; k < nblk; ++k) {
+      v = p[k];
+      a0 += v[0];
+      a1 += v[1];
+      a2 += v[2];
+    }
+    *reinterpret_cast<f32x2*>(flow + 2 * i) = f32x2{f[0] + sx * (a0 + b0), f[1] + sy * (a1 + b1)};
+    cert[i] = c0 + (a2 + b2);
+  }
+}
+
+int refiner_out_partials_launch(const float* part, int nblk, const float* b, float* flow, float* cert, long M, float sx, float sy,
+                                hipStream_t s) {
+  ROMA_REQUIRE(nblk >= 1 && (reinterpret_cast<uintptr_t>(part) & 15) == 0 && (reinterpret_cast<uintptr_t>(flow) & 7) == 0,
+               "refiner_out_partials: alignment");
+  ProfScope ps("refiner_out_partials_kernel", (double)M * (nblk * 16.0 + 24.0), "byte", s);
+  const long nb = std::min<long>((M + 255) / 256, 256 * 32);
+  hipLaunchKernelGGL(refiner_out_partials_kernel, dim3((unsigned)nb), dim3(256), 0, s, (const f32x4*)part, nblk, b, flow, cert, M, sx, sy);
+  ROMA_LAUNCH_CHECK();
+  return 0;
+}
+
 int refiner_apply_delta_launch(const float* delta, float* flow, float* cert, long M, float sx, float sy, hipStream_t s) {
   ROMA_REQUIRE((reinterpret_cast<uintptr_t>(delta) & 15) == 0 && (reinterpret_cast<uintptr_t>(flow) & 7) == 0, "refiner_apply_delta: alignment");
   const long nb = std::min<long>((M + 255) / 256, 256 * 32);
diff --git a/roma_amd/csrc/model.hip b/roma_amd/csrc/model.hip
--- a/roma_amd/csrc/model.hip
+++ b/roma_amd/csrc/model.hip
@@ -1105,6 +1105,13 @@
         ia.feat = pf; ia.ldf = ldf; ia.flow = flow; ia.d = d0; ia.ldd = r.Cp; ia.emb_w = r.emb_w; ia.emb_b = r.emb_b;
         ia.B = ndp; ia.H = hs; ia.W = ws; ia.C = r.Cf; ia.E = r.E; ia.Kcorr = r.K; ia.nimg = nimg; ia.shift = shift;
         ia.disp_scale = (float)(40.0 / 32.0 * scale_factor); ia.dt = act_dt;
+        const bool fused = fuse_refiner_blocks && refiner_block_supported(r.Cp, act_dt);
+        const bool ring = !fused && dwconv5x5_ring_takes(ndp, hs, ws, r.Cp, act_dt);
+        const bool blk0_wide = fuse_refiner_blocks && tuning(SW_RB_WIDE) && refiner_block_wide_supported(r.Cp, act_dt);
+        const auto al16 = [](const void* p) { return (reinterpret_cast<uintptr_t>(p) & 15) == 0; };
+        const bool x_from_pf = ring && !blk0_wide && dwconv5x5_two_source_enabled() && !tracing && !debug && r.Cf >= 64 &&
+                               r.Cf % 64 == 0 && ldf % 8 == 0 && al16(pf) && al16(d0) && al16(d1) && al16(r.dw_w[0]) && al16(r.dw_b[0]);
+        ia.skip_x = x_from_pf;
         if (tracing)
           if (int rc = CK(tp + "_flow_before", flow, (size_t)M * 2 * 4)) return rc;
         RUN(refiner_input_launch(ia, st));
@@ -1146,11 +1153,16 @@
               if (int rc = CKC(tp + "_din_pair" + std::to_string(b), off(d0, (long)b * hw * r.Cp), hw, 0, r.Cp)) return rc;
           }
         }
-        const bool fused = fuse_refiner_blocks && refiner_block_supported(r.Cp, act_dt);
         bool composed = false, final_done = false;
         if (dry && fused) {
           const size_t mk = arena.mark();
           (void)AL((size_t)M * 4, 4);
+          arena.release(mk);
+        }
+        const int nblk64 = (r.Cp + 63) / 64;
+        if (dry && !fused) {
+          const size_t mk = arena.mark();
+          (void)AL((size_t)M * nblk64 * 4, 4);
           arena.release(mk);
         }
         for (int b = 0; b < 9; ++b) {
@@ -1162,6 +1174,19 @@
             composed = true;
             final_done = true;
             break;
+          }
+          if (b == 8 && compose_out_conv && ring && dwconv5x5_final_enabled() && !dry) {
+            float* part = (float*)AL((size_t)M * nblk64 * 4, 4);
+            const int rcf = dwconv5x5_final_try_launch(dcur, part, r.dw_w[b], r.dw_b[b], r.oc_w, ndp, hs, ws, r.Cp, act_dt, st);
+            if (rcf < 0) return rcf;
+            if (rcf == 0) {
+              if (int rc = CK(tp + "_dw" + std::to_string(b) + "_part", part, (size_t)M * nblk64 * 16)) return rc;
+              const float sxf = (float)ins / (4.0f * (float)W), syf = (float)ins / (4.0f * (float)H);
+              RUN(refiner_out_partials_launch(part, nblk64, r.oc_b, flow, cert, M, sxf, syf, st));
+              composed = true;
+              final_done = true;
+              break;
+            }
           }
           if (b == 8 && compose_out_conv && !fused) {
             RUN(dwconv5x5_launch(dcur, dalt, r.dw_w[b], r.dw_b[b], ndp, hs, ws, r.Cp, act_dt, st));
@@ -1187,7 +1212,13 @@
               continue;
             }
           }
-          RUN(dwconv5x5_launch(dcur, dalt, r.dw_w[b], r.dw_b[b], ndp, hs, ws, r.Cp, act_dt, st));
+          if (b == 0 && x_from_pf && !dry) {
+            const int rc2 = dwconv5x5_two_source_try_launch(dcur, pf, ldf, r.Cf, dalt, r.dw_w[b], r.dw_b[b], ndp, hs, ws, r.Cp, act_dt, st);
+            if (rc2 < 0) return rc2;
+            ROMA_REQUIRE(rc2 == 0, "ConvRefiner: the two-source depthwise kernel declined block 0 (the x columns of its input were not written)");
+          } else {
+            RUN(dwconv5x5_launch(dcur, dalt, r.dw_w[b], r.dw_b[b], ndp, hs, ws, r.Cp, act_dt, st));
+          }
           if (int rc = CK(tp + "_dw" + std::to_string(b), dalt, (size_t)M * r.Cp * esz)) return rc;
           GemmArgs g;
           g.A = dalt; g.lda = r.Cp; g.W = r.pw[b].w; g.ldw = r.pw[b].ldw; g.C = dcur; g.ldc = r.Cp;
diff --git a/roma_amd/csrc/tuning.hip b/roma_amd/csrc/tuning.hip
--- a/roma_amd/csrc/tuning.hip
+++ b/roma_amd/csrc/tuning.hip
@@ -35,7 +35,7 @@
     {SW_RB24W, "rb24w", "ROMA_RB24W", 1, 0, false, "C = 24 fused refiner block: wave-private kernel (1) or two-barrier workgroup kernel (0); consulted in tools builds only"},
     {SW_RB144_1B, "rb144_1b", "ROMA_RB144_1B", 1, 0, true, "C = 144 fused refiner block: one barrier per row (1) or two (0, tools builds only)"},
     {SW_RB_WIDE, "rb_wide", "ROMA_RB_WIDE", 0, 0, false, "C = 576 refiner block as one fused kernel (1; key 2 / 3 = with the scalar / packed stencil) or dwconv5x5 + 1x1 GEMM (0)"},
-    {SW_DW_RING, "dw_ring", "ROMA_DW_RING", 1, 0, false, "depthwise 5x5: 0 register-prefetch kernel, 1 ring kernel for the large launches, 2 ring kernel for every shape it takes"},
+    {SW_DW_RING, "dw_ring", "ROMA_DW_RING", 1, 0, false, "depthwise 5x5, low two bits: 0 register-prefetch kernel, 1 ring kernel for the large launches, 2 ring kernel for every shape it takes; + 4 wide ConvRefiner block 0 reads a copied x (no second source), + 8 wide last block stores its map (no FINAL form)"},
     {SW_GP_COL, "gp_col", "ROMA_GP_COL", 1, 0, false, "GP Cholesky left-looking, one launch per block column (1) or the right-looking launch chain (0)"},
     {SW_POOL_PROJ, "pool_proj", "ROMA_POOL_PROJ", 1, 0, false, "max-pool + proj head of strides 1 / 2 in one pass (1) or as separate kernels (0)"},
     {SW_GP_COL_LEADER, "gp_col_leader", "ROMA_GP_COL_LEADER", 1, 0, false, "block-column Cholesky: one leader workgroup factorises the diagonal block (1) or every workgroup its own copy (0)"},
```

Measured after the change: 107.0 image-pairs/s (median of 6 runs). No clear change (+0.5%).
